# bxh1/VIDO-SLAM

Hardware: AMD Instinct MI355X
Metric: frames/sec end-to-end (flow+depth+track+local-BA) at 640x480; BA iters/sec (higher is better)
Workload: dtype f32

## Files before the change

include/vido_c.h:

```cpp
#ifndef VIDO_C_H
#define VIDO_C_H
#include <stdint.h>
#include <stddef.h>
#ifdef __cplusplus
extern "C" {
#endif

#define VIDO_OK              0
#define VIDO_E_INVALID      -1
#define VIDO_E_NO_DEVICE    -2
#define VIDO_E_HIP          -3
#define VIDO_E_CAPACITY     -4
#define VIDO_E_NOMEM        -5

#define VIDO_MAX_LEVELS 16

typedef struct vido_ctx vido_ctx;

typedef struct vido_keypoint { float x, y, size, angle, response; int32_t octave; } vido_keypoint;

typedef struct vido_config {
    int32_t device;
    int32_t width, height;
    int32_t max_batch;
// ... 93 lines not shown
    double info_edge, info_prior, huber_delta;
    int32_t use_huber, rounds, drop_kernel_after_round;
    int32_t iters[4];
    float chi2_th[4];
} vido_pose_problem;

typedef struct vido_pose_result { double T[16]; int32_t n_inliers, lm_iterations; double chi2_final; } vido_pose_result;

int vido_pose_optimize(vido_ctx* ctx, const vido_pose_problem* prob, vido_pose_result* result, uint8_t* outlier_out, double* flow_out);
int vido_pose_optimize_batch(vido_ctx* ctx, const vido_pose_problem* probs, int n_prob, vido_pose_result* results,
                             uint8_t* const* outlier_out, double* const* flow_out);

typedef struct vido_ba_problem {
    int32_t n_cam, n_pt, n_obs, n_odo, prior_cam, use_huber, max_iters, pad;
    double* cam_T; double* pt_xyz;
    const int32_t* obs_cam; const int32_t* obs_pt; const double* obs_meas;
    const int32_t* odo_i; const int32_t* odo_j; const double* odo_T;
    double prior_T[12];
    double info_obs, info_odo, info_prior, huber_obs, huber_odo, gain_threshold;
    int32_t pt_lo, pt_hi;
    int32_t rank, world;
} vido_ba_problem;

typedef struct vido_ba_result { int32_t iterations, lm_trials; double chi2_initial, chi2_final, lambda_final;
                                double ms_setup;
                                double ms_solve_loop;
                                double ms_linearize_kernel;
                                double ms_schur_kernel;
} vido_ba_result;

typedef int (*vido_allreduce_fn)(void* user, void* dev_ptr, size_t count, int op);

int vido_ba_optimize(vido_ctx* ctx, vido_ba_problem* prob, vido_ba_result* result, vido_allreduce_fn allreduce, void* user);
int vido_rccl_unique_id(uint8_t id_out[128]);
int vido_rccl_init(vido_ctx* ctx, const uint8_t id[128], int rank, int world);
int vido_rccl_allreduce(void* user_ctx, void* dev_ptr, size_t count, int op);
int vido_rccl_destroy(vido_ctx* ctx);

typedef struct vido_ba_dynamic {
    int32_t n_H, n_dyn, n_tern, n_smooth;
    double* H_T;
    double* dyn_xyz;
    const int32_t* dyn_cam; const double* dyn_meas;
    const int32_t* tern_prev; const int32_t* tern_cur; const int32_t* tern_H;
    const int32_t* sm_i; const int32_t* sm_j;
    double info_dyn, info_tern, info_smooth, huber_dyn, huber_tern, huber_smooth;
} vido_ba_dynamic;
int vido_ba_optimize_dynamic(vido_ctx* ctx, vido_ba_problem* prob, vido_ba_dynamic* dyn, vido_ba_result* result,
                             vido_allreduce_fn allreduce, void* user);

int vido_correlation(vido_ctx* ctx, const float* first, const float* second, int B, int C, int H, int W, int stride,
                     float* out, int on_device);
int vido_det_order(vido_ctx* ctx, const float* scores, const long long* labels, const int* n_det, float confidence, int cap, long long* order, long long* labels_out, long long* n_live);
int vido_roi_levels(vido_ctx* ctx, const float* boxes, int n, float k_min, float k_max, int* out);
int vido_mask_logit_select(vido_ctx* ctx, const float* feat, const float* w, const float* b, const long long* labels, float* out, int n, int c, int hw, int classes);
int vido_bias_act(vido_ctx* ctx, float* x, const float* bias, int N, int C, int H, int W, float slope);
int vido_bias_unary(vido_ctx* ctx, float* x, const float* bias, int N, int C, int H, int W, int kind);
int vido_upcat_reflect(vido_ctx* ctx, const float* x, const float* skip, int C1, int C2, int h, int w, float* out);
int vido_minmax_norm_u16(vido_ctx* ctx, const float* d, const float* mm, int64_t n, int32_t* out);
int vido_bias_res_act(vido_ctx* ctx, float* x, const float* bias, const float* res, int N, int C, int H, int W, float slope);
int vido_area_feed(vido_ctx* ctx, const uint8_t* bgr, int H, int W, float* out, int OH, int OW, float div);
int vido_backwarp(vido_ctx* ctx, const float* x, const float* flow, int B, int C, int H, int W, float* out);
int vido_deconv4s2_depthwise(vido_ctx* ctx, const float* x, const float* weight, int B, int C, int H, int W, float input_slope, float* out);

int vido_conv1x1_supported(int cin, int cout, int hw);
int vido_conv1x1_layout(int cin, int cout, int hw);
int vido_conv1x1_set_arith(int arith);
int vido_conv1x1_range_flag(vido_ctx* ctx, int reset);
int vido_range_latch(vido_ctx* ctx, unsigned* dst);
int vido_conv1x1_bias_act(vido_ctx* ctx, const float* x, const float* w_packed, const float* bias, const float* residual, float* y, int cin, int cout, int hw, float slope);
int vido_deconv2x2_supported(int n, int cin, int cout, int h, int w);
int vido_deconv2x2_bias_act(vido_ctx* ctx, const float* x, const float* w_packed, const float* bias, float* y, int n, int cin, int cout, int h, int w, float slope);
int vido_conv1x1_bias_up2_act(vido_ctx* ctx, const float* x, const float* w_packed, const float* bias, const float* residual_half, float* y, int cin, int cout, int h, int w, float slope);

int vido_conv_kxk_c2(vido_ctx* ctx, const float* x, const float* w, const float* bias, const float* residual, float* y, int cin, int k, int h, int w_);
int vido_conv1x1_skinny(vido_ctx* ctx, const float* x, const float* w_packed, const float* bias, const float* residual, float* y, int cin, int cout, long long hw, float slope);

int vido_conv_direct_supported(int cin, int cout, int h, int w, int kh, int kw, int sh, int sw, int ph, int pw);
long long vido_conv_direct_packed_floats(int cin, int cout, int kh, int kw);
int vido_conv_direct_pack(const float* w, int cin, int cout, int kh, int kw, float* w_packed);
int vido_conv_direct_bias_act(vido_ctx* ctx, const float* x, const float* w_packed, const float* bias, float* y, int n, int cin, int cout, int h, int w,
                              int kh, int kw, int sh, int sw, int ph, int pw, float slope);

int vido_wino3x3_supported(int cin, int cout, int h, int w);
int vido_wino3x3_fills_chip(int n, int cout, int h, int w, int min_wgs);
long long vido_wino3x3_packed_floats(int cin, int cout);
int vido_wino3x3_pack(const float* w, int cin, int cout, float* u_packed);
int vido_wino3x3_bias_act(vido_ctx* ctx, const float* x, const float* u_packed, const float* bias, float* y, int n, int cin, int cout, int h, int w, float slope);
int vido_wino3x3_form(int n, int cin, int cout, int h, int w);
int vido_fc_h_splitk(int rows, int k, int outs);
int vido_fc_h(vido_ctx* ctx, const float* x, const void* w_packed, const float* bias, float* part, float* y, int rows, int k, int outs, float slope);
int vido_conv3x3_h_supported(int n, int cin, int cout, int h, int w);
int vido_conv3x3_h_workgroups(int n, int cout, int h, int w);
int vido_conv3x3_h_bias_act(vido_ctx* ctx, const float* x, const void* w_packed, const float* bias, float* y, int n, int cin, int cout, int h, int w, float slope);
long long vido_wino3x3_packed_floats_form(int cin, int cout, int form);
int vido_wino3x3_pack_form(const float* w, int cin, int cout, int form, float* u_packed);
int vido_wino3x3_bias_act_form(vido_ctx* ctx, const float* x, const float* u_packed, const float* bias, float* y, int n, int cin, int cout, int h, int w, float slope, int form);
int vido_gconv3x3_supported(int H, int W, int cpg_in, int cpg_out);
int64_t vido_gconv3x3_packed_size(int groups, int cpg_in, int cpg_out);
int vido_gconv3x3_bias_act(vido_ctx* ctx, const float* x, const float* in_bias, const float* w_packed, const float* bias, float* y, int groups, int cpg_in, int cpg_out, int H, int W, float slope);
int vido_gconv3x3_s2_supported(int H, int W, int cpg_in, int cpg_out);
int vido_gconv3x3_s2_bias_act(vido_ctx* ctx, const float* x, const float* w_packed, const float* bias, float* y, int groups, int cpg_in, int cpg_out, int H, int W, float slope);
int vido_lfn_reg_front(vido_ctx* ctx, const float* im1, const float* im2, const float* flow, const float* mean, float scale, int B, int C, int H, int W, float* out, int out_channels);
int vido_lfn_reg_tail(vido_ctx* ctx, const float* dist, const float* flow, const float* wx, const float* bx, const float* wy, const float* by, int B, int K, int H, int W, float* out);
int vido_roi_align(vido_ctx* ctx, const float* feat, int B, int C, int H, int W, const float* rois, int n_rois,
                   float spatial_scale, int pooled_h, int pooled_w, int sampling_ratio, float* out, int on_device);
int vido_nms(vido_ctx* ctx, const float* boxes_xyxy, const float* scores, int n, float thresh, int32_t* keep_out,
             int32_t* n_keep, int on_device);
int vido_nms_grouped(vido_ctx* ctx, const float* boxes_xyxy, const float* scores, const int32_t* groups, int n, float thresh,
                     int32_t* keep_out, int32_t* n_keep, int on_device);
int vido_nms_segments(vido_ctx* ctx, const float* boxes_xyxy, const int32_t* groups, const int32_t* seg_off, const int32_t* seg_n, int n_seg, int max_n, int total,
                      float thresh, int32_t* keep_out, int32_t* n_keep);
int vido_roi_align_fpn(vido_ctx* ctx, const float* const feat[4], const int H[4], const int W[4], const float scale[4], int C, const float* boxes, const int32_t* level,
                       int n, int pooled_h, int pooled_w, int sampling_ratio, float* out);
int vido_nchw_to_nhwc(vido_ctx* ctx, const float* src, int B, int C, int H, int W, float* dst);
int vido_roi_align_fpn_nhwc(vido_ctx* ctx, const float* const feat[4], const int H[4], const int W[4], const float scale[4], int C, const float* boxes, const int32_t* level,
                            int n, int pooled_h, int pooled_w, int sampling_ratio, float* out);
int vido_bawin_create(vido_ctx* ctx, int cap_frames, int cap_features);
int vido_bawin_push_frame(vido_ctx* ctx, int frame, int n, const double* meas, const float* xyz, const int32_t* asso);
int vido_bawin_set_labels(vido_ctx* ctx, int n, const int32_t* quads);
int vido_bawin_solve(vido_ctx* ctx, int start, int N, vido_ba_problem* prob, vido_ba_result* res, int32_t* n_obs_out, int32_t* n_pt_out);
int vido_bawin_read_points(vido_ctx* ctx, int frame, int n, float* xyz_out);
int vido_rpn_select(vido_ctx* ctx, int n_levels, const float* const* logits, const float* const* deltas, const int* h, const int* w, const int* stride, const float* cell_anchors,
                    int A, int K, int img_w, int img_h, float* boxes_out, float* scores_out, int32_t* n_out);
int vido_rpn_merge(vido_ctx* ctx, const float* boxes, const float* scores, const int32_t* keep, const int32_t* cnt, int n_levels, int K, int post_nms_top_n, int n_final,
                   float* out_boxes, float* out_scores, int32_t* n_valid);
int vido_det_class_sort(vido_ctx* ctx, const float* prob, const float* deltas, const float* proposals, const float* objectness, int N, int nc, float thresh, const float weights[4],
                        int img_w, int img_h, float* seg_boxes, int32_t* order, int32_t* seg_n);
int vido_det_select(vido_ctx* ctx, const float* prob, const float* seg_boxes, const int32_t* order, const int32_t* keep, const int32_t* cnt, int N, int nc, int detections_per_img, int cap,
                    int32_t* scratch, float* out_boxes, float* out_scores, int64_t* out_labels, int32_t* n_det);
int vido_mask_label_image(vido_ctx* ctx, const float* masks, const float* boxes, const int64_t* labels, int n, int M, int padding, float thresh, int H, int W, uint8_t* out);
int vido_mask_instance_image(vido_ctx* ctx, const float* masks, const float* boxes, const int64_t* labels, int n, int M, int padding, float thresh, int H, int W,
                             const int32_t* id_base_dev, uint8_t* out, int32_t* area_out);
int vido_box_decode(vido_ctx* ctx, const float* deltas, const float* boxes, int n, int k, const float weights[4],
                    float* out, int on_device);

int vido_pnp_ransac(vido_ctx* ctx, const float* pts3d, const float* pts2d, int n, double fx, double fy, double cx, double cy,
                    int max_iters, double reproj_err, double confidence, uint64_t seed, double T_out[16], uint8_t* inlier_mask,
                    int32_t* n_inliers);

int vido_pnp_ransac_batch(vido_ctx* ctx, int n_prob, const float* const* pts3d, const float* const* pts2d, const int32_t* n, double fx, double fy, double cx, double cy,
                          int max_iters, double reproj_err, double confidence, const uint64_t* seeds, double* T_out, uint8_t* const* inlier_mask, int32_t* n_inliers);

typedef struct vido_host_maps { const int32_t* mask; const float* depth; const float* flow; int32_t width, height; } vido_host_maps;
float vido_depth_noise(float z, unsigned seed);
int vido_undistort_points(const float* xy, int n, const float K[4], const float dist[5], float* xy_out);
int vido_renew_static(const vido_host_maps* maps, const float* stat_xy, int n_stat, const int32_t* TM_sta, int n_tm, const float* sample_xy, int n_sample,
                      int max_num, int32_t* src_out, int32_t* inlier_out, float* flow_out, int cap, int32_t* n_out);
int vido_renew_objects(const vido_host_maps* maps, const float* obj_xy, const int32_t* obj_label, int n_obj_pts,
                       int n_objects, const int32_t* inl_off, const int32_t* inl_ids, const uint8_t* obj_stat, const int32_t* sem_position, const int32_t* mod_label,
                       const float* tmp_xy, const float* tmp_depth, const int32_t* tmp_sem, const float* tmp_flow, const float* tmp_corr, int n_tmp, int max_num_obj,
                       float* keys_out, float* depth_out, int32_t* sem_out, float* flow_out, float* corr_out, int32_t* inlier_out, int32_t* label_out, int cap, int32_t* n_out);
typedef struct vido_point_samples { const int32_t* mask; const float* depth; const float* flow; } vido_point_samples;
int vido_renew_static_sampled(int width, int height, const float* stat_xy, int n_stat, const vido_point_samples* stat_samples, const int32_t* TM_sta, int n_tm,
                              const float* sample_xy, int n_sample, const vido_point_samples* sample_samples, int max_num,
                              int32_t* src_out, int32_t* inlier_out, float* flow_out, int cap, int32_t* n_out);
int vido_renew_objects_sampled(int width, int height, const float* obj_xy, const int32_t* obj_label, int n_obj_pts, const vido_point_samples* obj_samples,
                               int n_objects, const int32_t* inl_off, const int32_t* inl_ids, const uint8_t* obj_stat, const int32_t* sem_position, const int32_t* mod_label,
                               const float* tmp_xy, const float* tmp_depth, const int32_t* tmp_sem, const float* tmp_flow, const float* tmp_corr, int n_tmp, int max_num_obj,
                               float* keys_out, float* depth_out, int32_t* sem_out, float* flow_out, float* corr_out, int32_t* inlier_out, int32_t* label_out, int cap, int32_t* n_out);
int vido_dyn_obj_tracking(const int32_t* sem_label, int32_t* obj_label, const float* obj_xy, const float* obj_depth, const float* flow3d, const int32_t* last_sem_label, int n,
                          const int32_t* last_sem_position, const uint8_t* last_obj_stat, const int32_t* last_mod_label, int n_last, int rows, int cols,
                          float sf_mg_thres, float sf_ds_thres, float th_depth_obj, int f_id, int32_t* max_id,
                          int32_t* obj_off, int32_t* obj_ids, int32_t* mod_label_out, int32_t* sem_position_out, int max_objects, int32_t* n_objects);

int vido_tracklets_incremental(int n_rows, const int32_t* row_off, const int32_t* row_n, const int32_t* TM, const int32_t* labels, int n_feat0,
                               int32_t* trk_off, int32_t* pairs, int32_t* obj_id, int32_t* owner_trk, int32_t* owner_pos, int cap_trk, int cap_pairs, int32_t* n_trk);

typedef struct vido_system vido_system;
typedef struct vido_system_stats {
// ... 30 lines not shown
```

vido-slam_amd/csrc/conv1x1.hip:

```cpp
#include "common.hpp"
#include <atomic>

namespace {
typedef float f32x16 __attribute__((ext_vector_type(16)));
typedef float f32x4 __attribute__((ext_vector_type(4)));
typedef float f32x2 __attribute__((ext_vector_type(2)));

#define C1_TM 128
#define C1_TN 128

struct C1Args { const float* x; const float* wp; const float* bias; const float* res; float* y; int M, N, K, mt, total, nchunk; float slope; unsigned xbytes, wbytes; int W; unsigned* range_flag; int hwimg, c4; };

template <int RES, int KC>
__global__ __launch_bounds__(256) void k_conv1x1(C1Args A)
{
    constexpr int NG = KC / 8;
    constexpr int A_BUF = 4 * NG * 256, B_BUF = KC * C1_TN;
    constexpr int NPW = KC / 4;
    extern __shared__ __attribute__((aligned(16))) float c1_lds[];
    float* Al = c1_lds; float* Bl = c1_lds + 2 * A_BUF;
    const int tid = threadIdx.x, lane = tid & 63, w = __builtin_amdgcn_readfirstlane(tid >> 6), wm = w & 1, wn = w >> 1;
    const int per = gridDim.x >> 3, item = (blockIdx.x & 7) * per + (blockIdx.x >> 3);
    if (item >= A.total) return;
    const int nt = item / A.mt, mtile = item - nt * A.mt, n0 = nt * C1_TN, m0 = mtile * C1_TM;
    const __amdgpu_buffer_rsrc_t wr = __builtin_amdgcn_make_buffer_rsrc((void*)A.wp, 0, A.wbytes, 0x00020000);
    const unsigned avo = 16u * (unsigned)lane;
    const unsigned bvo = 4u * ((unsigned)(lane >> 5) * (unsigned)A.N + (unsigned)(n0 + 4 * (lane & 31)));
    const int kg = A.K / 8;
    auto issue = [&](int chunk, int buf, int first, int count) {
#pragma unroll
        for (int q = first; q < first + count; q++) {
            if (q >= NPW) break;
            const int i = 4 * q + w;
            if (q < NG) {
                const int mb = i / NG, g = i - mb * NG;
                const unsigned so = 4u * (unsigned)((((m0 >> 5) + mb) * kg + chunk * NG + g) * 256);
                __builtin_amdgcn_raw_ptr_buffer_load_lds(wr, (__attribute__((address_space(3))) void*)(Al + buf * A_BUF + i * 256), 16, avo, so, 0, 0);
            } else {
                const int p = i - 4 * NG;
                const unsigned so = 4u * (unsigned)(chunk * KC + 2 * p) * (unsigned)A.N;
                const __amdgpu_buffer_rsrc_t xr = __builtin_amdgcn_make_buffer_rsrc((void*)((const char*)A.x + so), 0, A.xbytes - so, 0x00020000);
                __builtin_amdgcn_raw_ptr_buffer_load_lds(xr, (__attribute__((address_space(3))) void*)(Bl + buf * B_BUF + 2 * p * C1_TN), 16, bvo, 0, 0, 0);
            }
        }
    };
    f32x16 acc[2][2];
#pragma unroll
    for (int mi = 0; mi < 2; mi++)
#pragma unroll
        for (int ni = 0; ni < 2; ni++)
#pragma unroll
            for (int r = 0; r < 16; r++) acc[mi][ni][r] = 0.f;
    issue(0, 0, 0, NPW);
    constexpr int PG = (NPW + (NG > 2 ? NG - 3 : 0)) / (NG > 2 ? NG - 2 : 1);
    for (int c = 0; c < A.nchunk; c++) {
        asm volatile("s_waitcnt vmcnt(0)" ::: "memory");
        __syncthreads();
        const int nb = (c + 1) & 1, cn = min(c + 1, A.nchunk - 1);
        const float* Ab = Al + (c & 1) * A_BUF + (2 * wm * NG) * 256 + lane * 4;
        const float* Bb = Bl + (c & 1) * B_BUF + (lane >> 5) * C1_TN + 64 * wn + (lane & 31);
        typedef const __attribute__((address_space(3))) float* lds_f;
        lds_f Bb1 = (lds_f)(Bb + 32);
        asm("" : "+v"(Bb1));
        lds_f Bb0 = (lds_f)Bb;
// ... 128 lines not shown
                __builtin_amdgcn_sched_group_barrier(0x008, 1, 0);
                __builtin_amdgcn_sched_group_barrier(0x100, 1, 0);
                __builtin_amdgcn_sched_group_barrier(0x020, 1, 0);
            }
        }
        __builtin_amdgcn_sched_barrier(0);
    }
    asm volatile("s_waitcnt vmcnt(0)" ::: "memory");
#pragma unroll
    for (int mi = 0; mi < 2; mi++)
#pragma unroll
        for (int j = 0; j < 7; j++) {
            const int co0 = m0 + 32 * w + 16 * mi + 4 * (lane >> 4), q = n0 + 16 * j + (lane & 15);
            if (q < A.N) {
                float rv[4], bv[4];
                size_t rq = (size_t)q, rn = (size_t)A.N;
                if (RES == 2) { const int yy = q / A.W, xx = q - yy * A.W; rq = (size_t)(yy >> 1) * (A.W >> 1) + (xx >> 1); rn = (size_t)(A.N / A.W >> 1) * (A.W >> 1); }
#pragma unroll
                for (int r = 0; r < 4; r++) { bv[r] = A.bias ? A.bias[co0 + r] : 0.f; rv[r] = RES ? A.res[(size_t)(co0 + r) * rn + rq] : 0.f; }
#pragma unroll
                for (int r = 0; r < 4; r++) {
                    const float v = acc[mi][j][r] + bv[r] + rv[r];
                    A.y[(size_t)(co0 + r) * A.N + q] = fmaxf(v, v * A.slope);
                }
            }
        }
}

typedef __bf16 bf16x8 __attribute__((ext_vector_type(8)));
typedef _Float16 f16x8 __attribute__((ext_vector_type(8)));
typedef _Float16 f16x2 __attribute__((ext_vector_type(2)));
typedef unsigned u32x4 __attribute__((ext_vector_type(4)));
#define B3_SLOTB(NP) ((NP) * 4096 + 8192)
#define B3_PWN(NP) ((NP) + 2)

__device__ __forceinline__ unsigned b3_cvt_pk(float lo, float hi) { unsigned r; asm("v_cvt_pk_bf16_f32 %0, %1, %2" : "=v"(r) : "v"(lo), "v"(hi)); return r; }
__device__ __forceinline__ void b3_split2(float x0, float x1, unsigned& p0, unsigned& p1, unsigned& p2)
{
    p0 = b3_cvt_pk(x0, x1);
    const float r0 = x0 - __uint_as_float(p0 << 16), r1 = x1 - __uint_as_float(p0 & 0xffff0000u);
    p1 = b3_cvt_pk(r0, r1);
    const float s0 = r0 - __uint_as_float(p1 << 16), s1 = r1 - __uint_as_float(p1 & 0xffff0000u);
    p2 = b3_cvt_pk(s0, s1);
}

template <int RES, int G, int RB, int NP>
__global__ __launch_bounds__(256 * G, (G == 1 && RB != 6) ? 2 : G) void k_conv1x1_b3(C1Args A)
{
    constexpr int B3_SLOT = B3_SLOTB(NP), B3_PW = B3_PWN(NP);
    constexpr int SLOTB = G * B3_SLOT;
    extern __shared__ __attribute__((aligned(16))) float c1_lds[];
    char* L = (char*)c1_lds;
    const int tid = threadIdx.x, lane = tid & 63, wv = __builtin_amdgcn_readfirstlane(tid >> 6), w = wv & 3, g = wv >> 2;
    const int per = gridDim.x >> 3, item = (blockIdx.x & 7) * per + (blockIdx.x >> 3);
    if (item >= A.total) return;
    const int nt = item / A.mt, mtile = item - nt * A.mt, n0 = nt * C1_TN, m0 = mtile * C1_TM;
    const int ns = A.nchunk, nb = ns / G;
    const __amdgpu_buffer_rsrc_t wr = __builtin_amdgcn_make_buffer_rsrc((void*)A.wp, 0, A.wbytes, 0x00020000);
    const unsigned avo = 16u * (unsigned)lane;
    unsigned abase[3], bvo[2];
#pragma unroll
    for (int q = 0; q < NP; q++) { const int i = 4 * q + w, rb = i / NP, pl = i - NP * rb; abase[q] = 1024u * (unsigned)(((m0 >> 5) + rb) * ns * NP + pl); }
    unsigned pbase = 4u * (unsigned)(n0 + 4 * (lane & 31)), rowb = 4u * (unsigned)A.N;
    if (A.hwimg) { const int p = n0 + 4 * (lane & 31), img = p / A.hwimg; pbase = 4u * ((unsigned)img * (unsigned)A.K * (unsigned)A.hwimg + (unsigned)(p - img * A.hwimg)); rowb = 4u * (unsigned)A.hwimg; }
#pragma unroll
    for (int q = 0; q < 2; q++) bvo[q] = (unsigned)((lane >> 5) + 2 * (4 * q + w)) * rowb + pbase;
    const unsigned bstep = 16u * rowb;
    const int wofs = g * B3_SLOT + w * 1024;
    auto issue = [&](int T, int slot) {
        char* S = L + slot * SLOTB + wofs;
        const int t = G * T + g;
        const unsigned aoff = (unsigned)(NP * 1024) * (unsigned)t, boff = bstep * (unsigned)t;
#pragma unroll
        for (int q = 0; q < NP; q++) __builtin_amdgcn_raw_ptr_buffer_load_lds(wr, (__attribute__((address_space(3))) void*)(S + q * 4096), 16, avo, abase[q] + aoff, 0, 0);
        const __amdgpu_buffer_rsrc_t xr = __builtin_amdgcn_make_buffer_rsrc((void*)((const char*)A.x + boff), 0, A.xbytes - boff, 0x00020000);
#pragma unroll
        for (int q = 0; q < 2; q++) __builtin_amdgcn_raw_ptr_buffer_load_lds(xr, (__attribute__((address_space(3))) void*)(S + NP * 4096 + q * 4096), 16, bvo[q], 0, 0, 0);
    };
    f32x16 acc[4], acl[4];
#pragma unroll
    for (int rb = 0; rb < 4; rb++)
#pragma unroll
        for (int r = 0; r < 16; r++) { acc[rb][r] = 0.f; acl[rb][r] = 0.f; }
    for (int T = 0; T < RB - 1; T++) issue(min(T, nb - 1), T);
    u32x4 a[2][4][NP], bp[2][NP]; float braw[8];
    float xmax = 0.f;
    const f32x2 k2048 = {2048.f, 2048.f};
    typedef const __attribute__((address_space(3))) char* lds_c;
    const unsigned a_lane = (unsigned)(g * B3_SLOT) + 16u * (unsigned)lane, b_lane = (unsigned)(g * B3_SLOT) + (unsigned)(NP * 4096) + 4u * (unsigned)((lane >> 5) * 8 * C1_TN + 32 * w + (lane & 31));
    auto lda = [&](int slot, int buf) {
        lds_c Ab = (lds_c)(L + slot * SLOTB) + a_lane;
#pragma unroll
        for (int rb = 0; rb < 4; rb++)
#pragma unroll
            for (int pl = 0; pl < NP; pl++) a[buf][rb][pl] = *(const __attribute__((address_space(3))) u32x4*)(Ab + (rb * NP + pl) * 1024);
    };
    auto ldb = [&](int slot) {
#ifdef H2_PRESPLIT_EMU
        if (NP == 2) return;
#endif
        const __attribute__((address_space(3))) float* Bb = (const __attribute__((address_space(3))) float*)((lds_c)(L + slot * SLOTB) + b_lane);
#pragma unroll
        for (int i = 0; i < 8; i++) braw[i] = Bb[i * C1_TN];
    };
    auto split = [&](int buf) {
        if constexpr (NP == 2) {
#ifdef H2_PRESPLIT_EMU
            { lds_c Bq = (lds_c)(L + (buf ? SLOTB : 0)) + 16u * (unsigned)lane; bp[buf][0] = *(const __attribute__((address_space(3))) u32x4*)(Bq + 8192); bp[buf][1] = *(const __attribute__((address_space(3))) u32x4*)(Bq + 9216); }
            return;
#endif
#pragma unroll
            for (int pr = 0; pr < 4; pr++) {
                const f32x2 v = {braw[2 * pr], braw[2 * pr + 1]};
                const f16x2 h = __builtin_convertvector(v, f16x2);
                f32x2 vs, r;
                asm("v_pk_mul_f32 %0, %1, %2" : "=v"(vs) : "v"(v), "v"(k2048));
                asm("v_fma_mix_f32 %0, %1, %2, %3 op_sel_hi:[1,0,0]" : "=v"(r.x) : "v"(h), "s"(-2048.f), "v"(vs.x));
                asm("v_fma_mix_f32 %0, %1, %2, %3 op_sel:[1,0,0] op_sel_hi:[1,0,0]" : "=v"(r.y) : "v"(h), "s"(-2048.f), "v"(vs.y));
                const f16x2 l = __builtin_convertvector(r, f16x2);
                bp[buf][0][pr] = __builtin_bit_cast(unsigned, h); bp[buf][1][pr] = __builtin_bit_cast(unsigned, l);
                xmax = __builtin_elementwise_maximum(__builtin_elementwise_maximum(xmax, __builtin_fabsf(v.x)), __builtin_fabsf(v.y));
            }
        } else {
#pragma unroll
#ifdef B3_NOSPLIT
            for (int pr = 0; pr < 4; pr++) { bp[buf][0][pr] = __float_as_uint(braw[2 * pr]); bp[buf][1][pr] = __float_as_uint(braw[2 * pr + 1]); bp[buf][2][pr] = __float_as_uint(braw[2 * pr]) ^ 1; }
#else
            for (int pr = 0; pr < 4; pr++) { unsigned p0, p1, p2; b3_split2(braw[2 * pr], braw[2 * pr + 1], p0, p1, p2); bp[buf][0][pr] = p0; bp[buf][1][pr] = p1; bp[buf][2][pr] = p2; }
// ... 25 lines not shown
                        d = __builtin_amdgcn_mfma_f32_32x32x16_f16(__builtin_bit_cast(f16x8, a[h][rb][PA[term]]), __builtin_bit_cast(f16x8, bp[h][PB[term]]), d, 0, 0, 0);
                    }
                }
                split(h ^ 1);
                __builtin_amdgcn_sched_group_barrier(0x002, 2, 0);
#pragma unroll
                for (int i = 0; i < 12; i++) {
                    __builtin_amdgcn_sched_group_barrier(0x008, 1, 0);
                    if (i < 4) __builtin_amdgcn_sched_group_barrier(0x100, 3, 0); else if (i < 6) __builtin_amdgcn_sched_group_barrier(0x100, 2, 0);
                    if (i >= 1 && i < 5) __builtin_amdgcn_sched_group_barrier(0x020, 1, 0);
                    if (i >= 4) __builtin_amdgcn_sched_group_barrier(0x002, 4, 0);
                }
            } else {
#pragma unroll
            for (int term = 0; term < 6; term++) {
                constexpr int PA[6] = {0, 1, 2, 0, 1, 0}, PB[6] = {2, 1, 0, 1, 0, 0};
#pragma unroll
                for (int rb = 0; rb < 4; rb++) {
                    f32x16& d = term == 5 ? acc[rb] : acl[rb];
                    d = __builtin_amdgcn_mfma_f32_32x32x16_bf16(__builtin_bit_cast(bf16x8, a[h][rb][PA[term]]), __builtin_bit_cast(bf16x8, bp[h][PB[term]]), d, 0, 0, 0);
                }
            }
            split(h ^ 1);
            __builtin_amdgcn_sched_group_barrier(0x002, 2, 0);
#pragma unroll
            for (int i = 0; i < 24; i++) {
                __builtin_amdgcn_sched_group_barrier(0x008, 1, 0);
                if (i < 8) __builtin_amdgcn_sched_group_barrier(0x100, 2, 0); else if (i < 12) __builtin_amdgcn_sched_group_barrier(0x100, 1, 0);
                if (i >= 3 && i < 8) __builtin_amdgcn_sched_group_barrier(0x020, 1, 0);
                if (i >= 6) __builtin_amdgcn_sched_group_barrier(0x002, 3, 0);
            }
            }
            __builtin_amdgcn_sched_barrier(0);
            slot = sn;
        }
    }
    asm volatile("s_waitcnt vmcnt(0) lgkmcnt(0)" ::: "memory");
#pragma unroll
    for (int rb = 0; rb < 4; rb++) acc[rb] += NP == 2 ? acl[rb] * 0x1p-11f : acl[rb];
    if (NP == 2 && !(xmax < 65504.f) && A.range_flag) atomicOr(A.range_flag, 1u);
    const float* wsc = (const float*)((const char*)A.wp + (size_t)4 * A.K * A.M);
    struct Ep { float rv[16], bv[16], sv[16]; };
    const int q_out = n0 + 32 * w + (lane & 31);
    size_t rq = (size_t)q_out, rn = (size_t)A.N;
    if (RES == 2) { const int yy = q_out / A.W, xx = q_out - yy * A.W; rq = (size_t)(yy >> 1) * (A.W >> 1) + (xx >> 1); rn = (size_t)(A.N / A.W >> 1) * (A.W >> 1); }
    size_t oq = (size_t)q_out, on = (size_t)A.N; int co_sub = 0;
    if (RES == 3) {
        const int tap = m0 / A.c4, img = q_out / A.hwimg, rem = q_out - img * A.hwimg, ii = rem / A.W, jj = rem - ii * A.W;
        co_sub = tap * A.c4; on = (size_t)4 * A.hwimg;
        oq = (size_t)img * A.c4 * on + (size_t)(2 * ii + (tap >> 1)) * (2 * A.W) + 2 * jj + (tap & 1);
    }
    auto ep_load = [&](int rb, Ep& E) {
        const int co0 = m0 + 32 * rb + 4 * (lane >> 5);
        if (q_out < A.N) {
#pragma unroll
            for (int r = 0; r < 16; r++) {
                const int co = co0 + 8 * (r >> 2) + (r & 3);
                E.bv[r] = A.bias ? A.bias[co - co_sub] : 0.f;
                E.rv[r] = (RES == 1 || RES == 2) ? A.res[(size_t)co * rn + rq] : 0.f;
                E.sv[r] = NP == 2 ? wsc[co] : 1.f;
            }
        }
    };
    auto ep_store = [&](int rb, const f32x16& v0, const float* other, const Ep& E) {
        const int co0 = m0 + 32 * rb + 4 * (lane >> 5);
        float ov[16];
#pragma unroll
        for (int r = 0; r < 16; r++) ov[r] = other ? other[r * 64] : 0.f;
        if (q_out < A.N) {
#pragma unroll
            for (int r = 0; r < 16; r++) {
                const int co = co0 + 8 * (r >> 2) + (r & 3);
                const float v = (NP == 2 ? (v0[r] + ov[r]) * E.sv[r] : v0[r] + ov[r]) + E.bv[r] + E.rv[r];
                A.y[(size_t)(co - co_sub) * on + oq] = fmaxf(v, v * A.slope);
            }
        }
    };
    Ep E0, E1;
    if (G == 1) {
        ep_load(0, E0);
        ep_load(1, E1); ep_store(0, acc[0], nullptr, E0);
        ep_load(2, E0); ep_store(1, acc[1], nullptr, E1);
        ep_load(3, E1); ep_store(2, acc[2], nullptr, E0);
        ep_store(3, acc[3], nullptr, E1);
    } else {
        float* X = (float*)L;
        if (g == 0) { ep_load(0, E0); ep_load(1, E1); } else { ep_load(2, E0); ep_load(3, E1); }
        __builtin_amdgcn_s_barrier();
        auto put = [&](int which, const f32x16& v0, const f32x16& v1) {
            float* Pw = X + (((which * 4 + w) * 2) * 16) * 64 + lane;
#pragma unroll
            for (int r = 0; r < 16; r++) { Pw[r * 64] = v0[r]; Pw[(16 + r) * 64] = v1[r]; }
        };
        if (g == 1) put(0, acc[0], acc[1]); else put(1, acc[2], acc[3]);
        __syncthreads();
        const float* Pr = X + (((g * 4 + w) * 2) * 16) * 64 + lane;
        if (g == 0) { ep_store(0, acc[0], Pr, E0); ep_store(1, acc[1], Pr + 16 * 64, E1); }
        else { ep_store(2, acc[2], Pr, E0); ep_store(3, acc[3], Pr + 16 * 64, E1); }
    }
}
}

extern "C" {

int vido_conv1x1_supported(int cin, int cout, int hw)
{
    return cin >= 32 && cin % 32 == 0 && cout >= C1_TM && cout % C1_TM == 0 && hw >= C1_TN && 4ll * cin * hw < (1ll << 32) && 4ll * cin * cout < (1ll << 32);
}

static std::atomic<int>& c1_arith()
{
    static std::atomic<int> v{[] { const char* e = getenv("VIDO_CONV1X1_ARITH");
                                   return (e && !strcmp(e, "f32")) || (!e && getenv("VIDO_CONV1X1_TN")) ? 1 : (e && (!strcmp(e, "bf16x3") || !strcmp(e, "bf16"))) ? 2 : 0; }()};
    return v;
}

int vido_conv1x1_set_arith(int arith) { return c1_arith().exchange(arith == 1 ? 1 : arith == 2 ? 2 : 0); }

int vido_conv1x1_range_flag(vido_ctx* ctx, int reset)
{
    if (!ctx || !ctx->c1_range_flag) return 0;
    return reset ? (int)__atomic_exchange_n(ctx->c1_range_flag, 0u, __ATOMIC_ACQ_REL) : (int)__atomic_load_n(ctx->c1_range_flag, __ATOMIC_ACQUIRE);
}

int vido_conv1x1_layout(int cin, int cout, int hw)
{
    { const int ar = c1_arith().load(std::memory_order_relaxed); if (ar != 1) return ar == 2 ? 2 : 3; }
    static const int force = [] { const char* e = getenv("VIDO_CONV1X1_TN"); return e ? atoi(e) : 128; }();
    if (force == 128 || cin % 64 != 0) return 0;
    if (force == 112) return 1;
    const long long mt = cout / C1_TM, t128 = mt * ((hw + 127) / 128), t112 = mt * ((hw + C2_TN - 1) / C2_TN);
    const long long c128 = ((t128 + 255) / 256) * 128, c112 = ((t112 + 255) / 256) * C2_TN;
    return c112 < c128 ? 1 : 0;
}

static int c1_launch(vido_ctx* ctx, const float* x, const float* w_packed, const float* bias, const float* residual, int res_mode, float* y, int cin, int cout, int hw, int w, float slope,
                     int hwimg = 0, int c4 = 0)
{
    if (!ctx) return VIDO_E_INVALID;
    if (!x || !w_packed || !y || x == y || !vido_conv1x1_supported(cin, cout, hw) || slope < 0.f || slope > 1.f || (((uintptr_t)x | (uintptr_t)y | (uintptr_t)residual) & 3) || ((uintptr_t)w_packed & 15))
        return vido_set_error(ctx, VIDO_E_INVALID, "conv1x1: no kernel for %d -> %d channels at %d positions (or a pointer is misaligned, or slope outside [0, 1])", cin, cout, hw);
    HIP_TRY(ctx, hipSetDevice(ctx->device));
    hipStream_t st = ctx->has_ext_stream ? ctx->ext_stream : ctx->stream;
    const int rm = res_mode == 3 ? 3 : (residual ? res_mode : 0);
    const int layout = vido_conv1x1_layout(cin, cout, hw);
    if ((hwimg || rm == 3) && layout != 3) return vido_set_error(ctx, VIDO_E_INVALID, "conv1x1: the batch / transposed-convolution forms exist in the split-fp16 arithmetic only");
    if (layout >= 2) {
        const int np = layout == 3 ? 2 : 3;
        const int mt = cout / C1_TM, ntl = (hw + C1_TN - 1) / C1_TN, total = mt * ntl;
        C1Args A{x, w_packed, bias, residual, y, cout, hw, cin, mt, total, cin / 16, slope, (unsigned)(4ll * cin * hw), (unsigned)(2ll * np * cin * cout), w, ctx->c1_range_flag, hwimg, c4};
        static const int force_form = [] { const char* e = getenv("VIDO_CONV1X1_B3_FORM"); return e ? atoi(e) : 0; }();
        int form = force_form ? force_form : (cin >= 512 && total <= 320 ? 2 : 3);
        if (form == 2 && cin % 64) form = 3;
        static bool attr3[64] = {};
        if (!attr3[ctx->device & 63]) {
#define B3_ATTR(G_, RB_, NP_) for (const void* f : {(const void*)k_conv1x1_b3<0, G_, RB_, NP_>, (const void*)k_conv1x1_b3<1, G_, RB_, NP_>, (const void*)k_conv1x1_b3<2, G_, RB_, NP_>}) \
            HIP_TRY(ctx, hipFuncSetAttribute(f, hipFuncAttributeMaxDynamicSharedMemorySize, (int)((size_t)RB_ * G_ * B3_SLOTB(NP_))))
            B3_ATTR(1, 6, 3); B3_ATTR(2, 4, 3); B3_ATTR(1, 4, 3); B3_ATTR(2, 5, 2); B3_ATTR(1, 5, 2); B3_ATTR(1, 4, 2); B3_ATTR(1, 3, 2);
#undef B3_ATTR
            HIP_TRY(ctx, hipFuncSetAttribute((const void*)k_conv1x1_b3<3, 2, 5, 2>, hipFuncAttributeMaxDynamicSharedMemorySize, (int)((size_t)5 * 2 * B3_SLOTB(2))));
            HIP_TRY(ctx, hipFuncSetAttribute((const void*)k_conv1x1_b3<3, 1, 5, 2>, hipFuncAttributeMaxDynamicSharedMemorySize, (int)((size_t)5 * 1 * B3_SLOTB(2))));
            attr3[ctx->device & 63] = true;
        }
        const dim3 grid(8 * ((total + 7) / 8));
#define B3_LAUNCH(G_, RB_, NP_) do { const dim3 blk(256 * G_); const size_t lds = (size_t)RB_ * G_ * B3_SLOTB(NP_); \
            if (rm == 2) hipLaunchKernelGGL((k_conv1x1_b3<2, G_, RB_, NP_>), grid, blk, lds, st, A); else if (rm) hipLaunchKernelGGL((k_conv1x1_b3<1, G_, RB_, NP_>), grid, blk, lds, st, A); \
            else hipLaunchKernelGGL((k_conv1x1_b3<0, G_, RB_, NP_>), grid, blk, lds, st, A); } while (0)
        static const int rb_short = [] { const char* e = getenv("VIDO_CONV1X1_H2_RB"); return e ? atoi(e) : 5; }();
        if (rm == 3) {
            if (form == 2) hipLaunchKernelGGL((k_conv1x1_b3<3, 2, 5, 2>), grid, dim3(512), (size_t)5 * 2 * B3_SLOTB(2), st, A);
            else hipLaunchKernelGGL((k_conv1x1_b3<3, 1, 5, 2>), grid, dim3(256), (size_t)5 * B3_SLOTB(2), st, A);
        }
        else if (np == 2) { if (form == 2) B3_LAUNCH(2, 5, 2); else if (rb_short == 4) B3_LAUNCH(1, 4, 2); else if (rb_short == 3) B3_LAUNCH(1, 3, 2); else B3_LAUNCH(1, 5, 2); }
        else if (form == 2) B3_LAUNCH(2, 4, 3); else if (form == 1) B3_LAUNCH(1, 6, 3); else B3_LAUNCH(1, 4, 3);
#undef B3_LAUNCH
        HIP_TRY(ctx, hipGetLastError());
        return VIDO_OK;
    }
    if (layout == 1) {
        const int mt = cout / C1_TM, ntl = (hw + C2_TN - 1) / C2_TN, total = mt * ntl;
        C1Args A{x, w_packed, bias, residual, y, cout, hw, cin, mt, total, cin / 64, slope, (unsigned)(4ll * cin * hw), (unsigned)(4ll * cin * cout), w};
        constexpr size_t LDS112 = (size_t)2 * (8 * 4 * 256 + 2 * 16 * 272) * 4;
        static bool attr2[64] = {};
        if (!attr2[ctx->device & 63]) {
            for (const void* f : {(const void*)k_conv1x1_n112<0, 64>, (const void*)k_conv1x1_n112<1, 64>, (const void*)k_conv1x1_n112<2, 64>}) HIP_TRY(ctx, hipFuncSetAttribute(f, hipFuncAttributeMaxDynamicSharedMemorySize, (int)LDS112));
            attr2[ctx->device & 63] = true;
        }
        const dim3 grid(8 * ((total + 7) / 8)), blk(256);
        if (rm == 2) hipLaunchKernelGGL((k_conv1x1_n112<2, 64>), grid, blk, LDS112, st, A); else if (rm) hipLaunchKernelGGL((k_conv1x1_n112<1, 64>), grid, blk, LDS112, st, A); else hipLaunchKernelGGL((k_conv1x1_n112<0, 64>), grid, blk, LDS112, st, A);
        HIP_TRY(ctx, hipGetLastError());
        return VIDO_OK;
    }
    const int mt = cout / C1_TM, ntl = (hw + C1_TN - 1) / C1_TN, total = mt * ntl;
    static const int force_kc = [] { const char* e = getenv("VIDO_CONV1X1_KC"); return e ? atoi(e) : 0; }();
    const int kc = (cin % 64 == 0 && force_kc != 32) ? 64 : 32;
    C1Args A{x, w_packed, bias, residual, y, cout, hw, cin, mt, total, cin / kc, slope, (unsigned)(4ll * cin * hw), (unsigned)(4ll * cin * cout), w};
    const dim3 grid(8 * ((total + 7) / 8)), blk(256);
    constexpr size_t LDS64 = (size_t)2 * (4 * 8 * 256 + 64 * C1_TN) * 4, LDS32 = (size_t)2 * (4 * 4 * 256 + 32 * C1_TN) * 4;
    static bool attr[64] = {};
    if (!attr[ctx->device & 63]) {
        for (const void* f : {(const void*)k_conv1x1<0, 64>, (const void*)k_conv1x1<1, 64>, (const void*)k_conv1x1<2, 64>}) HIP_TRY(ctx, hipFuncSetAttribute(f, hipFuncAttributeMaxDynamicSharedMemorySize, (int)LDS64));
        for (const void* f : {(const void*)k_conv1x1<0, 32>, (const void*)k_conv1x1<1, 32>, (const void*)k_conv1x1<2, 32>}) HIP_TRY(ctx, hipFuncSetAttribute(f, hipFuncAttributeMaxDynamicSharedMemorySize, (int)LDS32));
        attr[ctx->device & 63] = true;
    }
    if (kc == 64) { if (rm == 2) hipLaunchKernelGGL((k_conv1x1<2, 64>), grid, blk, LDS64, st, A); else if (rm) hipLaunchKernelGGL((k_conv1x1<1, 64>), grid, blk, LDS64, st, A); else hipLaunchKernelGGL((k_conv1x1<0, 64>), grid, blk, LDS64, st, A); }
    else { if (rm == 2) hipLaunchKernelGGL((k_conv1x1<2, 32>), grid, blk, LDS32, st, A); else if (rm) hipLaunchKernelGGL((k_conv1x1<1, 32>), grid, blk, LDS32, st, A); else hipLaunchKernelGGL((k_conv1x1<0, 32>), grid, blk, LDS32, st, A); }
    HIP_TRY(ctx, hipGetLastError());
    return VIDO_OK;
}

int vido_deconv2x2_supported(int n, int cin, int cout, int h, int w)
{
    return n >= 1 && h >= 1 && w >= 1 && cout >= 128 && cout % 128 == 0 && (h * w) % 4 == 0 && (long long)n * h * w < (1ll << 28) && vido_conv1x1_supported(cin, 4 * cout, n * h * w)
           && 16ll * n * cout * h * w < (1ll << 32) && vido_conv1x1_layout(cin, 4 * cout, n * h * w) == 3;
}
int vido_deconv2x2_bias_act(vido_ctx* ctx, const float* x, const float* w_packed, const float* bias, float* y, int n, int cin, int cout, int h, int w, float slope)
{
    if (ctx && !vido_deconv2x2_supported(n, cin, cout, h, w)) return vido_set_error(ctx, VIDO_E_INVALID, "deconv2x2: no kernel for %d x %d -> %d channels at %d x %d", n, cin, cout, h, w);
    return c1_launch(ctx, x, w_packed, bias, nullptr, 3, y, cin, 4 * cout, n * h * w, w, slope, h * w, cout);
}

int vido_conv1x1_bias_act(vido_ctx* ctx, const float* x, const float* w_packed, const float* bias, const float* residual, float* y, int cin, int cout, int hw, float slope)
{
    return c1_launch(ctx, x, w_packed, bias, residual, 1, y, cin, cout, hw, hw, slope);
}

int vido_conv1x1_bias_up2_act(vido_ctx* ctx, const float* x, const float* w_packed, const float* bias, const float* residual_half, float* y, int cin, int cout, int h, int w, float slope)
{
    if (ctx && (h < 2 || w < 2 || (h & 1) || (w & 1) || !residual_half)) return vido_set_error(ctx, VIDO_E_INVALID, "conv1x1 (upsampled residual): %d x %d must be even and the residual given", h, w);
    return c1_launch(ctx, x, w_packed, bias, residual_half, 2, y, cin, cout, h * w, w, slope);
}

}
```

vido-slam_amd/csrc/conv3x3h.hip:

```cpp
#include "common.hpp"
#include <type_traits>

namespace {
typedef float f32x16 __attribute__((ext_vector_type(16)));
typedef float f32x2 __attribute__((ext_vector_type(2)));
typedef _Float16 f16x8 __attribute__((ext_vector_type(8)));
typedef _Float16 f16x2 __attribute__((ext_vector_type(2)));
typedef unsigned u32x4 __attribute__((ext_vector_type(4)));

#define C3_OOB 0x40000000u
#define C3_WSLOT 24576
#define C3_RBW 3
#define C3_WPIX(BR) (((BR) + 2) * 18)
#define C3_XP(BR) ((16 * C3_WPIX(BR) + 511) / 512)
#define C3_RAW(BR) (C3_XP(BR) * 8 * 256)
#define C3_PLANE(BR) (C3_WPIX(BR) * 32)
#define C3_PBUF(BR) (2 * C3_PLANE(BR))
#define C3_LDS(BR) (C3_RBW * C3_WSLOT + C3_RAW(BR) + 2 * C3_PBUF(BR))

struct C3Args { const float* x; const void* wp; const float* bias; float* y; int N, Cin, Cout, H, W, nby, nbx, mt, total, nchunk; float slope; unsigned wbytes; unsigned* range_flag; };

template <int RPW, int CG>
__global__ __launch_bounds__(512) void k_conv3x3_h(C3Args A)
{
    constexpr int BR = 16 / CG, MT = 32 * RPW * CG, WPIX = C3_WPIX(BR), XP = C3_XP(BR), RAWB = C3_RAW(BR), PLANE = C3_PLANE(BR), PBUF = C3_PBUF(BR), CK = (WPIX * 8 + 511) / 512, NMM = 9 * RPW, NRD = 2 * RPW + 2;
    extern __shared__ __attribute__((aligned(16))) char c3_lds[];
    char* L = c3_lds;
    const int tid = threadIdx.x, lane = tid & 63, w = __builtin_amdgcn_readfirstlane(tid >> 6);
    const int per = gridDim.x >> 3, item = (blockIdx.x & 7) * per + (blockIdx.x >> 3);
    if (item >= A.total) return;
    const int nt = item / A.mt, mtile = item - nt * A.mt, m0 = mtile * MT;
    const int bpi = A.nby * A.nbx, n = nt / bpi, brem = nt - n * bpi, by = brem / A.nbx, bx = brem - by * A.nbx, Y0 = by * BR, X0 = bx * 16;
    const int rp = CG == 1 ? w : (w & 3), rb0 = CG == 1 ? 0 : RPW * (w >> 2);
    const int hw = A.H * A.W, nsteps = A.nchunk * 3;

    const __amdgpu_buffer_rsrc_t wr = __builtin_amdgcn_make_buffer_rsrc((void*)A.wp, 0, A.wbytes, 0x00020000);
    const unsigned avo = 16u * (unsigned)lane;
    unsigned abase[3], avq[3];
#pragma unroll
    for (int q = 0; q < 3; q++) { const int i = w + 8 * q, rb = i / 6, rem = i - 6 * rb; abase[q] = 1024u * (unsigned)(((m0 >> 5) + rb) * A.nchunk * 18 + rem); avq[q] = rb < RPW * CG ? avo : 0x80000000u; }
    unsigned xvo[11];
#pragma unroll
    for (int j = 0; j < XP; j++) {
        const int e = 64 * (8 * j + w) + lane, ch = e / WPIX, rem = e - ch * WPIX, row = rem / 18, col = rem - row * 18, gy = Y0 - 1 + row, gx = X0 - 1 + col;
        xvo[j] = (e < 16 * WPIX && gy >= 0 && gy < A.H && gx >= 0 && gx < A.W) ? 4u * (unsigned)(ch * hw + gy * A.W + gx) : C3_OOB;
    }
    const unsigned ximg = 4u * (unsigned)n * (unsigned)A.Cin * (unsigned)hw, ximg_end = ximg + 4u * (unsigned)A.Cin * (unsigned)hw, xchunk = 64u * (unsigned)hw;
    char* const RAW = L + C3_RBW * C3_WSLOT;
    char* const PL = RAW + RAWB;
    auto issue_w = [&](int s, int slot) {
        char* S = L + slot * C3_WSLOT + w * 1024;
        const unsigned so = 6144u * (unsigned)s;
#pragma unroll
        for (int q = 0; q < 3; q++) __builtin_amdgcn_raw_ptr_buffer_load_lds(wr, (__attribute__((address_space(3))) void*)(S + q * 8192), 16, avq[q], abase[q] + so, 0, 0);
    };
    auto issue_x = [&](int c) {
        const unsigned so = ximg + xchunk * (unsigned)c;
        const __amdgpu_buffer_rsrc_t xc = __builtin_amdgcn_make_buffer_rsrc((void*)((const char*)A.x + so), 0, ximg_end - so, 0x00020000);
#pragma unroll
        for (int j = 0; j < XP; j++) __builtin_amdgcn_raw_ptr_buffer_load_lds(xc, (__attribute__((address_space(3))) void*)(RAW + (8 * j + w) * 256), 4, xvo[j], 0, 0, 0);
    };
    float xmax = 0.f;
    const f32x2 k2048 = {2048.f, 2048.f};
    auto convert = [&](int buf) {
        const float* R = (const float*)RAW;
        unsigned* P = (unsigned*)(PL + buf * PBUF);
#pragma unroll
        for (int k = 0; k < CK; k++) {
            const int idx = tid + 512 * k;
            if (k < CK - 1 || idx < WPIX * 8) {
                const int q = idx / WPIX, pix = idx - q * WPIX;
                const f32x2 v = {R[(2 * q) * WPIX + pix], R[(2 * q + 1) * WPIX + pix]};
                const f16x2 h = __builtin_convertvector(v, f16x2);
                f32x2 vs, r;
                asm("v_pk_mul_f32 %0, %1, %2" : "=v"(vs) : "v"(v), "v"(k2048));
                asm("v_fma_mix_f32 %0, %1, %2, %3 op_sel_hi:[1,0,0]" : "=v"(r.x) : "v"(h), "s"(-2048.f), "v"(vs.x));
                asm("v_fma_mix_f32 %0, %1, %2, %3 op_sel:[1,0,0] op_sel_hi:[1,0,0]" : "=v"(r.y) : "v"(h), "s"(-2048.f), "v"(vs.y));
                const f16x2 l = __builtin_convertvector(r, f16x2);
                P[pix * 8 + q] = __builtin_bit_cast(unsigned, h); P[PLANE / 4 + pix * 8 + q] = __builtin_bit_cast(unsigned, l);
                xmax = __builtin_elementwise_maximum(__builtin_elementwise_maximum(xmax, __builtin_fabsf(v.x)), __builtin_fabsf(v.y));
            }
        }
    };
// ... 60 lines not shown
        asm volatile("s_waitcnt vmcnt(3) lgkmcnt(0)\n\ts_barrier" ::: "memory");
        step(std::integral_constant<int, 2>{}, std::integral_constant<int, 3>{}, pbuf, [&] { const int sf = slot == 0 ? C3_RBW - 1 : slot - 1; issue_w(min(3 * c + 4, nsteps - 1), sf); });
        convert(pbuf ^ 1);
        slot = slot + 1 == C3_RBW ? 0 : slot + 1;
    }
    asm volatile("s_waitcnt vmcnt(0) lgkmcnt(0)" ::: "memory");
#pragma unroll
    for (int rb = 0; rb < RPW; rb++) acc[rb] += acl[rb] * 0x1p-11f;
    if (!(xmax < 65504.f) && A.range_flag) atomicOr(A.range_flag, 1u);

    const float* wsc = (const float*)((const char*)A.wp + (size_t)A.nchunk * 16 * 18 * A.Cout * 2);
    const int p = lane & 31, Y = Y0 + 2 * rp + (p >> 4), X = X0 + (p & 15);
    const bool inside = Y < A.H && X < A.W;
    float* yb = A.y + (size_t)n * A.Cout * hw + (size_t)Y * A.W + X;
#pragma unroll
    for (int rb = 0; rb < RPW; rb++) {
        float bv[16], sv[16];
#pragma unroll
        for (int r = 0; r < 16; r++) { const int co = m0 + 32 * (rb0 + rb) + 8 * (r >> 2) + 4 * (lane >> 5) + (r & 3); bv[r] = A.bias ? A.bias[co] : 0.f; sv[r] = wsc[co]; }
        if (inside) {
#pragma unroll
            for (int r = 0; r < 16; r++) {
                const int co = m0 + 32 * (rb0 + rb) + 8 * (r >> 2) + 4 * (lane >> 5) + (r & 3);
                const float v = acc[rb][r] * sv[r] + bv[r];
                yb[(size_t)co * hw] = fmaxf(v, v * A.slope);
            }
        }
    }
}
}

extern "C" {

int vido_conv3x3_h_supported(int n, int cin, int cout, int h, int w)
{
    const long long cp = (cin + 15) / 16 * 16;
    return n >= 1 && cin >= 1 && (cout == 32 || cout == 64 || (cout >= 128 && cout % 128 == 0)) && h >= 1 && w >= 1 && 4ll * n * cin * h * w < (1ll << 30) && 4ll * n * cout * h * w < (1ll << 30)
           && 36ll * cp * cout < (1ll << 31);
}

#define C3_MIN16 190
static int c3_block_rows(int n, int cout, int h, int w)
{
    static const int force = [] { const char* e = getenv("VIDO_CONV3X3_H_ROWS"); return e ? atoi(e) : 0; }();
    if (cout == 32) return 16;
    if (force == 16 || force == 8) return force;
    const int mt = cout >= 128 ? cout / 128 : 1;
    return n * ((h + 15) / 16) * ((w + 15) / 16) * mt >= C3_MIN16 ? 16 : 8;
}
int vido_conv3x3_h_workgroups(int n, int cout, int h, int w) { const int br = c3_block_rows(n, cout, h, w); return n * ((h + br - 1) / br) * ((w + 15) / 16) * (cout >= 128 ? cout / 128 : 1); }

int vido_conv3x3_h_bias_act(vido_ctx* ctx, const float* x, const void* w_packed, const float* bias, float* y, int n, int cin, int cout, int h, int w, float slope)
{
    if (!ctx) return VIDO_E_INVALID;
    if (!x || !w_packed || !y || x == y || !vido_conv3x3_h_supported(n, cin, cout, h, w) || slope < 0.f || slope > 1.f || (((uintptr_t)x | (uintptr_t)y) & 3) || ((uintptr_t)w_packed & 15))
        return vido_set_error(ctx, VIDO_E_INVALID, "conv3x3_h: no kernel for %d x %d -> %d channels at %d x %d (or a pointer is misaligned, or slope outside [0, 1])", n, cin, cout, h, w);
    HIP_TRY(ctx, hipSetDevice(ctx->device));
    hipStream_t st = ctx->has_ext_stream ? ctx->ext_stream : ctx->stream;
    const int br = c3_block_rows(n, cout, h, w);
    const int nby = (h + br - 1) / br, nbx = (w + 15) / 16, mt = cout >= 128 ? cout / 128 : 1, total = n * nby * nbx * mt;
    const int nchunk = (cin + 15) / 16;
    C3Args A{x, w_packed, bias, y, n, cin, cout, h, w, nby, nbx, mt, total, nchunk, slope, (unsigned)(36ll * 16 * nchunk * cout), ctx->c1_range_flag};
    static bool attr[64] = {};
    if (!attr[ctx->device & 63]) {
#define C3_ATTR(RPW_, CG_) HIP_TRY(ctx, hipFuncSetAttribute((const void*)k_conv3x3_h<RPW_, CG_>, hipFuncAttributeMaxDynamicSharedMemorySize, (int)C3_LDS(16 / CG_)))
        C3_ATTR(4, 1); C3_ATTR(2, 2); C3_ATTR(2, 1); C3_ATTR(1, 2); C3_ATTR(1, 1);
#undef C3_ATTR
        attr[ctx->device & 63] = true;
    }
    const dim3 grid(8 * ((total + 7) / 8));
#define C3_LAUNCH(RPW_, CG_) hipLaunchKernelGGL((k_conv3x3_h<RPW_, CG_>), grid, dim3(512), C3_LDS(16 / CG_), st, A)
    if (cout >= 128) { if (br == 16) C3_LAUNCH(4, 1); else C3_LAUNCH(2, 2); }
    else if (cout == 64) { if (br == 16) C3_LAUNCH(2, 1); else C3_LAUNCH(1, 2); }
    else C3_LAUNCH(1, 1);
#undef C3_LAUNCH
    HIP_TRY(ctx, hipGetLastError());
    return VIDO_OK;
}

}
```

vido-slam_amd/csrc/nets.hip:

```cpp
#include "common.hpp"
#include <numeric>

#define CORR_CH 8
__global__ __launch_bounds__(256) void k_correlation(const float* __restrict__ f1, const float* __restrict__ f2, int C, int H, int W, int s,
                                                     int Ho, int Wo, float* __restrict__ out, int nsplit, int cper)
{
    __shared__ float t2[CORR_CH][22][23];
    const int tx = threadIdx.x & 15, ty = threadIdx.x >> 4, b = blockIdx.z / nsplit, split = blockIdx.z - b * nsplit;
    const int c_lo = split * cper, c_hi = min(C, c_lo + cper);
    const int x = blockIdx.x * 16 + tx, y = blockIdx.y * 16 + ty;
    const bool valid = x < Wo && y < Ho;
    float acc[49];
#pragma unroll
    for (int k = 0; k < 49; k++) acc[k] = 0.f;
    const size_t plane = (size_t)H * W;
    for (int c0 = c_lo; c0 < c_hi; c0 += CORR_CH) {
        const int nc = min(CORR_CH, c_hi - c0);
        for (int i = threadIdx.x; i < nc * 22 * 22; i += 256) {
            const int cc = i / (22 * 22), r = (i / 22) % 22, q = i % 22;
            const int yy = (blockIdx.y * 16 + r - 3), xx = (blockIdx.x * 16 + q - 3);
            float v = 0.f;
            if (yy >= 0 && yy < Ho && xx >= 0 && xx < Wo) v = f2[((size_t)b * C + c0 + cc) * plane + (size_t)(yy * s) * W + xx * s];
            t2[cc][r][q] = v;
        }
        float a[CORR_CH];
#pragma unroll
        for (int cc = 0; cc < CORR_CH; cc++) a[cc] = (valid && cc < nc) ? f1[((size_t)b * C + c0 + cc) * plane + (size_t)(y * s) * W + x * s] : 0.f;
        __syncthreads();
#pragma unroll
        for (int cc = 0; cc < CORR_CH; cc++) {
            if (cc < nc) {
#pragma unroll
                for (int p = 0; p < 7; p++)
#pragma unroll
                    for (int o = 0; o < 7; o++) acc[p * 7 + o] += a[cc] * t2[cc][ty + p][tx + o];
            }
        }
        __syncthreads();
    }
    if (valid) {
        float* o = out + (size_t)split * (gridDim.z / nsplit) * 49 * Ho * Wo;
#pragma unroll
        for (int k = 0; k < 49; k++) o[(((size_t)b * 49 + k) * Ho + y) * Wo + x] = nsplit == 1 ? acc[k] / (float)C : acc[k];
    }
}
__global__ __launch_bounds__(256) void k_correlation_reduce(const float* __restrict__ part, int nsplit, size_t n, float inv_c_dummy, int C, float* __restrict__ out)
{
    const size_t i = blockIdx.x * (size_t)blockDim.x + threadIdx.x;
    if (i >= n) return;
    float sum = 0.f;
    for (int k = 0; k < nsplit; k++) sum += part[(size_t)k * n + i];
    out[i] = sum / (float)C;
}

__global__ __launch_bounds__(1024) void k_det_order(const float* __restrict__ scores, const long long* __restrict__ labels, const int* __restrict__ n_det, float confidence, int cap,
                                                   long long* __restrict__ order, long long* __restrict__ labels_out, long long* __restrict__ n_live)
{
    __shared__ float key[1024];
    __shared__ int cnt;
    const int i = threadIdx.x;
    if (i == 0) cnt = 0;
    const int nd = *n_det;
    bool live = false;
    if (i < cap) { live = scores[i] > confidence && i < nd; key[i] = live ? scores[i] : -1.0f; }
    __syncthreads();
    if (i < cap) {
        const float k = key[i]; int rank = 0;
        for (int j = 0; j < cap; j++) { const float kj = key[j]; rank += (kj > k) || (kj == k && j < i); }
        order[rank] = i; labels_out[rank] = live ? labels[i] : 0;
        if (live) atomicAdd(&cnt, 1);
    }
    __syncthreads();
    if (i == 0) *n_live = cnt;
}

__global__ void k_roi_levels(const float* __restrict__ boxes, int n, float k_min, float k_max, int* __restrict__ out)
{
    const int i = blockIdx.x * blockDim.x + threadIdx.x;
    if (i >= n) return;
    const float x1 = boxes[4 * i], y1 = boxes[4 * i + 1], x2 = boxes[4 * i + 2], y2 = boxes[4 * i + 3];
    const float area = __fmul_rn(__fadd_rn(__fsub_rn(x2, x1), 1.f), __fadd_rn(__fsub_rn(y2, y1), 1.f));
    const float t = __fadd_rn(__fdiv_rn(__fsqrt_rn(area), 224.f), 1e-6f);
    float l = floorf(__fadd_rn(4.f, log2f(t)));
    l = fminf(fmaxf(l, k_min), k_max);
    out[i] = (int)l - (int)k_min;
}

__global__ __launch_bounds__(256) void k_mask_logit_select(const float* __restrict__ feat, const float* __restrict__ w, const float* __restrict__ b, const long long* __restrict__ labels,
                                                           float* __restrict__ out, int c, int hw, int classes)
{
    __shared__ float wl[1024];
    const int n = blockIdx.y, p = blockIdx.x * 256 + threadIdx.x;
    long long lab = labels[n]; lab = lab < 0 ? 0 : (lab >= classes ? classes - 1 : lab);
    for (int i = threadIdx.x; i < c; i += 256) wl[i] = w[(size_t)lab * c + i];
    __syncthreads();
    if (p >= hw) return;
    const float* f = feat + (size_t)n * c * hw + p;
    double a0 = 0, a1 = 0, a2 = 0, a3 = 0;
    int i = 0;
    for (; i + 4 <= c; i += 4) { a0 += (double)wl[i] * f[(size_t)i * hw]; a1 += (double)wl[i + 1] * f[(size_t)(i + 1) * hw]; a2 += (double)wl[i + 2] * f[(size_t)(i + 2) * hw]; a3 += (double)wl[i + 3] * f[(size_t)(i + 3) * hw]; }
    for (; i < c; i++) a0 += (double)wl[i] * f[(size_t)i * hw];
    const float v = (float)((a0 + a1) + (a2 + a3) + (b ? (double)b[lab] : 0.0));
    out[(size_t)n * hw + p] = 1.f / (1.f + expf(-v));
}

__global__ __launch_bounds__(256) void k_bias_act(float* __restrict__ x, const float* __restrict__ bias, int C, size_t hw, size_t total, float slope)
{
    const size_t i = (blockIdx.x * (size_t)blockDim.x + threadIdx.x) * 4;
    if (i >= total) return;
    if ((hw & 3) == 0) {
        const float b = bias[(i / hw) % C];
        float4 v = *(float4*)(x + i);
        v.x += b; v.y += b; v.z += b; v.w += b;
        v.x = v.x > 0.f ? v.x : v.x * slope; v.y = v.y > 0.f ? v.y : v.y * slope; v.z = v.z > 0.f ? v.z : v.z * slope; v.w = v.w > 0.f ? v.w : v.w * slope;
        *(float4*)(x + i) = v;
    } else {
        for (size_t k = i; k < min(i + 4, total); k++) { float v = x[k] + bias[(k / hw) % C]; x[k] = v > 0.f ? v : v * slope; }
    }
}

template <int KIND>
__global__ __launch_bounds__(256) void k_bias_unary(float* __restrict__ x, const float* __restrict__ bias, int C, size_t hw, size_t total)
{
    const size_t i = blockIdx.x * (size_t)blockDim.x + threadIdx.x;
    if (i >= total) return;
    const float v = x[i] + bias[(i / hw) % C];
    x[i] = KIND == 1 ? (v > 0.f ? v : expf(v) - 1.f) : 1.f / (1.f + expf(-v));
}

__global__ __launch_bounds__(256) void k_upcat_reflect(const float* __restrict__ x, const float* __restrict__ skip, int C1, int C2, int h, int w, float* __restrict__ out)
{
    const int H2 = 2 * h, W2 = 2 * w, OW = W2 + 2, OH = H2 + 2;
    const size_t i = blockIdx.x * (size_t)blockDim.x + threadIdx.x, total = (size_t)(C1 + C2) * OH * OW;
    if (i >= total) return;
    const int X = (int)(i % OW), Y = (int)((i / OW) % OH), c = (int)(i / ((size_t)OW * OH));
    int yy = Y - 1, xx = X - 1;
    yy = yy < 0 ? -yy : (yy >= H2 ? 2 * H2 - 2 - yy : yy); xx = xx < 0 ? -xx : (xx >= W2 ? 2 * W2 - 2 - xx : xx);
    out[i] = c < C1 ? x[((size_t)c * h + (yy >> 1)) * w + (xx >> 1)] : skip[((size_t)(c - C1) * H2 + yy) * W2 + xx];
}

__global__ __launch_bounds__(256) void k_minmax_norm_u16(const float* __restrict__ d, const float* __restrict__ mm, size_t n, int* __restrict__ out)
{
    const size_t i = blockIdx.x * (size_t)blockDim.x + threadIdx.x;
    if (i >= n) return;
    const float lo = mm[0], hi = mm[1];
    float v = (d[i] - lo) / (hi - lo + 1e-12f) * 65536.0f;
    v = fminf(fmaxf(v, 0.f), 65535.f);
    out[i] = (int)v;
}

__global__ __launch_bounds__(256) void k_bias_res_act(float* __restrict__ x, const float* __restrict__ bias, const float* __restrict__ res, int C, size_t hw, size_t total, float slope)
{
    const size_t i = (blockIdx.x * (size_t)blockDim.x + threadIdx.x) * 4;
    if (i >= total) return;
    if ((hw & 3) == 0) {
        const float b = bias[(i / hw) % C];
        float4 v = *(float4*)(x + i); const float4 r = *(const float4*)(res + i);
        v.x += b + r.x; v.y += b + r.y; v.z += b + r.z; v.w += b + r.w;
        v.x = v.x > 0.f ? v.x : v.x * slope; v.y = v.y > 0.f ? v.y : v.y * slope; v.z = v.z > 0.f ? v.z : v.z * slope; v.w = v.w > 0.f ? v.w : v.w * slope;
        *(float4*)(x + i) = v;
    } else {
        for (size_t k = i; k < min(i + 4, total); k++) { float v = x[k] + bias[(k / hw) % C] + res[k]; x[k] = v > 0.f ? v : v * slope; }
    }
}

struct RoiLevels { const float* feat[4]; int H[4], W[4]; float scale[4]; };
template <int SR >
__global__ __launch_bounds__(256) void k_roi_align_nhwc(RoiLevels L, int C, const float* __restrict__ rois, int roi_stride ,
                                                        const int* __restrict__ level , int PH, int PW, int sampling, float* __restrict__ out)
{
    extern __shared__ __attribute__((aligned(16))) float rl_tile[];
    const int i = blockIdx.x, c0 = blockIdx.y * 64, lane = threadIdx.x & 63, wave = threadIdx.x >> 6;
    const int nbin = PH * PW, pitch = nbin | 1;
    const float* r = rois + (size_t)roi_stride * i;
    const int l = level ? level[i] : 0, bi = roi_stride == 5 ? (int)r[0] : 0;
    const float* box = r + (roi_stride == 5 ? 1 : 0);
    const float scale = L.scale[l]; const int H = L.H[l], W = L.W[l];
    const float sw = box[0] * scale, sh = box[1] * scale, ew = box[2] * scale, eh = box[3] * scale;
    const float rw = fmaxf(ew - sw, 1.f), rh = fmaxf(eh - sh, 1.f);
    const float bh = rh / (float)PH, bw = rw / (float)PW;
    const int gh = SR > 0 ? SR : (sampling > 0 ? sampling : (int)ceilf(rh / PH)), gw = SR > 0 ? SR : (sampling > 0 ? sampling : (int)ceilf(rw / PW));
    const float count = (float)(gh * gw);
    const int c = min(c0 + lane, C - 1);
    const float* d = L.feat[l] + (size_t)bi * H * W * C + c;
    auto taps = [&](float y, float x, int& o1, int& o2, int& o3, int& o4, float& w1, float& w2, float& w3, float& w4) {
        const bool out = y < -1.0 || y > H || x < -1.0 || x > W;
        if (y <= 0) y = 0;
        if (x <= 0) x = 0;
        int yl = out ? 0 : (int)y, xl = out ? 0 : (int)x, yh, xh;
        if (yl >= H - 1) { yh = yl = H - 1; y = (float)yl; } else yh = yl + 1;
        if (xl >= W - 1) { xh = xl = W - 1; x = (float)xl; } else xh = xl + 1;
        const float ly = y - yl, lx = x - xl, hy = 1.f - ly, hx = 1.f - lx;
        o1 = yl * W + xl; o2 = yl * W + xh; o3 = yh * W + xl; o4 = yh * W + xh;
        w1 = hy * hx; w2 = hy * lx; w3 = ly * hx; w4 = ly * lx;
        return out;
    };
    for (int bin = wave; bin < nbin; bin += 4) {
        const int ph = bin / PW, pw = bin - ph * PW;
        float acc = 0.f;
        if (SR == 2) {
            int o[4][4]; float w[4][4], v[4][4]; bool out[4];
#pragma unroll
            for (int s2 = 0; s2 < 4; s2++) {
                const int iy = s2 >> 1, ix = s2 & 1;
                const float y = sh + ph * bh + (float)(iy + .5f) * bh / (float)gh, x = sw + pw * bw + (float)(ix + .5f) * bw / (float)gw;
                out[s2] = taps(y, x, o[s2][0], o[s2][1], o[s2][2], o[s2][3], w[s2][0], w[s2][1], w[s2][2], w[s2][3]);
            }
#pragma unroll
            for (int s2 = 0; s2 < 4; s2++)
#pragma unroll
                for (int t = 0; t < 4; t++) v[s2][t] = d[(size_t)o[s2][t] * C];
#pragma unroll
            for (int s2 = 0; s2 < 4; s2++) acc += out[s2] ? 0.f : (w[s2][0] * v[s2][0] + w[s2][1] * v[s2][1] + w[s2][2] * v[s2][2] + w[s2][3] * v[s2][3]);
        } else {
            for (int iy = 0; iy < gh; iy++) {
                const float y = sh + ph * bh + (float)(iy + .5f) * bh / (float)gh;
                for (int ix = 0; ix < gw; ix++) {
                    const float x = sw + pw * bw + (float)(ix + .5f) * bw / (float)gw;
                    int o1, o2, o3, o4; float w1, w2, w3, w4;
                    if (taps(y, x, o1, o2, o3, o4, w1, w2, w3, w4)) { acc += 0.f; continue; }
                    const float v1 = d[(size_t)o1 * C], v2 = d[(size_t)o2 * C], v3 = d[(size_t)o3 * C], v4 = d[(size_t)o4 * C];
                    acc += (w1 * v1 + w2 * v2 + w3 * v3 + w4 * v4);
                }
            }
// ... 408 lines not shown
    }
    out[((size_t)bc * OH + oy) * OW + ox] = acc;
}

static int roi_lds_limit(vido_ctx* ctx, size_t lds)
{
    static size_t have = 48 * 1024;
    if (lds <= have) return VIDO_OK;
    HIP_TRY(ctx, hipFuncSetAttribute((const void*)k_roi_align_nhwc<2>, hipFuncAttributeMaxDynamicSharedMemorySize, (int)lds));
    HIP_TRY(ctx, hipFuncSetAttribute((const void*)k_roi_align_nhwc<0>, hipFuncAttributeMaxDynamicSharedMemorySize, (int)lds));
    have = lds;
    return VIDO_OK;
}

extern "C" {

int vido_correlation(vido_ctx* ctx, const float* first, const float* second, int B, int C, int H, int W, int stride, float* out, int on_device)
{
    if (!ctx) return VIDO_E_INVALID;
    if (!first || !second || !out || B < 1 || C < 1 || H < 1 || W < 1 || (stride != 1 && stride != 2)) return vido_set_error(ctx, VIDO_E_INVALID, "correlation: bad arguments");
    HIP_TRY(ctx, hipSetDevice(ctx->device));
    hipStream_t st = (on_device && ctx->has_ext_stream) ? ctx->ext_stream : ctx->stream;
    const int Ho = (H + stride - 1) / stride, Wo = (W + stride - 1) / stride;
    const size_t nin = (size_t)B * C * H * W * 4, nout = (size_t)B * 49 * Ho * Wo * 4;
    const float *d1 = first, *d2 = second; float* dout = out;
    const int tiles = ((Wo + 15) / 16) * ((Ho + 15) / 16) * B, nchunk = (C + CORR_CH - 1) / CORR_CH;
    int nsplit = std::max(1, std::min(nchunk, 512 / std::max(tiles, 1)));
    const int cper = ((nchunk + nsplit - 1) / nsplit) * CORR_CH; nsplit = (C + cper - 1) / cper;
    const size_t nel = (size_t)B * 49 * Ho * Wo, io_bytes = on_device ? 0 : 2 * al256(nin) + al256(nout), pbytes = nsplit > 1 ? al256(nel * 4 * nsplit) : 0;
    NetState* S = nullptr;
    if (io_bytes + pbytes) { int rc = net_scratch(ctx, io_bytes + pbytes, &S); if (rc) return rc; }
    if (!on_device) {
        memcpy(S->h, first, nin); memcpy(S->h + al256(nin), second, nin);
        HIP_TRY(ctx, hipMemcpyAsync(S->d, S->h, 2 * al256(nin), hipMemcpyHostToDevice, st));
        d1 = (float*)S->d; d2 = (float*)(S->d + al256(nin)); dout = (float*)(S->d + 2 * al256(nin));
    }
    if (nsplit == 1) hipLaunchKernelGGL(k_correlation, dim3((Wo + 15) / 16, (Ho + 15) / 16, B), dim3(256), 0, st, d1, d2, C, H, W, stride, Ho, Wo, dout, 1, C);
    else {
        float* part = (float*)(S->d + io_bytes);
        hipLaunchKernelGGL(k_correlation, dim3((Wo + 15) / 16, (Ho + 15) / 16, B * nsplit), dim3(256), 0, st, d1, d2, C, H, W, stride, Ho, Wo, part, nsplit, cper);
        hipLaunchKernelGGL(k_correlation_reduce, dim3((unsigned)((nel + 255) / 256)), dim3(256), 0, st, (const float*)part, nsplit, nel, 0.f, C, dout);
    }
    HIP_TRY(ctx, hipGetLastError());
    if (!on_device) {
        HIP_TRY(ctx, hipStreamSynchronize(st));
        HIP_TRY(ctx, hipMemcpyAsync(S->h, dout, nout, hipMemcpyDeviceToHost, st)); HIP_TRY(ctx, hipStreamSynchronize(st));
        memcpy(out, S->h, nout);
    }
    return VIDO_OK;
}

int vido_det_order(vido_ctx* ctx, const float* scores, const long long* labels, const int* n_det, float confidence, int cap, long long* order, long long* labels_out, long long* n_live)
{
    if (!ctx) return VIDO_E_INVALID;
    if (!scores || !labels || !n_det || !order || !labels_out || !n_live || cap < 1 || cap > 1024) return vido_set_error(ctx, VIDO_E_INVALID, "det_order: bad arguments (cap 1 .. 1024)");
    HIP_TRY(ctx, hipSetDevice(ctx->device));
    hipStream_t st = ctx->has_ext_stream ? ctx->ext_stream : ctx->stream;
    hipLaunchKernelGGL(k_det_order, dim3(1), dim3(1024), 0, st, scores, labels, n_det, confidence, cap, order, labels_out, n_live);
    HIP_TRY(ctx, hipGetLastError());
    return VIDO_OK;
}

int vido_roi_levels(vido_ctx* ctx, const float* boxes, int n, float k_min, float k_max, int* out)
{
    if (!ctx) return VIDO_E_INVALID;
    if (!boxes || !out || n < 0 || !(k_min <= k_max)) return vido_set_error(ctx, VIDO_E_INVALID, "roi_levels: bad arguments");
    if (n == 0) return VIDO_OK;
    HIP_TRY(ctx, hipSetDevice(ctx->device));
    hipStream_t st = ctx->has_ext_stream ? ctx->ext_stream : ctx->stream;
    hipLaunchKernelGGL(k_roi_levels, dim3((unsigned)((n + 255) / 256)), dim3(256), 0, st, boxes, n, k_min, k_max, out);
    HIP_TRY(ctx, hipGetLastError());
    return VIDO_OK;
}

int vido_mask_logit_select(vido_ctx* ctx, const float* feat, const float* w, const float* b, const long long* labels, float* out, int n, int c, int hw, int classes)
{
    if (!ctx) return VIDO_E_INVALID;
    if (!feat || !w || !labels || !out || n < 1 || c < 1 || c > 1024 || hw < 1 || classes < 1) return vido_set_error(ctx, VIDO_E_INVALID, "mask_logit_select: bad arguments");
    HIP_TRY(ctx, hipSetDevice(ctx->device));
    hipStream_t st = ctx->has_ext_stream ? ctx->ext_stream : ctx->stream;
    hipLaunchKernelGGL(k_mask_logit_select, dim3((unsigned)((hw + 255) / 256), (unsigned)n), dim3(256), 0, st, feat, w, b, labels, out, c, hw, classes);
    HIP_TRY(ctx, hipGetLastError());
    return VIDO_OK;
}

int vido_bias_act(vido_ctx* ctx, float* x, const float* bias, int N, int C, int H, int W, float slope)
{
    if (!ctx) return VIDO_E_INVALID;
    if (!x || !bias || N < 1 || C < 1 || H < 1 || W < 1) return vido_set_error(ctx, VIDO_E_INVALID, "bias_act: bad arguments");
    HIP_TRY(ctx, hipSetDevice(ctx->device));
    hipStream_t st = ctx->has_ext_stream ? ctx->ext_stream : ctx->stream;
    const size_t hw = (size_t)H * W, total = (size_t)N * C * hw;
    hipLaunchKernelGGL(k_bias_act, dim3((unsigned)((total / 4 + 256) / 256)), dim3(256), 0, st, x, bias, C, hw, total, slope);
    HIP_TRY(ctx, hipGetLastError());
    return VIDO_OK;
}

int vido_bias_unary(vido_ctx* ctx, float* x, const float* bias, int N, int C, int H, int W, int kind)
{
    if (!ctx) return VIDO_E_INVALID;
    if (!x || !bias || N < 1 || C < 1 || H < 1 || W < 1 || (kind != 1 && kind != 2)) return vido_set_error(ctx, VIDO_E_INVALID, "bias_unary: bad arguments");
    HIP_TRY(ctx, hipSetDevice(ctx->device));
    hipStream_t st = ctx->has_ext_stream ? ctx->ext_stream : ctx->stream;
    const size_t hw = (size_t)H * W, total = (size_t)N * C * hw;
    if (kind == 1) hipLaunchKernelGGL(k_bias_unary<1>, dim3((unsigned)((total + 255) / 256)), dim3(256), 0, st, x, bias, C, hw, total);
    else hipLaunchKernelGGL(k_bias_unary<2>, dim3((unsigned)((total + 255) / 256)), dim3(256), 0, st, x, bias, C, hw, total);
    HIP_TRY(ctx, hipGetLastError());
    return VIDO_OK;
}

int vido_upcat_reflect(vido_ctx* ctx, const float* x, const float* skip, int C1, int C2, int h, int w, float* out)
{
    if (!ctx) return VIDO_E_INVALID;
    if (!x || !out || C1 < 1 || C2 < 0 || (C2 && !skip) || h < 1 || w < 1) return vido_set_error(ctx, VIDO_E_INVALID, "upcat_reflect: bad arguments");
    HIP_TRY(ctx, hipSetDevice(ctx->device));
    hipStream_t st = ctx->has_ext_stream ? ctx->ext_stream : ctx->stream;
    const size_t total = (size_t)(C1 + C2) * (2 * h + 2) * (2 * w + 2);
    hipLaunchKernelGGL(k_upcat_reflect, dim3((unsigned)((total + 255) / 256)), dim3(256), 0, st, x, skip, C1, C2, h, w, out);
    HIP_TRY(ctx, hipGetLastError());
    return VIDO_OK;
}

int vido_minmax_norm_u16(vido_ctx* ctx, const float* d, const float* mm, int64_t n, int32_t* out)
{
    if (!ctx) return VIDO_E_INVALID;
    if (!d || !mm || !out || n < 1) return vido_set_error(ctx, VIDO_E_INVALID, "minmax_norm_u16: bad arguments");
    HIP_TRY(ctx, hipSetDevice(ctx->device));
    hipStream_t st = ctx->has_ext_stream ? ctx->ext_stream : ctx->stream;
    hipLaunchKernelGGL(k_minmax_norm_u16, dim3((unsigned)((n + 255) / 256)), dim3(256), 0, st, d, mm, (size_t)n, (int*)out);
    HIP_TRY(ctx, hipGetLastError());
    return VIDO_OK;
}

int vido_area_feed(vido_ctx* ctx, const uint8_t* bgr, int H, int W, float* out, int OH, int OW, float div)
// ... 52 lines not shown
    else hipLaunchKernelGGL(k_lfn_reg_tail<7>, grid, dim3(256), 0, st, dist, flow, wx, bx, wy, by, B, H, W, out);
    HIP_TRY(ctx, hipGetLastError());
    return VIDO_OK;
}

int vido_bias_res_act(vido_ctx* ctx, float* x, const float* bias, const float* res, int N, int C, int H, int W, float slope)
{
    if (!ctx) return VIDO_E_INVALID;
    if (!res) return vido_bias_act(ctx, x, bias, N, C, H, W, slope);
    if (!x || !bias || N < 1 || C < 1 || H < 1 || W < 1) return vido_set_error(ctx, VIDO_E_INVALID, "bias_res_act: bad arguments");
    HIP_TRY(ctx, hipSetDevice(ctx->device));
    hipStream_t st = ctx->has_ext_stream ? ctx->ext_stream : ctx->stream;
    const size_t hw = (size_t)H * W, total = (size_t)N * C * hw;
    hipLaunchKernelGGL(k_bias_res_act, dim3((unsigned)((total / 4 + 256) / 256)), dim3(256), 0, st, x, bias, res, C, hw, total, slope);
    HIP_TRY(ctx, hipGetLastError());
    return VIDO_OK;
}

int vido_nchw_to_nhwc(vido_ctx* ctx, const float* src, int B, int C, int H, int W, float* dst)
{
    if (!ctx) return VIDO_E_INVALID;
    if (!src || !dst || B < 1 || C < 1 || H < 1 || W < 1 || B > 65535) return vido_set_error(ctx, VIDO_E_INVALID, "nchw_to_nhwc: bad arguments");
    HIP_TRY(ctx, hipSetDevice(ctx->device));
    hipStream_t st = ctx->has_ext_stream ? ctx->ext_stream : ctx->stream;
    hipLaunchKernelGGL(k_nchw_to_nhwc, dim3((H * W + 63) / 64, (C + 63) / 64, B), dim3(256), 0, st, src, C, H * W, dst);
    HIP_TRY(ctx, hipGetLastError());
    return VIDO_OK;
}

int vido_roi_align(vido_ctx* ctx, const float* feat, int B, int C, int H, int W, const float* rois, int n_rois, float spatial_scale,
                   int pooled_h, int pooled_w, int sampling_ratio, float* out, int on_device)
{
    if (!ctx) return VIDO_E_INVALID;
    if (!feat || (n_rois && (!rois || !out)) || B < 1 || C < 1 || H < 1 || W < 1 || n_rois < 0 || pooled_h < 1 || pooled_w < 1) return vido_set_error(ctx, VIDO_E_INVALID, "roi_align: bad arguments");
    if (n_rois == 0) return VIDO_OK;
    HIP_TRY(ctx, hipSetDevice(ctx->device));
    hipStream_t st = (on_device && ctx->has_ext_stream) ? ctx->ext_stream : ctx->stream;
    const size_t nf = (size_t)B * C * H * W * 4, nr = (size_t)n_rois * 5 * 4, nout = (size_t)n_rois * C * pooled_h * pooled_w * 4;
    const float *df = feat, *dr = rois; float* dout = out; NetState* S = nullptr;
    const size_t base = on_device ? 0 : al256(nf) + al256(nr) + al256(nout);
    { int rc = net_scratch(ctx, base + al256(nf), &S); if (rc) return rc; }
    if (!on_device) {
        for (int i = 0; i < n_rois; i++) if (!(rois[5 * i] >= 0 && rois[5 * i] < B)) return vido_set_error(ctx, VIDO_E_INVALID, "roi_align: roi %d has batch index %g", i, rois[5 * i]);
        memcpy(S->h, feat, nf); memcpy(S->h + al256(nf), rois, nr);
        HIP_TRY(ctx, hipMemcpyAsync(S->d, S->h, al256(nf) + al256(nr), hipMemcpyHostToDevice, st));
        df = (float*)S->d; dr = (float*)(S->d + al256(nf)); dout = (float*)(S->d + al256(nf) + al256(nr));
    }
    float* nhwc = (float*)(S->d + base);
    hipLaunchKernelGGL(k_nchw_to_nhwc, dim3((H * W + 63) / 64, (C + 63) / 64, B), dim3(256), 0, st, df, C, H * W, nhwc);
    RoiLevels L{}; L.feat[0] = nhwc; L.H[0] = H; L.W[0] = W; L.scale[0] = spatial_scale;
    const size_t lds = (size_t)64 * ((pooled_h * pooled_w) | 1) * sizeof(float);
    if (lds > 150 * 1024) return vido_set_error(ctx, VIDO_E_CAPACITY, "roi_align: pooled size %d x %d too large", pooled_h, pooled_w);
    { int rc = roi_lds_limit(ctx, lds); if (rc) return rc; }
    if (sampling_ratio == 2) hipLaunchKernelGGL(k_roi_align_nhwc<2>, dim3(n_rois, (C + 63) / 64), dim3(256), lds, st, L, C, dr, 5, (const int*)nullptr, pooled_h, pooled_w, sampling_ratio, dout);
    else hipLaunchKernelGGL(k_roi_align_nhwc<0>, dim3(n_rois, (C + 63) / 64), dim3(256), lds, st, L, C, dr, 5, (const int*)nullptr, pooled_h, pooled_w, sampling_ratio, dout);
    HIP_TRY(ctx, hipGetLastError());
    if (!on_device) {
        HIP_TRY(ctx, hipStreamSynchronize(st));
        HIP_TRY(ctx, hipMemcpyAsync(S->h, dout, nout, hipMemcpyDeviceToHost, st)); HIP_TRY(ctx, hipStreamSynchronize(st));
        memcpy(out, S->h, nout);
    }
    return VIDO_OK;
}

static int nms_impl(vido_ctx* ctx, const float* boxes_xyxy, const float* scores, const int32_t* groups, int n, float thresh, int32_t* keep_out, int32_t* n_keep, int on_device)
{
    if (!ctx) return VIDO_E_INVALID;
    if (n < 0 || !n_keep || (n && (!boxes_xyxy || !keep_out)) || (!on_device && n && !scores)) return vido_set_error(ctx, VIDO_E_INVALID, "nms: bad arguments");
    if (n > 65536) return vido_set_error(ctx, VIDO_E_CAPACITY, "nms: %d boxes > 65536", n);
    HIP_TRY(ctx, hipSetDevice(ctx->device));
    hipStream_t st = (on_device && ctx->has_ext_stream) ? ctx->ext_stream : ctx->stream;
    if (n == 0) { if (on_device) HIP_TRY(ctx, hipMemsetAsync(n_keep, 0, 4, st)); else *n_keep = 0; return VIDO_OK; }
    const int cb = (n + 63) / 64;
    const size_t nb = (size_t)n * 16, nm = (size_t)n * cb * 8, nk = (size_t)n * 4 + 256, ng = (size_t)n * 4;
    NetState* S = nullptr;
    int rc = net_scratch(ctx, al256(nb) + al256(nm) + al256(nk) + al256(ng), &S); if (rc) return rc;
    const int* dgroups = groups;
    const float* dboxes = boxes_xyxy; unsigned long long* dmask = (unsigned long long*)(S->d + al256(nb));
    int* dkeep = keep_out; int* dn = n_keep;
    std::vector<int> order;
    if (!on_device) {
        order.resize(n); std::iota(order.begin(), order.end(), 0);
        std::stable_sort(order.begin(), order.end(), [&](int a, int b) { return scores[a] > scores[b]; });
        float* hb = (float*)S->h;
        for (int i = 0; i < n; i++) memcpy(hb + 4 * (size_t)i, boxes_xyxy + 4 * (size_t)order[i], 16);
        HIP_TRY(ctx, hipMemcpyAsync(S->d, S->h, nb, hipMemcpyHostToDevice, st));
        dboxes = (float*)S->d; dkeep = (int*)(S->d + al256(nb) + al256(nm)); dn = dkeep + n;
        if (groups) {
            int* hg = (int*)(S->h + al256(nb)); for (int i = 0; i < n; i++) hg[i] = groups[order[i]];
            int* dg = (int*)(S->d + al256(nb) + al256(nm) + al256(nk));
            HIP_TRY(ctx, hipMemcpyAsync(dg, hg, ng, hipMemcpyHostToDevice, st)); dgroups = dg;
        }
    }
    hipLaunchKernelGGL(k_nms_mask, dim3((cb * (cb + 1) / 2 + 3) / 4), dim3(256), 0, st, dboxes, dgroups, n, thresh, dmask, cb);
    hipLaunchKernelGGL(k_nms_sweep, dim3(1), dim3(64), 0, st, dmask, n, cb, dkeep, dn);
    HIP_TRY(ctx, hipGetLastError());
    if (!on_device) {
        HIP_TRY(ctx, hipStreamSynchronize(st));
        HIP_TRY(ctx, hipMemcpyAsync(S->h, dkeep, nk, hipMemcpyDeviceToHost, st)); HIP_TRY(ctx, hipStreamSynchronize(st));
        const int* hk = (const int*)S->h; const int m = hk[n];
        for (int i = 0; i < m; i++) keep_out[i] = order[hk[i]];
        std::sort(keep_out, keep_out + m);
        *n_keep = m;
    }
    return VIDO_OK;
}

int vido_nms(vido_ctx* ctx, const float* boxes_xyxy, const float* scores, int n, float thresh, int32_t* keep_out, int32_t* n_keep, int on_device)
{
    return nms_impl(ctx, boxes_xyxy, scores, nullptr, n, thresh, keep_out, n_keep, on_device);
}
int vido_nms_grouped(vido_ctx* ctx, const float* boxes_xyxy, const float* scores, const int32_t* groups, int n, float thresh,
                     int32_t* keep_out, int32_t* n_keep, int on_device)
{
    if (n > 0 && !groups) return ctx ? vido_set_error(ctx, VIDO_E_INVALID, "nms_grouped: null groups") : VIDO_E_INVALID;
    return nms_impl(ctx, boxes_xyxy, scores, groups, n, thresh, keep_out, n_keep, on_device);
}

int vido_nms_segments(vido_ctx* ctx, const float* boxes_xyxy, const int32_t* groups, const int32_t* seg_off, const int32_t* seg_n, int n_seg, int max_n, int total,
                      float thresh, int32_t* keep_out, int32_t* n_keep)
{
    if (!ctx) return VIDO_E_INVALID;
    if (!boxes_xyxy || !seg_off || !seg_n || !keep_out || !n_keep || n_seg < 1 || max_n < 1 || total < 1) return vido_set_error(ctx, VIDO_E_INVALID, "nms_segments: bad arguments");
    if (max_n > 65536) return vido_set_error(ctx, VIDO_E_CAPACITY, "nms_segments: %d boxes per segment > 65536", max_n);
    HIP_TRY(ctx, hipSetDevice(ctx->device));
    hipStream_t st = ctx->has_ext_stream ? ctx->ext_stream : ctx->stream;
    const int cb = (max_n + 63) / 64;
    NetState* S = nullptr;
    int rc = net_scratch(ctx, al256((size_t)total * cb * 8), &S); if (rc) return rc;
    unsigned long long* dmask = (unsigned long long*)S->d;
    hipLaunchKernelGGL(k_nms_mask_seg, dim3((cb * (cb + 1) / 2 + 3) / 4, n_seg), dim3(256), 0, st, boxes_xyxy, groups, seg_off, seg_n, thresh, dmask, cb);
    hipLaunchKernelGGL(k_nms_sweep_seg, dim3(n_seg), dim3(64), 0, st, dmask, seg_off, seg_n, cb, keep_out, n_keep, max_n);
    HIP_TRY(ctx, hipGetLastError());
    return VIDO_OK;
}

int vido_roi_align_fpn(vido_ctx* ctx, const float* const feat[4], const int H[4], const int W[4], const float scale[4], int C, const float* boxes, const int32_t* level,
                       int n, int pooled_h, int pooled_w, int sampling_ratio, float* out)
{
    if (!ctx) return VIDO_E_INVALID;
    if (!feat || !H || !W || !scale || C < 1 || n < 0 || pooled_h < 1 || pooled_w < 1 || (n && (!boxes || !level || !out))) return vido_set_error(ctx, VIDO_E_INVALID, "roi_align_fpn: bad arguments");
    if (n == 0) return VIDO_OK;
    HIP_TRY(ctx, hipSetDevice(ctx->device));
    hipStream_t st = ctx->has_ext_stream ? ctx->ext_stream : ctx->stream;
    size_t off[5] = {0, 0, 0, 0, 0};
    for (int l = 0; l < 4; l++) off[l + 1] = off[l] + al256((size_t)C * H[l] * W[l] * 4);
    NetState* S = nullptr;
    { int rc = net_scratch(ctx, off[4], &S); if (rc) return rc; }
    const float* nh[4];
    for (int l = 0; l < 4; l++) {
        hipLaunchKernelGGL(k_nchw_to_nhwc, dim3((H[l] * W[l] + 63) / 64, (C + 63) / 64, 1), dim3(256), 0, st, feat[l], C, H[l] * W[l], (float*)(S->d + off[l]));
        nh[l] = (const float*)(S->d + off[l]);
    }
    return vido_roi_align_fpn_nhwc(ctx, nh, H, W, scale, C, boxes, level, n, pooled_h, pooled_w, sampling_ratio, out);
}

int vido_roi_align_fpn_nhwc(vido_ctx* ctx, const float* const feat[4], const int H[4], const int W[4], const float scale[4], int C, const float* boxes, const int32_t* level,
                            int n, int pooled_h, int pooled_w, int sampling_ratio, float* out)
{
    if (!ctx) return VIDO_E_INVALID;
    if (!feat || !H || !W || !scale || C < 1 || n < 0 || pooled_h < 1 || pooled_w < 1 || (n && (!boxes || !level || !out))) return vido_set_error(ctx, VIDO_E_INVALID, "roi_align_fpn_nhwc: bad arguments");
    if (n == 0) return VIDO_OK;
    HIP_TRY(ctx, hipSetDevice(ctx->device));
    hipStream_t st = ctx->has_ext_stream ? ctx->ext_stream : ctx->stream;
    RoiLevels L;
    for (int l = 0; l < 4; l++) { L.feat[l] = feat[l]; L.H[l] = H[l]; L.W[l] = W[l]; L.scale[l] = scale[l]; }
    const size_t lds = (size_t)64 * ((pooled_h * pooled_w) | 1) * sizeof(float);
    if (lds > 150 * 1024) return vido_set_error(ctx, VIDO_E_CAPACITY, "roi_align_fpn: pooled size %d x %d too large", pooled_h, pooled_w);
    { int rc = roi_lds_limit(ctx, lds); if (rc) return rc; }
    if (sampling_ratio == 2) hipLaunchKernelGGL(k_roi_align_nhwc<2>, dim3(n, (C + 63) / 64), dim3(256), lds, st, L, C, boxes, 4, level, pooled_h, pooled_w, sampling_ratio, out);
    else hipLaunchKernelGGL(k_roi_align_nhwc<0>, dim3(n, (C + 63) / 64), dim3(256), lds, st, L, C, boxes, 4, level, pooled_h, pooled_w, sampling_ratio, out);
    HIP_TRY(ctx, hipGetLastError());
    return VIDO_OK;
}

int vido_mask_label_image(vido_ctx* ctx, const float* masks, const float* boxes, const int64_t* labels, int n, int M, int padding, float thresh, int H, int W, uint8_t* out)
{
    if (!ctx) return VIDO_E_INVALID;
    if (!out || H < 1 || W < 1 || n < 0 || M < 1 || padding < 0 || (n && (!masks || !boxes || !labels))) return vido_set_error(ctx, VIDO_E_INVALID, "mask_label_image: bad arguments");
    HIP_TRY(ctx, hipSetDevice(ctx->device));
    hipStream_t st = ctx->has_ext_stream ? ctx->ext_stream : ctx->stream;
    if (n == 0) { HIP_TRY(ctx, hipMemsetAsync(out, 0, (size_t)H * W, st)); return VIDO_OK; }
    NetState* S = nullptr;
    int rc = net_scratch(ctx, al256((size_t)n * sizeof(PasteDet)), &S); if (rc) return rc;
    PasteDet* det = (PasteDet*)S->d;
    hipLaunchKernelGGL(k_paste_prepare, dim3((n + 255) / 256), dim3(256), 0, st, boxes, labels, n, M, padding, det);
    hipLaunchKernelGGL(k_paste_label, dim3((W + 31) / 32, (H + 7) / 8), dim3(256), 0, st, masks, det, n, M, padding, thresh, H, W, out);
    HIP_TRY(ctx, hipGetLastError());
    return VIDO_OK;
}

int vido_mask_instance_image(vido_ctx* ctx, const float* masks, const float* boxes, const int64_t* labels, int n, int M, int padding, float thresh, int H, int W,
                             const int32_t* id_base_dev, uint8_t* out, int32_t* area_out)
{
    if (!ctx) return VIDO_E_INVALID;
    if (!out || H < 1 || W < 1 || n < 0 || M < 1 || padding < 0 || (n && (!masks || !boxes || !labels))) return vido_set_error(ctx, VIDO_E_INVALID, "mask_instance_image: bad arguments");
    if (n > 255) return vido_set_error(ctx, VIDO_E_CAPACITY, "mask_instance_image: %d detections, ids are u8 (n + id_base <= 255)", n);
    HIP_TRY(ctx, hipSetDevice(ctx->device));
    hipStream_t st = ctx->has_ext_stream ? ctx->ext_stream : ctx->stream;
    PasteDet* det = nullptr;
    if (n) {
        NetState* S = nullptr;
        int rc = net_scratch(ctx, al256((size_t)n * sizeof(PasteDet)), &S); if (rc) return rc;
        det = (PasteDet*)S->d;
        if (area_out) hipLaunchKernelGGL(k_zero_i32, dim3((n + 255) / 256), dim3(256), 0, st, area_out, n);
        hipLaunchKernelGGL(k_paste_prepare, dim3((n + 255) / 256), dim3(256), 0, st, boxes, labels, n, M, padding, det);
    }
    hipLaunchKernelGGL(k_paste_instance, dim3((W + 31) / 32, (H + 7) / 8), dim3(256), 0, st, masks, det, n, M, padding, thresh, H, W, id_base_dev, out, area_out);
    HIP_TRY(ctx, hipGetLastError());
    return VIDO_OK;
}

int vido_box_decode(vido_ctx* ctx, const float* deltas, const float* boxes, int n, int k, const float weights[4], float* out, int on_device)
{
    if (!ctx) return VIDO_E_INVALID;
    if (n < 0 || k < 1 || !weights || (n && (!deltas || !boxes || !out))) return vido_set_error(ctx, VIDO_E_INVALID, "box_decode: bad arguments");
    if (n == 0) return VIDO_OK;
    HIP_TRY(ctx, hipSetDevice(ctx->device));
    hipStream_t st = (on_device && ctx->has_ext_stream) ? ctx->ext_stream : ctx->stream;
    const size_t nd = (size_t)n * k * 16, nb = (size_t)n * 16;
    const float *dd = deltas, *db = boxes; float* dout = out; NetState* S = nullptr;
    if (!on_device) {
        int rc = net_scratch(ctx, 2 * al256(nd) + al256(nb), &S); if (rc) return rc;
        memcpy(S->h, deltas, nd); memcpy(S->h + al256(nd), boxes, nb);
// ... 15 lines not shown
```

vido-slam_amd/nets/maskrcnn.py:

```python
import math
import os
from collections import OrderedDict
from dataclasses import dataclass
import numpy as np
import torch
import torch.nn as nn
import torch.nn.functional as F


@dataclass
class MaskRCNNConfig:
    blocks: tuple = (3, 4, 23, 3)
    groups: int = 32
    width_per_group: int = 8
    stride_in_1x1: bool = False
    stem_out: int = 64
    res2_out: int = 256
    fpn_out: int = 256
    anchor_sizes: tuple = (32, 64, 128, 256, 512)
    aspect_ratios: tuple = (0.5, 1.0, 2.0)
    anchor_strides: tuple = (4, 8, 16, 32, 64)
    pre_nms_top_n: int = 1000
    post_nms_top_n: int = 1000
    fpn_post_nms_top_n: int = 1000
# ... 164 lines not shown
    rows = [[xc - 0.5 * (a * s - 1), yc - 0.5 * (b * s - 1), xc + 0.5 * (a * s - 1), yc + 0.5 * (b * s - 1)] for a, b in zip(ws, hs)]
    return torch.from_numpy(np.asarray(rows, np.float64)).float()


class _Buffers(nn.Module):
    def __init__(self, tensors):
        super().__init__()
        for i, t in enumerate(tensors):
            self.register_buffer(str(i), t)

    def __iter__(self):
        return iter(self._buffers.values())


class _AnchorGenerator(nn.Module):
    def __init__(self, c):
        super().__init__()
        self.strides = c.anchor_strides
        self.cell_anchors = _Buffers([cell_anchors(st, sz, c.aspect_ratios) for st, sz in zip(c.anchor_strides, c.anchor_sizes)])

    def forward(self, grid_sizes):
        out = []
        for (gh, gw), stride, base in zip(grid_sizes, self.strides, self.cell_anchors):
            sx = torch.arange(0, gw * stride, step=stride, dtype=torch.float32, device=base.device)
            sy = torch.arange(0, gh * stride, step=stride, dtype=torch.float32, device=base.device)
            yy, xx = torch.meshgrid(sy, sx, indexing="ij")
            shifts = torch.stack((xx.reshape(-1), yy.reshape(-1), xx.reshape(-1), yy.reshape(-1)), 1)
            out.append((shifts.view(-1, 1, 4) + base.view(1, -1, 4)).reshape(-1, 4))
        return out


class _RPNHead(nn.Module):
    def __init__(self, ch, na):
        super().__init__()
        self.conv = nn.Conv2d(ch, ch, 3, 1, 1); self.cls_logits = nn.Conv2d(ch, na, 1); self.bbox_pred = nn.Conv2d(ch, na * 4, 1)

    _ops = None

    def forward(self, feats):
        t = [_conv_bias_relu(self.conv, f, self._ops) for f in feats]
        ops = self._ops
        if ops is not None and t[0].is_cuda and hasattr(ops, "conv1x1_skinny") and not os.environ.get("VIDO_NO_CONVSMALL") and t[0].shape[0] == 1 and self.conv.out_channels % 2 == 0 and self.conv.out_channels <= 256:
            from .ops import pack_conv1x1_skinny
            key = (self.cls_logits.weight.data_ptr(), self.cls_logits.weight._version, self.bbox_pred.weight.data_ptr(), self.bbox_pred.weight._version, str(t[0].device))
            if getattr(self, "_head_key", None) != key:
                self._head_w = pack_conv1x1_skinny(torch.cat([self.cls_logits.weight, self.bbox_pred.weight], 0)).to(t[0].device)
                self._head_b = torch.cat([self.cls_logits.bias, self.bbox_pred.bias], 0).detach().contiguous(); self._head_key = key
            na = self.cls_logits.out_channels; nt = na + self.bbox_pred.out_channels
            ys = [ops.conv1x1_skinny(x, self._head_w, self._head_b, nt, 1.0) for x in t]
            return [y[:, :na] for y in ys], [y[:, na:] for y in ys]
        return [self.cls_logits(x) for x in t], [self.bbox_pred(x) for x in t]


def _conv_bias_relu(conv, x, ops):
    if ops is None or not x.is_cuda or conv.bias is None:
        return F.relu(conv(x))
    if isinstance(conv, nn.Conv2d) and hasattr(ops, "wino3x3_conv") and not os.environ.get("VIDO_NO_WINO"):
        y = ops.wino3x3_conv(conv, x, 0.0)
        if y is not None:
            return y
    if isinstance(conv, nn.ConvTranspose2d) and hasattr(ops, "deconv2x2_conv"):
        y = ops.deconv2x2_conv(conv, x, 0.0)
        if y is not None:
            return y
    if isinstance(conv, nn.ConvTranspose2d):
        y = F.conv_transpose2d(x, conv.weight, None, conv.stride, conv.padding, conv.output_padding, conv.groups, conv.dilation)
    else:
        y = F.conv2d(x, conv.weight, None, conv.stride, conv.padding, conv.dilation, conv.groups)
    return ops.bias_act_(y.contiguous(), conv.bias, 0.0)


def clip_boxes(b, w, h):
    b = b.clone()
    b[:, 0::2] = b[:, 0::2].clamp(min=0, max=w - 1); b[:, 1::2] = b[:, 1::2].clamp(min=0, max=h - 1)
    return b


def _topk_stable(v, k):
    s, idx = torch.sort(v, descending=True, stable=True)
    return s[:k], idx[:k]


class _RPN(nn.Module):
    def __init__(self, c, ops):
        super().__init__()
        self.c, self.ops = c, ops
        self.anchor_generator = _AnchorGenerator(c)
        self.head = _RPNHead(c.fpn_out, len(c.aspect_ratios))

    def forward(self, feats, image_wh):
        logits, deltas = self.head(feats)
        return self.proposals(feats, logits, deltas, image_wh)

    def proposals(self, feats, logits, deltas, image_wh):
        if hasattr(self.ops, "nms_segments") and logits[0].is_cuda and self.c.rpn_min_size <= 0:
            return self.proposals_device(feats, logits, deltas, image_wh)
        c = self.c; W, H = image_wh
        anchors = self.anchor_generator([f.shape[-2:] for f in feats])
        boxes, scores = [], []
        for a, lo, de in zip(anchors, logits, deltas):
            A, h, w = lo.shape[1:]
            obj = lo[0].permute(1, 2, 0).reshape(-1).sigmoid()
            reg = de[0].view(A, 4, h, w).permute(2, 3, 0, 1).reshape(-1, 4)
            k = min(c.pre_nms_top_n, obj.numel())
            obj, idx = _topk_stable(obj, k)
            prop = clip_boxes(self.ops.box_decode(reg[idx], a[idx], (1.0, 1.0, 1.0, 1.0)), W, H)
            keep = ((prop[:, 2] - prop[:, 0] + 1 >= c.rpn_min_size) & (prop[:, 3] - prop[:, 1] + 1 >= c.rpn_min_size)).nonzero().squeeze(1)
            prop, obj = prop[keep], obj[keep]
            keep = self.ops.nms(prop, obj, c.rpn_nms)[: c.post_nms_top_n]
            boxes.append(prop[keep]); scores.append(obj[keep])
        boxes, scores = torch.cat(boxes), torch.cat(scores)
        k = min(c.fpn_post_nms_top_n, scores.numel())
        _, idx = _topk_stable(scores, k)
        return boxes[idx], scores[idx]

# ... 9 lines not shown
        reg = de[0].view(A, 4, h, w).permute(2, 3, 0, 1).reshape(-1, 4)
        k = min(K, obj.numel())
        obj, idx = _topk_stable(obj, k)
        prop = clip_boxes(self.ops.box_decode(reg[idx], a[idx], (1.0, 1.0, 1.0, 1.0)), W, H)
        if k < K:
            prop = torch.cat([prop, prop.new_zeros((K - k, 4))]); obj = torch.cat([obj, obj.new_full((K - k,), -1.0)])
        props.append(prop); objs.append(obj); ns.append(k)
    L = len(props)
    boxes = torch.cat(props); scores = torch.cat(objs)
    dev = boxes.device
    key = (L, K, tuple(ns), str(dev))
    if getattr(self, "_seg_key", None) != key:
        self._seg_off = torch.arange(L, device=dev, dtype=torch.int32) * K; self._seg_n = torch.tensor(ns, device=dev, dtype=torch.int32); self._seg_key = key
        self._pos = torch.arange(K, device=dev, dtype=torch.int32).unsqueeze(0).expand(L, K)
    keep, cnt = self.ops.nms_segments(boxes, self._seg_off, self._seg_n, K, c.rpn_nms)
    kept = torch.zeros((L, K + 1), dtype=torch.bool, device=dev)
    kept.scatter_(1, torch.where(keep >= 0, keep, torch.full_like(keep, K)).long(), True)
    kept = kept[:, :K]
    if c.post_nms_top_n < K:
        kept &= (kept.cumsum(1) <= c.post_nms_top_n)
    scores = torch.where(kept.reshape(-1), scores, scores.new_full((), -1.0))
    k = min(c.fpn_post_nms_top_n, scores.numel())
    top, idx = _topk_stable(scores, k)
    valid = top >= 0
    return torch.where(valid.unsqueeze(1), boxes[idx], boxes.new_zeros(())), top


_RPN.proposals_device = _rpn_proposals_device


def _rpn_proposals_fused(self, feats, logits, deltas, image_wh):
    c = self.c; W, H = image_wh; K = c.pre_nms_top_n; L = len(logits); dev = logits[0].device
    boxes, scores, n = self.ops.rpn_select(logits, deltas, list(self.anchor_generator.cell_anchors), self.anchor_generator.strides, K, (W, H))
    if getattr(self, "_fseg_key", None) != (L, K, str(dev)):
        self._fseg_off = torch.arange(L, device=dev, dtype=torch.int32) * K; self._fseg_key = (L, K, str(dev))
    keep, cnt = self.ops.nms_segments(boxes, self._fseg_off, n, K, c.rpn_nms)
    props, obj, _ = self.ops.rpn_merge(boxes, scores, keep, cnt, K, c.post_nms_top_n, min(c.fpn_post_nms_top_n, L * K))
    return props, obj


_RPN.proposals_fused = _rpn_proposals_fused


class FpnMaps(tuple):
    nhwc = ()


class _Pooler(nn.Module):
    def __init__(self, resolution, scales, sampling_ratio, ops):
        super().__init__()
        self.res, self.scales, self.sr, self.ops = resolution, scales, sampling_ratio, ops
        self.k_min = -math.log2(scales[0]); self.k_max = -math.log2(scales[-1])

    def forward(self, feats, boxes):
        if boxes.is_cuda and boxes.dtype == torch.float32 and hasattr(self.ops, "roi_levels") and not os.environ.get("VIDO_NO_ROI_LEVELS"):
            lvl = self.ops.roi_levels(boxes, self.k_min, self.k_max)
        else:
            area = (boxes[:, 2] - boxes[:, 0] + 1) * (boxes[:, 3] - boxes[:, 1] + 1)
            lvl = torch.floor(4 + torch.log2(torch.sqrt(area) / 224 + 1e-6)).clamp(min=self.k_min, max=self.k_max).to(torch.int64) - int(self.k_min)
        if isinstance(feats, FpnMaps):
            return self.ops.roi_align_fpn_nhwc(feats.nhwc, boxes, lvl, (self.res, self.res), self.scales, self.sr)
        if hasattr(self.ops, "roi_align_fpn") and boxes.is_cuda and len(feats) == 4:
            return self.ops.roi_align_fpn(feats, boxes, lvl, (self.res, self.res), self.scales, self.sr)
        rois = torch.cat([boxes.new_zeros((len(boxes), 1)), boxes], 1)
        out = feats[0].new_zeros((len(boxes), feats[0].shape[1], self.res, self.res))
        for l, (f, s) in enumerate(zip(feats, self.scales)):
            idx = torch.nonzero(lvl == l).squeeze(1)
            if idx.numel():
                out[idx] = self.ops.roi_align(f, rois[idx], (self.res, self.res), s, self.sr)
        return out


class _BoxFeatures(nn.Module):
    def __init__(self, c, ops):
        super().__init__()
        self.pooler = _Pooler(c.box_resolution, c.pool_scales, c.sampling_ratio, ops)
        self.fc6 = nn.Linear(c.fpn_out * c.box_resolution ** 2, c.mlp_dim); self.fc7 = nn.Linear(c.mlp_dim, c.mlp_dim)

    def forward(self, feats, boxes):
        x = self.pooler(feats, boxes).flatten(1)
        ops = self.pooler.ops
        use = ops is not None and hasattr(ops, "fc_h_linear") and x.shape[0] >= 128
        y = ops.fc_h_linear(self.fc6, x, 0.0) if use else None
        if y is None:
            y = F.relu(self.fc6(x))
        z = ops.fc_h_linear(self.fc7, y, 0.0) if use else None
        return z if z is not None else F.relu(self.fc7(y))


class _BoxPredictor(nn.Module):
    def __init__(self, c):
        super().__init__()
        self.cls_score = nn.Linear(c.mlp_dim, c.num_classes); self.bbox_pred = nn.Linear(c.mlp_dim, c.num_classes * 4)

    def forward(self, x):
        return self.cls_score(x), self.bbox_pred(x)


class _BoxHead(nn.Module):
    def __init__(self, c, ops):
        super().__init__()
        self.c, self.ops = c, ops
        self.feature_extractor = _BoxFeatures(c, ops); self.predictor = _BoxPredictor(c)

    def forward(self, feats, proposals, image_wh, objectness=None):
        logits, deltas = self.predictor(self.feature_extractor(feats, proposals))
        return self.postprocess(logits, deltas, proposals, image_wh, objectness)

    def postprocess(self, logits, deltas, proposals, image_wh, objectness=None):
        c = self.c; W, H = image_wh; nc = logits.shape[1]
        prob = F.softmax(logits, -1)
        if objectness is not None and objectness.is_cuda:
            prob = prob * (objectness >= 0).unsqueeze(1)
        boxes = clip_boxes(self.ops.box_decode(deltas, proposals, c.bbox_reg_weights).reshape(-1, 4), W, H).reshape(-1, nc * 4)
# ... 26 lines not shown
    bx_sorted = torch.gather(bx_cls, 1, order.unsqueeze(-1).expand(-1, -1, 4)).reshape(-1, 4)
    st = getattr(self, "_static_tabs", None)
    if st is None or st[0] != (nc, N, str(dev)):
        st = ((nc, N, str(dev)), torch.arange(nc - 1, device=dev, dtype=torch.int32) * N,
              (torch.arange(1, nc, device=dev, dtype=torch.int64).unsqueeze(1).expand(nc - 1, N)).reshape(-1).contiguous())
        self._static_tabs = st
    seg_off, lab_grid = st[1], st[2]
    seg_n = valid.sum(1).to(torch.int32)
    keep, _ = self.ops.nms_segments(bx_sorted, seg_off, seg_n, N, c.nms)
    kept_sorted = torch.zeros((nc - 1, N + 1), dtype=torch.bool, device=dev)
    kept_sorted.scatter_(1, torch.where(keep >= 0, keep, torch.full_like(keep, N)).long(), True)
    Fk = torch.zeros((nc - 1, N), dtype=torch.bool, device=dev).scatter_(1, order, kept_sorted[:, :N])
    Sc = torch.where(Fk, S, S.new_full((), -1.0)).reshape(-1)
    n_keep = Fk.sum()
    if c.detections_per_img > 0:
        top = torch.sort(Sc, descending=True)[0]
        th = torch.where(n_keep > c.detections_per_img, top[c.detections_per_img - 1], top.new_full((), -0.5))
        Fk = Fk & (Sc.reshape(nc - 1, N) >= th)
    flat = Fk.reshape(-1)
    pos = torch.cumsum(flat, 0) - 1
    n_det = flat.sum()
    dst = torch.where(flat & (pos < cap), pos, torch.full_like(pos, cap))
    ob = boxes.new_zeros((cap + 1, 4)).index_copy_(0, dst, bx_cls.reshape(-1, 4))
    osc = boxes.new_zeros((cap + 1,)).index_copy_(0, dst, S.reshape(-1))
    olb = torch.zeros((cap + 1,), dtype=torch.int64, device=dev).index_copy_(0, dst, lab_grid)
    return ob[:cap], osc[:cap], olb[:cap], n_det


_BoxHead.postprocess_static = _postprocess_static


def _postprocess_fused(self, logits, deltas, proposals, image_wh, objectness, cap):
    c = self.c; W, H = image_wh; nc = logits.shape[1]; N = logits.shape[0]; dev = logits.device
    prob = F.softmax(logits, -1)
    seg, order, seg_n = self.ops.det_class_sort(prob, deltas, proposals, objectness, c.score_thresh, c.bbox_reg_weights, (W, H))
    if getattr(self, "_fseg_key", None) != (nc, N, str(dev)):
        self._fseg_off = torch.arange(nc - 1, device=dev, dtype=torch.int32) * N; self._fseg_key = (nc, N, str(dev))
    keep, cnt = self.ops.nms_segments(seg, self._fseg_off, seg_n, N, c.nms)
    ob, osc, ol, nd = self.ops.det_select(prob, seg, order, keep, cnt, c.detections_per_img, cap)
    return ob, osc, ol, nd[0]


_BoxHead.postprocess_fused = _postprocess_fused


class _MaskFeatures(nn.Module):
    def __init__(self, c, ops):
        super().__init__()
        self.pooler = _Pooler(c.mask_resolution, c.pool_scales, c.sampling_ratio, ops)
        cin = c.fpn_out; self.names = []
        for i, ch in enumerate(c.mask_layers, 1):
            setattr(self, "mask_fcn%d" % i, nn.Conv2d(cin, ch, 3, 1, 1)); self.names.append("mask_fcn%d" % i); cin = ch

    def forward(self, feats, boxes):
        x = self.pooler(feats, boxes)
        for n in self.names:
            x = _conv_bias_relu(getattr(self, n), x, self.pooler.ops if hasattr(self.pooler.ops, "bias_act_") else None)
        return x


class _MaskPredictor(nn.Module):
    def __init__(self, c):
        super().__init__()
        self.conv5_mask = nn.ConvTranspose2d(c.mask_layers[-1], c.mask_layers[-1], 2, 2, 0)
        self.mask_fcn_logits = nn.Conv2d(c.mask_layers[-1], c.num_classes, 1)

    _ops = None

    def forward(self, x):
        return self.mask_fcn_logits(_conv_bias_relu(self.conv5_mask, x, self._ops))

    def selected(self, x, labels):
        y = _conv_bias_relu(self.conv5_mask, x, self._ops)
        if self._ops is not None and y.is_cuda and hasattr(self._ops, "mask_logit_select") and not os.environ.get("VIDO_NO_MASK_SELECT") and labels.dtype == torch.int64:
            return self._ops.mask_logit_select(y.contiguous(), self.mask_fcn_logits, labels.contiguous())
        return self.mask_fcn_logits(y).sigmoid()[torch.arange(x.shape[0], device=labels.device), labels][:, None]


class _MaskHead(nn.Module):
    buckets = (4, 8, 16, 32, 64, 100)

    def __init__(self, c, ops):
        super().__init__()
        self.feature_extractor = _MaskFeatures(c, ops); self.predictor = _MaskPredictor(c)

    def forward(self, feats, boxes, labels):
        if not len(boxes):
            return feats[0].new_zeros((0, 1, 2 * self.feature_extractor.pooler.res, 2 * self.feature_extractor.pooler.res))
        n = len(boxes); self.last_n = n
        idx = torch.arange(n, device=labels.device)
        if not (boxes.is_cuda and self.buckets):
            return self.predictor(self.feature_extractor(feats, boxes)).sigmoid()[idx, labels][:, None]
        out = []; big = self.buckets[-1]
        for a in range(0, n, big):
            bx, lb = boxes[a:a + big], labels[a:a + big]; k = len(bx)
            m = next(b for b in self.buckets if b >= k)
            if m > k:
                bx = torch.cat([bx, bx.new_zeros((m - k, 4))]); lb = torch.cat([lb, lb.new_zeros((m - k,))])
            g = self.graphed.get(m) if self.graphed and feats[0].data_ptr() == self._graph_feat_ptr else None
            logits = g(bx) if g is not None else self.chunk_logits(feats, bx)
            out.append(logits.sigmoid()[torch.arange(m, device=lb.device), lb][:k, None])
        return torch.cat(out)

    graphed = None; _graph_feat_ptr = 0; last_n = 0

    def chunk_logits(self, feats, bx):
        return self.predictor(self.feature_extractor(feats, bx))

    def capture_buckets(self, feats, graphed_cls):
        feats = list(feats)
        self.graphed = {}
        for b in self.buckets:
            ex = torch.tensor([[10.0, 10.0, 200.0, 300.0]], device=feats[0].device).repeat(b, 1)
            self.graphed[b] = graphed_cls(lambda bx, _f=feats: self.chunk_logits(_f, bx), [ex])
        self._graph_feat_ptr = feats[0].data_ptr()


class _RoiHeads(nn.Module):
    def __init__(self, c, ops):
        super().__init__()
        self.box = _BoxHead(c, ops); self.mask = _MaskHead(c, ops)


def paste_masks(masks, boxes, im_h, im_w, thresh=0.5, padding=1):
    n, M = masks.shape[0], masks.shape[-1]
    out = torch.zeros((n, im_h, im_w), dtype=torch.bool, device=masks.device)
    if n == 0:
        return out
# ... 4 lines not shown
    xc, yc = (b[:, 2] + b[:, 0]) * 0.5, (b[:, 3] + b[:, 1]) * 0.5
    ib = torch.stack([xc - wh, yc - hh, xc + wh, yc + hh], 1).to(torch.int32).cpu().tolist()
    for i, (x0, y0, x1, y1) in enumerate(ib):
        w, h = max(x1 - x0 + 1, 1), max(y1 - y0 + 1, 1)
        m = F.interpolate(padded[i:i + 1], size=(h, w), mode="bilinear", align_corners=False)[0, 0] > thresh
        xa, xb, ya, yb = max(x0, 0), min(x1 + 1, im_w), max(y0, 0), min(y1 + 1, im_h)
        if xb > xa and yb > ya:
            out[i, ya:yb, xa:xb] = m[ya - y0:yb - y0, xa - x0:xb - x0]
    return out


class MaskRCNN(nn.Module):

    def __init__(self, ops, config=None):
        super().__init__()
        self.config = c = config or MaskRCNNConfig()
        self.backbone = nn.Sequential(OrderedDict([("body", _Body(c)), ("fpn", _FPN(c))]))
        self.rpn = _RPN(c, ops)
        self.roi_heads = _RoiHeads(c, ops)
        for m in self.modules():
            if isinstance(m, (_RPNHead, _MaskPredictor, _FPN)):
                m._ops = ops if hasattr(ops, "bias_act_") else None

    @torch.no_grad()
    def forward(self, image):
        feats, logits, deltas = self.trunk(image)
        return self.heads(feats, logits, deltas, image.shape[-2:])

    @torch.no_grad()
    def trunk(self, image):
        feats = self.backbone(image)
        logits, deltas = self.rpn.head(feats)
        return feats, logits, deltas

    @torch.no_grad()
    def heads(self, feats, logits, deltas, image_hw):
        H, W = image_hw
        proposals, objectness = self.rpn.proposals(feats, logits, deltas, (W, H))
        maps = self.fpn_maps(feats)
        boxes, scores, labels = self.roi_heads.box(maps, proposals, (W, H), objectness)
        masks = self.roi_heads.mask(maps, boxes, labels)
        return dict(boxes=boxes, scores=scores, labels=labels, masks=masks, proposals=proposals, objectness=objectness, n_proposals=(objectness >= 0).sum())


def _fpn_maps(self, feats):
    ops = self.rpn.ops; lv = tuple(feats[:len(self.config.pool_scales)])
    if not (hasattr(ops, "to_nhwc") and lv[0].is_cuda and len(lv) == 4):
        return lv
    m = FpnMaps(lv); m.nhwc = tuple(ops.to_nhwc(f) for f in lv)
    return m


@torch.no_grad()
def _heads_static(self, feats, logits, deltas, image_hw, cap=None):
    H, W = image_hw; c = self.config; cap = cap or c.detections_per_img
    fused = self.fused_post and hasattr(self.rpn.ops, "det_select") and c.pre_nms_top_n <= 1024 and c.rpn_min_size <= 0
    proposals, objectness = (self.rpn.proposals_fused if fused else self.rpn.proposals_device)(feats, logits, deltas, (W, H))
    maps = self.fpn_maps(feats)
    bh = self.roi_heads.box
    lg, dl = bh.predictor(bh.feature_extractor(maps, proposals))
    boxes, scores, labels, n_det = (bh.postprocess_fused if fused else bh.postprocess_static)(lg, dl, proposals, (W, H), objectness, cap)
    mh = self.roi_heads.mask
    masks = mh.predictor.selected(mh.feature_extractor(maps, boxes), labels)
    return dict(boxes=boxes, scores=scores, labels=labels, masks=masks, n_det=n_det, proposals=proposals, objectness=objectness, n_proposals=(objectness >= 0).sum())


MaskRCNN.fused_post = True
MaskRCNN.fpn_maps = _fpn_maps
MaskRCNN.heads_static = _heads_static


LABEL_MODES = ("class", "instance")


def _check_label_mode(label_mode):
    if label_mode not in LABEL_MODES:
        raise ValueError("label_mode: one of %s, not %r" % (LABEL_MODES, label_mode))


def label_image_torch(masks, boxes, scores, labels, H, W, confidence=0.8, label_mode="class", id_base=0, max_instances=None):
    _check_label_mode(label_mode)
    keep = torch.nonzero(scores > confidence).squeeze(1)
    keep = keep[scores[keep].sort(0, descending=True)[1]]
    if label_mode == "instance" and max_instances is not None:
        keep = keep[:max_instances]
    labels = labels[keep]
    n = int(keep.numel())
    if n == 0:
        return torch.zeros((H, W), dtype=torch.uint8, device=masks.device), labels
    pasted = paste_masks(masks[keep], boxes[keep], H, W)
    if label_mode == "class":
        return (pasted.to(torch.int32) * labels.view(-1, 1, 1).to(torch.int32)).sum(0).remainder(256).to(torch.uint8), labels
    if not torch.is_tensor(id_base) and n + int(id_base) > 255:
        raise ValueError("label_mode='instance': %d detections above id base %d, ids are u8 (n + id_base <= 255)" % (n, id_base))
    slot = torch.arange(1, n + 1, dtype=torch.int32, device=masks.device).view(-1, 1, 1)
    first = torch.where(pasted & (labels != 0).view(-1, 1, 1), slot, slot.new_full((), n + 1)).min(0)[0]
    base = id_base.reshape(()).to(torch.int32) if torch.is_tensor(id_base) else int(id_base)
    return torch.where(first <= n, first + base, torch.zeros_like(first)).to(torch.uint8), labels


@torch.no_grad()
def analyse_image_static(net, feats, logits, deltas, out_hw, feed=(1088, 800), confidence=0.8, cap=None, label_mode="class", id_base=None):
    _check_label_mode(label_mode)
    H, W = out_hw
    out = net.heads_static(feats, logits, deltas, feed, cap)
    cap = out["boxes"].shape[0]
    rw, rh = float(W) / feed[1], float(H) / feed[0]
    cache = net.__dict__.setdefault("_const_cache", {})
    key = ("box_scale", rw, rh, str(out["boxes"].device))
    if key not in cache:
        cache[key] = out["boxes"].new_tensor([rw, rh, rw, rh])
    boxes = out["boxes"] * cache[key]
    ops = net.rpn.ops
    nd = out["n_det"]
    if hasattr(ops, "det_order") and cap <= 1024 and nd.dtype == torch.int32 and out["labels"].dtype == torch.int64 and not os.environ.get("VIDO_NO_DET_ORDER"):
        order, labels, n_live = ops.det_order(out["scores"].contiguous(), out["labels"].contiguous(), nd.reshape(1), confidence)
    else:
        live = (out["scores"] > confidence) & (torch.arange(cap, device=boxes.device) < nd)
        order = torch.sort(torch.where(live, out["scores"], out["scores"].new_full((), -1.0)), descending=True, stable=True)[1]
        labels = torch.where(live, out["labels"], torch.zeros_like(out["labels"]))[order]
        n_live = live.sum()
    if label_mode == "instance":
        if cap > 255:
            raise ValueError("label_mode='instance': %d slots, ids are u8" % cap)
        img = ops.mask_instance_image(out["masks"][order], boxes[order], labels, H, W, id_base=id_base)
    else:
        img = ops.mask_label_image(out["masks"][order], boxes[order], labels, H, W)
    return img, labels, n_live, out["n_det"]


def image_to_feed(bgr, dev, feed=(1088, 800), ops=None):
    if ops is not None and torch.is_tensor(bgr) and bgr.is_cuda and bgr.dtype == torch.uint8:
        return ops.area_feed(bgr.contiguous(), feed)
    t = (bgr.to(dev).flip(-1) if torch.is_tensor(bgr) else torch.as_tensor(bgr[:, :, ::-1].copy(), device=dev)).permute(2, 0, 1).float().unsqueeze(0)
    return F.interpolate(t, size=feed, mode="area")


@torch.no_grad()
def analyse_image(net, bgr, feed=(1088, 800), confidence=0.8, trunk=None, on_range=None, label_mode="class", id_base=None, max_instances=None):
    _check_label_mode(label_mode)
    if on_range is not None:
        from .ops import range_checked
        return range_checked(lambda safe: analyse_image(net, bgr, feed, confidence, None if safe else trunk, None, label_mode, id_base, max_instances), (net,), on_range, "the detector")
    dev = next(net.parameters()).device
    H, W = bgr.shape[:2]
    if trunk is not None:
        feats, logits, deltas = trunk(bgr)
        out = net.heads(feats, logits, deltas, feed)
    else:
        out = net(image_to_feed(bgr, dev, feed))
    rw, rh = float(W) / feed[1], float(H) / feed[0]
    boxes = out["boxes"] * out["boxes"].new_tensor([rw, rh, rw, rh]) if rw != rh else out["boxes"] * rw
    ops = getattr(net.rpn, "ops", None)
    if hasattr(ops, "mask_label_image") and out["masks"].is_cuda:
        keep = torch.nonzero(out["scores"] > confidence).squeeze(1)
        keep = keep[out["scores"][keep].sort(0, descending=True)[1]]
        if label_mode == "instance" and max_instances is not None:
            keep = keep[:max_instances]
        labels = out["labels"][keep]
        if label_mode == "instance":
            return ops.mask_instance_image(out["masks"][keep], boxes[keep], labels, H, W, id_base=id_base), labels
        return ops.mask_label_image(out["masks"][keep], boxes[keep], labels, H, W), labels
    return label_image_torch(out["masks"], boxes, out["scores"], out["labels"], H, W, confidence, label_mode, 0 if id_base is None else id_base, max_instances)
```

vido-slam_amd/nets/ops.py:

```python
import contextlib
import ctypes as C
import os
import torch

_WINO_MIN_WGS = int(os.environ.get("VIDO_WINO_MIN_WGS", "0"))
_CONV3X3_H_MIN_WGS = 0 if os.environ.get("VIDO_CONV3X3_H") == "0" else int(os.environ.get("VIDO_CONV3X3_H_MIN_WGS", "128"))
_CONVDIRECT_SET = os.environ.get("VIDO_CONVDIRECT_SET", "novalu")


def correlation_torch_reference(first, second, stride):
    a, b = first[:, :, ::stride, ::stride], second[:, :, ::stride, ::stride]
    pad = torch.nn.functional.pad(b, (3, 3, 3, 3))
    H, W = a.shape[2], a.shape[3]
    return torch.stack([(a * pad[:, :, p:p + H, o:o + W]).mean(1) for p in range(7) for o in range(7)], 1)


class HipOps:

    _range_safe = 0

    def __init__(self, ctx):
        self.ctx = ctx

    @property
    def range_safe_active(self):
        return self._range_safe > 0

    def _adopt_stream(self):
        st = torch.cuda.current_stream().cuda_stream
        self.ctx._check(self.ctx.lib.vido_set_stream(self.ctx.h, C.c_void_p(st), 1))

    def correlation(self, first, second, stride):
        if not first.is_cuda:
            raise RuntimeError("HipOps.correlation needs CUDA(HIP) tensors; there is no CPU fallback")
        first = first.contiguous().float(); second = second.contiguous().float()
        B, Cc, H, W = first.shape
        out = torch.empty((B, 49, (H + stride - 1) // stride, (W + stride - 1) // stride), device=first.device, dtype=torch.float32)
        self._adopt_stream()
        self.ctx._check(self.ctx.lib.vido_correlation(self.ctx.h, C.c_void_p(first.data_ptr()), C.c_void_p(second.data_ptr()), B, Cc, H, W, stride,
                                                      C.c_void_p(out.data_ptr()), 1))
        return out

    def bias_act_(self, x, bias, slope):
        assert x.is_cuda and x.is_contiguous() and x.dtype == torch.float32
        N, Cc, H, W = x.shape
        self._adopt_stream()
        self.ctx._check(self.ctx.lib.vido_bias_act(self.ctx.h, C.c_void_p(x.data_ptr()), C.c_void_p(bias.data_ptr()), N, Cc, H, W, C.c_float(slope)))
        return x

    def deconv2x2_conv(self, conv, x, slope):
        w = conv.weight
        if (tuple(w.shape[2:]) != (2, 2) or tuple(conv.stride) != (2, 2) or tuple(conv.padding) != (0, 0) or tuple(conv.output_padding) != (0, 0) or tuple(conv.dilation) != (1, 1)
                or conv.groups != 1 or not x.is_cuda or x.dtype != torch.float32 or os.environ.get("VIDO_NO_DECONV_H") or self._range_safe):
            return None
        n, cin, H, W = (int(v) for v in x.shape); cout = int(w.shape[1])
        if not self.ctx.lib.vido_deconv2x2_supported(n, cin, cout, H, W):
            return None
        key = (w.data_ptr(), w._version, str(x.device))
        if getattr(conv, "_dc_key", None) != key:
            conv._dc_w = pack_deconv2x2(w).to(x.device); conv._dc_key = key
        out = torch.empty((n, cout, 2 * H, 2 * W), device=x.device, dtype=torch.float32)
        self.gconv_flops = getattr(self, "gconv_flops", 0.0) + 2.0 * n * cin * cout * 4 * H * W
        self._adopt_stream()
        b = conv.bias
        self.ctx._check(self.ctx.lib.vido_deconv2x2_bias_act(self.ctx.h, C.c_void_p(x.contiguous().data_ptr()), C.c_void_p(conv._dc_w.data_ptr()), C.c_void_p(b.data_ptr()) if b is not None else None,
                                                             C.c_void_p(out.data_ptr()), n, cin, cout, H, W, C.c_float(slope)))
        return out

    def det_order(self, scores, labels, n_det, confidence):
        assert scores.is_cuda and scores.dtype == torch.float32 and labels.dtype == torch.int64 and n_det.dtype == torch.int32 and scores.is_contiguous() and labels.is_contiguous()
        cap = int(scores.shape[0]); dev = scores.device
        order = torch.empty((cap,), device=dev, dtype=torch.int64); lab = torch.empty((cap,), device=dev, dtype=torch.int64); n_live = torch.empty((), device=dev, dtype=torch.int64)
        self._adopt_stream()
        self.ctx._check(self.ctx.lib.vido_det_order(self.ctx.h, C.c_void_p(scores.data_ptr()), C.c_void_p(labels.data_ptr()), C.c_void_p(n_det.data_ptr()), C.c_float(confidence), cap,
                                                    C.c_void_p(order.data_ptr()), C.c_void_p(lab.data_ptr()), C.c_void_p(n_live.data_ptr())))
        return order, lab, n_live

    def roi_levels(self, boxes, k_min, k_max):
        assert boxes.is_cuda and boxes.dtype == torch.float32
        boxes = boxes.contiguous(); n = int(boxes.shape[0])
        out = torch.empty((n,), device=boxes.device, dtype=torch.int32)
        self._adopt_stream()
        self.ctx._check(self.ctx.lib.vido_roi_levels(self.ctx.h, C.c_void_p(boxes.data_ptr()), n, C.c_float(k_min), C.c_float(k_max), C.c_void_p(out.data_ptr())))
        return out

    def mask_logit_select(self, feat, conv, labels):
        assert feat.is_cuda and feat.is_contiguous() and feat.dtype == torch.float32 and labels.dtype == torch.int64 and labels.is_contiguous()
        n, c, H, W = feat.shape; classes = int(conv.weight.shape[0])
        w = conv.weight.reshape(classes, c)
        if not w.is_contiguous():
            w = w.contiguous()
        out = torch.empty((n, 1, H, W), device=feat.device, dtype=torch.float32)
        self._adopt_stream()
        self.ctx._check(self.ctx.lib.vido_mask_logit_select(self.ctx.h, C.c_void_p(feat.data_ptr()), C.c_void_p(w.data_ptr()), C.c_void_p(conv.bias.data_ptr()) if conv.bias is not None else None,
                                                            C.c_void_p(labels.data_ptr()), C.c_void_p(out.data_ptr()), int(n), int(c), int(H * W), classes))
        return out

    def bias_res_act_(self, x, bias, res, slope):
        assert x.is_cuda and x.is_contiguous() and x.dtype == torch.float32
        N, Cc, H, W = x.shape
        if res is not None:
            assert res.shape == x.shape and res.is_contiguous() and res.dtype == torch.float32
        self._adopt_stream()
        self.ctx._check(self.ctx.lib.vido_bias_res_act(self.ctx.h, C.c_void_p(x.data_ptr()), C.c_void_p(bias.data_ptr()),
                                                       C.c_void_p(res.data_ptr()) if res is not None else None, N, Cc, H, W, C.c_float(slope)))
        return x

    def bias_unary_(self, x, bias, kind):
        assert x.is_cuda and x.is_contiguous() and x.dtype == torch.float32
        N, Cc, H, W = x.shape
        self._adopt_stream()
        self.ctx._check(self.ctx.lib.vido_bias_unary(self.ctx.h, C.c_void_p(x.data_ptr()), C.c_void_p(bias.data_ptr()), N, Cc, H, W, 1 if kind == "elu" else 2))
        return x

    def upcat_reflect(self, x, skip=None):
        assert x.is_cuda and x.is_contiguous() and x.dtype == torch.float32 and x.shape[0] == 1
        _, C1, h, w = x.shape
        C2 = 0
        if skip is not None:
            assert skip.is_contiguous() and skip.shape[0] == 1 and tuple(skip.shape[2:]) == (2 * h, 2 * w)
            C2 = skip.shape[1]
        out = torch.empty((1, C1 + C2, 2 * h + 2, 2 * w + 2), device=x.device, dtype=torch.float32)
        self._adopt_stream()
        self.ctx._check(self.ctx.lib.vido_upcat_reflect(self.ctx.h, C.c_void_p(x.data_ptr()), C.c_void_p(skip.data_ptr()) if skip is not None else None, C1, C2, h, w, C.c_void_p(out.data_ptr())))
        return out

    def minmax_norm_u16(self, d):
        d = d.contiguous()
        mm = torch.stack(torch.aminmax(d))
        out = torch.empty(d.shape, device=d.device, dtype=torch.int32)
        self._adopt_stream()
        self.ctx._check(self.ctx.lib.vido_minmax_norm_u16(self.ctx.h, C.c_void_p(d.data_ptr()), C.c_void_p(mm.data_ptr()), C.c_int64(d.numel()), C.c_void_p(out.data_ptr())))
        return out

    def area_feed(self, bgr, feed, div=1.0):
        assert bgr.is_cuda and bgr.dtype == torch.uint8 and bgr.is_contiguous() and bgr.dim() == 3 and bgr.shape[2] == 3
        out = torch.empty((1, 3, int(feed[0]), int(feed[1])), device=bgr.device, dtype=torch.float32)
        self._adopt_stream()
        self.ctx._check(self.ctx.lib.vido_area_feed(self.ctx.h, C.c_void_p(bgr.data_ptr()), bgr.shape[0], bgr.shape[1], C.c_void_p(out.data_ptr()), int(feed[0]), int(feed[1]), C.c_float(div)))
        return out

    def backwarp(self, x, flow):
        assert x.is_cuda and x.dtype == torch.float32 and flow.dtype == torch.float32 and x.shape[0] == flow.shape[0] and x.shape[2:] == flow.shape[2:] and flow.shape[1] == 2
        x = x.contiguous(); flow = flow.contiguous()
        out = torch.empty_like(x)
        self._adopt_stream()
        self.ctx._check(self.ctx.lib.vido_backwarp(self.ctx.h, C.c_void_p(x.data_ptr()), C.c_void_p(flow.data_ptr()), x.shape[0], x.shape[1], x.shape[2], x.shape[3], C.c_void_p(out.data_ptr())))
        return out
# ... 98 lines not shown
        if (w.shape[0] != 2 or w.shape[2] != w.shape[3] or k not in (3, 5, 7) or tuple(conv.stride) != (1, 1) or tuple(conv.padding) != (k // 2, k // 2) or tuple(conv.dilation) != (1, 1)
                or conv.groups != 1 or not x.is_cuda or x.shape[0] != 1 or x.dtype != torch.float32):
            return None
        x = x.contiguous(); wc = w.contiguous()
        _, cin, H, W = x.shape
        out = torch.empty((1, 2, H, W), device=x.device, dtype=torch.float32)
        if residual is not None:
            residual = residual.contiguous(); assert residual.shape == out.shape
        self.gconv_flops = getattr(self, "gconv_flops", 0.0) + 2.0 * 2 * cin * k * k * H * W
        self._adopt_stream()
        self.ctx._check(self.ctx.lib.vido_conv_kxk_c2(self.ctx.h, C.c_void_p(x.data_ptr()), C.c_void_p(wc.data_ptr()), C.c_void_p(conv.bias.data_ptr()) if conv.bias is not None else None,
                                                      C.c_void_p(residual.data_ptr()) if residual is not None else None, C.c_void_p(out.data_ptr()), int(cin), k, int(H), int(W)))
        return out

    def conv1x1_skinny(self, x, w_packed, bias, cout, slope=1.0, residual=None):
        assert x.is_cuda and x.dtype == torch.float32 and x.shape[0] == 1
        x = x.contiguous(); cin, H, W = int(x.shape[1]), int(x.shape[2]), int(x.shape[3])
        out = torch.empty((1, cout, H, W), device=x.device, dtype=torch.float32)
        if residual is not None:
            residual = residual.contiguous(); assert residual.shape == out.shape
        self.gconv_flops = getattr(self, "gconv_flops", 0.0) + 2.0 * cout * cin * H * W
        self._adopt_stream()
        self.ctx._check(self.ctx.lib.vido_conv1x1_skinny(self.ctx.h, C.c_void_p(x.data_ptr()), C.c_void_p(w_packed.data_ptr()), C.c_void_p(bias.data_ptr()) if bias is not None else None,
                                                         C.c_void_p(residual.data_ptr()) if residual is not None else None, C.c_void_p(out.data_ptr()), cin, int(cout), C.c_longlong(H * W), C.c_float(slope)))
        return out

    def conv1x1_skinny_conv(self, conv, x, slope=1.0):
        w = conv.weight
        cout, cin = int(w.shape[0]), int(w.shape[1])
        if (tuple(w.shape[2:]) != (1, 1) or tuple(conv.stride) != (1, 1) or tuple(conv.padding) != (0, 0) or conv.groups != 1 or cin % 2 or cin > 256 or cout > 256
                or not x.is_cuda or x.shape[0] != 1 or x.dtype != torch.float32):
            return None
        key = (w.data_ptr(), w._version, str(x.device))
        if getattr(conv, "_c1s_key", None) != key:
            conv._c1s_w = pack_conv1x1_skinny(w).to(x.device); conv._c1s_key = key
        return self.conv1x1_skinny(x, conv._c1s_w, conv.bias, cout, slope)

    def wino3x3_supported(self, cin, cout, H, W):
        return bool(self.ctx.lib.vido_wino3x3_supported(int(cin), int(cout), int(H), int(W)))

    def wino3x3_form(self, N, cin, cout, H, W):
        return int(self.ctx.lib.vido_wino3x3_form(int(N), int(cin), int(cout), int(H), int(W)))

    def wino3x3_bias_act(self, x, u_packed, bias, cout, slope=1.0, form=0):
        assert x.is_cuda and x.is_contiguous() and x.dtype == torch.float32 and u_packed.is_cuda
        N, cin, H, W = x.shape
        out = torch.empty((N, cout, H, W), device=x.device, dtype=torch.float32)
        self.gconv_flops = getattr(self, "gconv_flops", 0.0) + 2.0 * N * cout * cin * 9 * H * W
        self._adopt_stream()
        self.ctx._check(self.ctx.lib.vido_wino3x3_bias_act_form(self.ctx.h, C.c_void_p(x.data_ptr()), C.c_void_p(u_packed.data_ptr()), C.c_void_p(bias.data_ptr()) if bias is not None else None,
                                                                C.c_void_p(out.data_ptr()), int(N), int(cin), int(cout), int(H), int(W), C.c_float(slope), int(form)))
        return out

    def wino3x3_conv(self, conv, x, slope, weight=None, bias=None):
        w = conv.weight if weight is None else weight
        b = conv.bias if bias is None and weight is None else bias
        if (tuple(w.shape[2:]) != (3, 3) or tuple(conv.stride) != (1, 1) or tuple(conv.padding) != (1, 1) or tuple(conv.dilation) != (1, 1) or conv.groups != 1
                or getattr(conv, "padding_mode", "zeros") != "zeros" or not x.is_cuda or not self.wino3x3_supported(w.shape[1], w.shape[0], x.shape[2], x.shape[3])
                or 4 * x.numel() >= 1 << 30 or 4 * x.shape[0] * w.shape[0] * x.shape[2] * x.shape[3] >= 1 << 30):
            return None
        if _WINO_MIN_WGS > 0 and not self.ctx.lib.vido_wino3x3_fills_chip(int(x.shape[0]), int(w.shape[0]), int(x.shape[2]), int(x.shape[3]), _WINO_MIN_WGS):
            return None
        if (_CONV3X3_H_MIN_WGS > 0 and x.dtype == torch.float32 and not self._range_safe and self.ctx.lib.vido_conv3x3_h_supported(int(x.shape[0]), int(w.shape[1]), int(w.shape[0]), int(x.shape[2]), int(x.shape[3]))
                and self.ctx.lib.vido_conv3x3_h_workgroups(int(x.shape[0]), int(w.shape[0]), int(x.shape[2]), int(x.shape[3])) >= (1 if int(w.shape[0]) == 64 else _CONV3X3_H_MIN_WGS)):
            key = (w.data_ptr(), w._version, str(x.device))
            if getattr(conv, "_c3h_key", None) != key:
                conv._c3h_w = pack_conv3x3_h(w).to(x.device); conv._c3h_key = key
            return self.conv3x3_h_bias_act(x.contiguous(), conv._c3h_w, b, int(w.shape[0]), slope)
        form = self.wino3x3_form(x.shape[0], w.shape[1], w.shape[0], x.shape[2], x.shape[3])
        key = (w.data_ptr(), w._version, str(x.device))
        if getattr(conv, "_wino_key", None) != key:
            conv._wino_u = {}; conv._wino_key = key
        if form not in conv._wino_u:
            conv._wino_u[form] = pack_wino3x3(w, form).to(x.device)
        return self.wino3x3_bias_act(x.contiguous(), conv._wino_u[form], b, int(w.shape[0]), slope, form)

    def conv3x3_h_bias_act(self, x, w_packed, bias, cout, slope):
        assert x.is_cuda and x.is_contiguous() and x.dtype == torch.float32
        N, cin, H, W = x.shape
        assert w_packed.dtype == torch.int16 and w_packed.numel() == 2 * cout * ((cin + 15) // 16 * 16 * 9 + 1), "conv3x3_h: weight not packed by pack_conv3x3_h for this layer"
        out = torch.empty((N, cout, H, W), device=x.device, dtype=torch.float32)
        self.gconv_flops = getattr(self, "gconv_flops", 0.0) + 2.0 * N * cout * cin * 9 * H * W
        self._adopt_stream()
        self.ctx._check(self.ctx.lib.vido_conv3x3_h_bias_act(self.ctx.h, C.c_void_p(x.data_ptr()), C.c_void_p(w_packed.data_ptr()), C.c_void_p(bias.data_ptr()) if bias is not None else None,
                                                             C.c_void_p(out.data_ptr()), int(N), int(cin), int(cout), int(H), int(W), C.c_float(slope)))
        return out

    def fc_h(self, x, w_packed, bias, outs, slope=1.0):
        assert x.is_cuda and x.is_contiguous() and x.dtype == torch.float32 and x.dim() == 2
        rows, k = int(x.shape[0]), int(x.shape[1])
        S = int(self.ctx.lib.vido_fc_h_splitk(rows, k, int(outs)))
        if S <= 0:
            return None
        assert w_packed.dtype == torch.int16 and w_packed.numel() == 2 * outs * (k + 1), "fc_h: weight not packed (pack_conv1x1(w[:, :, None, None], 3))"
        part = torch.empty((S, rows, outs), device=x.device, dtype=torch.float32); y = torch.empty((rows, outs), device=x.device, dtype=torch.float32)
        self.gconv_flops = getattr(self, "gconv_flops", 0.0) + 2.0 * rows * k * outs
        self._adopt_stream()
        self.ctx._check(self.ctx.lib.vido_fc_h(self.ctx.h, C.c_void_p(x.data_ptr()), C.c_void_p(w_packed.data_ptr()), C.c_void_p(bias.data_ptr()) if bias is not None else None,
                                               C.c_void_p(part.data_ptr()), C.c_void_p(y.data_ptr()), rows, k, int(outs), C.c_float(slope)))
        return y

    def fc_h_linear(self, lin, x, slope=1.0):
        w = lin.weight
        if not x.is_cuda or x.dtype != torch.float32 or x.dim() != 2 or os.environ.get("VIDO_NO_FC_H") or self._range_safe or int(self.ctx.lib.vido_fc_h_splitk(int(x.shape[0]), int(w.shape[1]), int(w.shape[0]))) <= 0:
            return None
        key = (w.data_ptr(), w._version, str(x.device))
        if getattr(lin, "_fch_key", None) != key:
            lin._fch_w = pack_conv1x1(w.detach().reshape(int(w.shape[0]), int(w.shape[1]), 1, 1), 3).to(x.device); lin._fch_key = key
        return self.fc_h(x.contiguous(), lin._fch_w, lin.bias, int(w.shape[0]), slope)

    def conv_direct_conv(self, conv, x, slope):
        w = conv.weight
        kh, kw = int(w.shape[2]), int(w.shape[3]); sh, sw = (int(v) for v in conv.stride); ph, pw = (int(v) for v in conv.padding)
        if _CONVDIRECT_SET == "novalu" and (kh, kw) in ((3, 3), (7, 7)) and int(w.shape[0]) >= 32:
            return None
        if (tuple(conv.dilation) != (1, 1) or conv.groups != 1 or getattr(conv, "padding_mode", "zeros") != "zeros" or not x.is_cuda or x.dtype != torch.float32
                or not self.ctx.lib.vido_conv_direct_supported(int(w.shape[1]), int(w.shape[0]), int(x.shape[2]), int(x.shape[3]), kh, kw, sh, sw, ph, pw)
                or 4 * x.numel() >= 1 << 30):
            return None
        N, cin, H, W = x.shape; cout = int(w.shape[0])
        Ho, Wo = (H + 2 * ph - kh) // sh + 1, (W + 2 * pw - kw) // sw + 1
        if 4 * N * cout * Ho * Wo >= 1 << 30:
            return None
        key = (w.data_ptr(), w._version, str(x.device))
        if getattr(conv, "_cd_key", None) != key:
            conv._cd_w = pack_conv_direct(w).to(x.device); conv._cd_key = key
        x = x.contiguous()
        out = torch.empty((N, cout, Ho, Wo), device=x.device, dtype=torch.float32)
        self.gconv_flops = getattr(self, "gconv_flops", 0.0) + 2.0 * N * cout * cin * kh * kw * Ho * Wo
        self._adopt_stream()
        b = conv.bias
        self.ctx._check(self.ctx.lib.vido_conv_direct_bias_act(self.ctx.h, C.c_void_p(x.data_ptr()), C.c_void_p(conv._cd_w.data_ptr()), C.c_void_p(b.data_ptr()) if b is not None else None,
                                                               C.c_void_p(out.data_ptr()), int(N), int(cin), cout, int(H), int(W), kh, kw, sh, sw, ph, pw, C.c_float(slope)))
        return out

    def lfn_reg_front(self, im1, im2, flow, scale, feat):
        im1 = im1.contiguous(); im2 = im2.contiguous(); flow = flow.contiguous()
        B, Cc, H, W = im1.shape
# ... 95 lines not shown
        return out

    def rpn_select(self, logits, deltas, cell_anchors, strides, K, image_wh):
        L = len(logits); A = logits[0].shape[1]; dev = logits[0].device
        logits = [t.contiguous() for t in logits]; deltas = [t.contiguous() for t in deltas]
        boxes = torch.empty((L * K, 4), device=dev, dtype=torch.float32); scores = torch.empty((L * K,), device=dev, dtype=torch.float32); n = torch.empty((L,), device=dev, dtype=torch.int32)
        lp = (C.c_void_p * L)(*[t.data_ptr() for t in logits]); dp = (C.c_void_p * L)(*[t.data_ptr() for t in deltas])
        hs = (C.c_int * L)(*[t.shape[2] for t in logits]); ws = (C.c_int * L)(*[t.shape[3] for t in logits]); st = (C.c_int * L)(*[int(s) for s in strides])
        key = ("anch", L, A)
        if getattr(self, "_anch_key", None) != key:
            self._anch = (C.c_float * (L * A * 4))(*[float(v) for a in cell_anchors for v in a.detach().cpu().reshape(-1).tolist()]); self._anch_key = key
        self._adopt_stream()
        self.ctx._check(self.ctx.lib.vido_rpn_select(self.ctx.h, L, lp, dp, hs, ws, st, self._anch, A, int(K), int(image_wh[0]), int(image_wh[1]),
                                                     C.c_void_p(boxes.data_ptr()), C.c_void_p(scores.data_ptr()), C.c_void_p(n.data_ptr())))
        return boxes, scores, n

    def rpn_merge(self, boxes, scores, keep, cnt, K, post_nms_top_n, n_final):
        L = cnt.shape[0]; dev = boxes.device
        ob = torch.empty((n_final, 4), device=dev, dtype=torch.float32); osc = torch.empty((n_final,), device=dev, dtype=torch.float32); nv = torch.empty((1,), device=dev, dtype=torch.int32)
        self._adopt_stream()
        self.ctx._check(self.ctx.lib.vido_rpn_merge(self.ctx.h, C.c_void_p(boxes.data_ptr()), C.c_void_p(scores.data_ptr()), C.c_void_p(keep.data_ptr()), C.c_void_p(cnt.data_ptr()),
                                                    L, int(K), int(post_nms_top_n), int(n_final), C.c_void_p(ob.data_ptr()), C.c_void_p(osc.data_ptr()), C.c_void_p(nv.data_ptr())))
        return ob, osc, nv

    def det_class_sort(self, prob, deltas, proposals, objectness, thresh, weights, image_wh):
        prob = prob.contiguous(); deltas = deltas.contiguous(); proposals = proposals.contiguous()
        N, nc = prob.shape; dev = prob.device
        seg = torch.empty(((nc - 1) * N, 4), device=dev, dtype=torch.float32); order = torch.empty((nc - 1, N), device=dev, dtype=torch.int32); seg_n = torch.empty((nc - 1,), device=dev, dtype=torch.int32)
        wv = (C.c_float * 4)(*[float(x) for x in weights])
        self._adopt_stream()
        self.ctx._check(self.ctx.lib.vido_det_class_sort(self.ctx.h, C.c_void_p(prob.data_ptr()), C.c_void_p(deltas.data_ptr()), C.c_void_p(proposals.data_ptr()),
                                                         C.c_void_p(objectness.data_ptr()) if objectness is not None else None, N, nc, C.c_float(thresh), wv, int(image_wh[0]), int(image_wh[1]),
                                                         C.c_void_p(seg.data_ptr()), C.c_void_p(order.data_ptr()), C.c_void_p(seg_n.data_ptr())))
        return seg, order, seg_n

    def det_select(self, prob, seg_boxes, order, keep, cnt, detections_per_img, cap):
        N, nc = prob.shape; dev = prob.device
        ob = torch.empty((cap, 4), device=dev, dtype=torch.float32); osc = torch.empty((cap,), device=dev, dtype=torch.float32); ol = torch.empty((cap,), device=dev, dtype=torch.int64)
        nd = torch.empty((1,), device=dev, dtype=torch.int32); scratch = torch.empty((nc + 3,), device=dev, dtype=torch.int32)
        self._adopt_stream()
        self.ctx._check(self.ctx.lib.vido_det_select(self.ctx.h, C.c_void_p(prob.data_ptr()), C.c_void_p(seg_boxes.data_ptr()), C.c_void_p(order.data_ptr()), C.c_void_p(keep.data_ptr()),
                                                     C.c_void_p(cnt.data_ptr()), N, nc, int(detections_per_img), int(cap), C.c_void_p(scratch.data_ptr()),
                                                     C.c_void_p(ob.data_ptr()), C.c_void_p(osc.data_ptr()), C.c_void_p(ol.data_ptr()), C.c_void_p(nd.data_ptr())))
        return ob, osc, ol, nd

    def to_nhwc(self, x):
        assert x.is_cuda and x.dtype == torch.float32 and x.dim() == 4
        x = x.contiguous(); B, Cc, H, W = x.shape
        out = torch.empty((B, H, W, Cc), device=x.device, dtype=torch.float32)
        self._adopt_stream()
        self.ctx._check(self.ctx.lib.vido_nchw_to_nhwc(self.ctx.h, C.c_void_p(x.data_ptr()), B, Cc, H, W, C.c_void_p(out.data_ptr())))
        return out

    def roi_align_fpn_nhwc(self, feats_nhwc, boxes, level, output_size, scales, sampling_ratio):
        n = boxes.shape[0]; ph, pw = output_size; Cc = feats_nhwc[0].shape[3]
        out = torch.empty((n, Cc, ph, pw), device=boxes.device, dtype=torch.float32)
        if n == 0:
            return out
        boxes = boxes.contiguous().float(); level = level.to(torch.int32).contiguous()
        fp = (C.c_void_p * 4)(*[f.data_ptr() for f in feats_nhwc]); Hs = (C.c_int * 4)(*[f.shape[1] for f in feats_nhwc]); Ws = (C.c_int * 4)(*[f.shape[2] for f in feats_nhwc])
        sc = (C.c_float * 4)(*[float(x) for x in scales])
        self._adopt_stream()
        self.ctx._check(self.ctx.lib.vido_roi_align_fpn_nhwc(self.ctx.h, fp, Hs, Ws, sc, Cc, C.c_void_p(boxes.data_ptr()), C.c_void_p(level.data_ptr()), n, ph, pw, sampling_ratio,
                                                             C.c_void_p(out.data_ptr())))
        return out

    def mask_label_image(self, masks, boxes, labels, H, W, thresh=0.5, padding=1):
        out = torch.empty((H, W), device=masks.device, dtype=torch.uint8)
        n = masks.shape[0]
        masks = masks.contiguous().float(); boxes = boxes.contiguous().float(); labels = labels.contiguous().to(torch.int64)
        self._adopt_stream()
        self.ctx._check(self.ctx.lib.vido_mask_label_image(self.ctx.h, C.c_void_p(masks.data_ptr()) if n else None, C.c_void_p(boxes.data_ptr()) if n else None,
                                                           C.c_void_p(labels.data_ptr()) if n else None, n, masks.shape[-1] if n else 28, padding, C.c_float(thresh), H, W,
                                                           C.c_void_p(out.data_ptr())))
        return out

    def mask_propagate(self, mask, flow, depth=None, out=None, stats=None):
        from ..host import VidoError
        def bad(why):
            raise VidoError(-1, "mask_propagate: " + why)
        for name, t, dt in (("mask", mask, torch.int32), ("flow", flow, torch.float32), ("depth", depth, torch.float32), ("out", out, torch.int32), ("stats", stats, torch.int32)):
            if t is None:
                continue
            if not torch.is_tensor(t) or not t.is_cuda:
                bad("%s must be a device tensor; there is no CPU fallback" % name)
            if t.dtype != dt:
                bad("%s must be %s, got %s" % (name, dt, t.dtype))
            if not t.is_contiguous():
                bad("%s must be contiguous" % name)
            if t.device != mask.device:
                bad("%s is on another device than mask" % name)
        if mask.dim() != 2:
            bad("mask must be [H, W]")
        H, W = int(mask.shape[0]), int(mask.shape[1])
        if tuple(flow.shape) != (H, W, 2):
            bad("flow must be [%d, %d, 2], got %s" % (H, W, tuple(flow.shape)))
        if depth is not None and tuple(depth.shape) != (H, W):
            bad("depth must be [%d, %d], got %s" % (H, W, tuple(depth.shape)))
        if out is None:
            out = torch.empty((H, W), device=mask.device, dtype=torch.int32)
        elif tuple(out.shape) != (H, W):
            bad("out must be [%d, %d], got %s" % (H, W, tuple(out.shape)))
        if out.data_ptr() < mask.data_ptr() + 4 * H * W and mask.data_ptr() < out.data_ptr() + 4 * H * W:
            bad("out aliases mask")
        if stats is not None and stats.numel() < 3:
            bad("stats needs 3 elements")
        self._adopt_stream()
        self.ctx._check(self.ctx.lib.vido_mask_propagate(self.ctx.h, C.c_void_p(mask.data_ptr()), C.c_void_p(flow.data_ptr()), C.c_void_p(depth.data_ptr()) if depth is not None else None,
                                                         H, W, C.c_void_p(out.data_ptr()), C.c_void_p(stats.data_ptr()) if stats is not None else None))
        return out

    def mask_associate(self, prev, cur, state, classes=None, n=None, hold=0, out=None, lut=None, stats=None):
        from ..host import VidoError
        def bad(why):
            raise VidoError(-1, "mask_associate: " + why)
        for name, t, dt in (("cur", cur, torch.int32), ("prev", prev, torch.int32), ("state", state, torch.int32), ("classes", classes, torch.int64), ("out", out, torch.int32),
                            ("lut", lut, torch.int32), ("stats", stats, torch.int32)):
# ... 253 lines not shown
```

Baseline: 125.8.

## Skip dead detection slots in mask-head kernels using a device-side live count

The detection ordering kernel now also writes a 32-bit live-detection count on the device. The mask-head kernels (ROI align, 3x3 convs, 2x2 deconv, logit select) read that count and exit early or shrink their tile space, so padded, non-live detection slots cost almost nothing. The grid is still sized for the full capacity and a host sync is never needed, but outputs for dead slots are left unwritten (logit select zeros them), so anything downstream that reads those slots sees garbage.

```diff
diff --git a/include/vido_c.h b/include/vido_c.h
--- a/include/vido_c.h
+++ b/include/vido_c.h
@@ -169,8 +169,11 @@
 int vido_correlation(vido_ctx* ctx, const float* first, const float* second, int B, int C, int H, int W, int stride,
                      float* out, int on_device);
 int vido_det_order(vido_ctx* ctx, const float* scores, const long long* labels, const int* n_det, float confidence, int cap, long long* order, long long* labels_out, long long* n_live);
+int vido_det_order_n(vido_ctx* ctx, const float* scores, const long long* labels, const int* n_det, float confidence, int cap, long long* order, long long* labels_out, long long* n_live,
+                     int32_t* n_live32);
 int vido_roi_levels(vido_ctx* ctx, const float* boxes, int n, float k_min, float k_max, int* out);
 int vido_mask_logit_select(vido_ctx* ctx, const float* feat, const float* w, const float* b, const long long* labels, float* out, int n, int c, int hw, int classes);
+int vido_mask_logit_select_n(vido_ctx* ctx, const float* feat, const float* w, const float* b, const long long* labels, float* out, int n, int c, int hw, int classes, const int32_t* n_live);
 int vido_bias_act(vido_ctx* ctx, float* x, const float* bias, int N, int C, int H, int W, float slope);
 int vido_bias_unary(vido_ctx* ctx, float* x, const float* bias, int N, int C, int H, int W, int kind);
 int vido_upcat_reflect(vido_ctx* ctx, const float* x, const float* skip, int C1, int C2, int h, int w, float* out);
@@ -188,6 +191,7 @@
 int vido_conv1x1_bias_act(vido_ctx* ctx, const float* x, const float* w_packed, const float* bias, const float* residual, float* y, int cin, int cout, int hw, float slope);
 int vido_deconv2x2_supported(int n, int cin, int cout, int h, int w);
 int vido_deconv2x2_bias_act(vido_ctx* ctx, const float* x, const float* w_packed, const float* bias, float* y, int n, int cin, int cout, int h, int w, float slope);
+int vido_deconv2x2_bias_act_n(vido_ctx* ctx, const float* x, const float* w_packed, const float* bias, float* y, int n, int cin, int cout, int h, int w, float slope, const int32_t* n_live);
 int vido_conv1x1_bias_up2_act(vido_ctx* ctx, const float* x, const float* w_packed, const float* bias, const float* residual_half, float* y, int cin, int cout, int h, int w, float slope);
 
 int vido_conv_kxk_c2(vido_ctx* ctx, const float* x, const float* w, const float* bias, const float* residual, float* y, int cin, int k, int h, int w_);
@@ -210,6 +214,7 @@
 int vido_conv3x3_h_supported(int n, int cin, int cout, int h, int w);
 int vido_conv3x3_h_workgroups(int n, int cout, int h, int w);
 int vido_conv3x3_h_bias_act(vido_ctx* ctx, const float* x, const void* w_packed, const float* bias, float* y, int n, int cin, int cout, int h, int w, float slope);
+int vido_conv3x3_h_bias_act_n(vido_ctx* ctx, const float* x, const void* w_packed, const float* bias, float* y, int n, int cin, int cout, int h, int w, float slope, const int32_t* n_live);
 long long vido_wino3x3_packed_floats_form(int cin, int cout, int form);
 int vido_wino3x3_pack_form(const float* w, int cin, int cout, int form, float* u_packed);
 int vido_wino3x3_bias_act_form(vido_ctx* ctx, const float* x, const float* u_packed, const float* bias, float* y, int n, int cin, int cout, int h, int w, float slope, int form);
@@ -233,6 +238,8 @@
 int vido_nchw_to_nhwc(vido_ctx* ctx, const float* src, int B, int C, int H, int W, float* dst);
 int vido_roi_align_fpn_nhwc(vido_ctx* ctx, const float* const feat[4], const int H[4], const int W[4], const float scale[4], int C, const float* boxes, const int32_t* level,
                             int n, int pooled_h, int pooled_w, int sampling_ratio, float* out);
+int vido_roi_align_fpn_nhwc_n(vido_ctx* ctx, const float* const feat[4], const int H[4], const int W[4], const float scale[4], int C, const float* boxes, const int32_t* level,
+                              int n, int pooled_h, int pooled_w, int sampling_ratio, float* out, const int32_t* n_live);
 int vido_bawin_create(vido_ctx* ctx, int cap_frames, int cap_features);
 int vido_bawin_push_frame(vido_ctx* ctx, int frame, int n, const double* meas, const float* xyz, const int32_t* asso);
 int vido_bawin_set_labels(vido_ctx* ctx, int n, const int32_t* quads);
diff --git a/vido-slam_amd/csrc/conv1x1.hip b/vido-slam_amd/csrc/conv1x1.hip
--- a/vido-slam_amd/csrc/conv1x1.hip
+++ b/vido-slam_amd/csrc/conv1x1.hip
@@ -9,7 +9,7 @@
 #define C1_TM 128
 #define C1_TN 128
 
-struct C1Args { const float* x; const float* wp; const float* bias; const float* res; float* y; int M, N, K, mt, total, nchunk; float slope; unsigned xbytes, wbytes; int W; unsigned* range_flag; int hwimg, c4; };
+struct C1Args { const float* x; const float* wp; const float* bias; const float* res; float* y; int M, N, K, mt, total, nchunk; float slope; unsigned xbytes, wbytes; int W; unsigned* range_flag; int hwimg, c4; const int* n_live; };
 
 template <int RES, int KC>
 __global__ __launch_bounds__(256) void k_conv1x1(C1Args A)
@@ -244,8 +244,16 @@
     extern __shared__ __attribute__((aligned(16))) float c1_lds[];
     char* L = (char*)c1_lds;
     const int tid = threadIdx.x, lane = tid & 63, wv = __builtin_amdgcn_readfirstlane(tid >> 6), w = wv & 3, g = wv >> 2;
-    const int per = gridDim.x >> 3, item = (blockIdx.x & 7) * per + (blockIdx.x >> 3);
-    if (item >= A.total) return;
+    int total = A.total, per = gridDim.x >> 3, NL = A.N;
+    unsigned xbytes = A.xbytes;
+    if constexpr (RES == 3) {
+        if (A.n_live) {
+            const int nl = min(max(*A.n_live, 0), A.N / A.hwimg);
+            NL = nl * A.hwimg; total = A.mt * ((NL + C1_TN - 1) / C1_TN); per = (total + 7) >> 3; xbytes = 4u * (unsigned)A.K * (unsigned)NL;
+        }
+    }
+    const int q8 = blockIdx.x >> 3, item = (blockIdx.x & 7) * per + q8;
+    if (q8 >= per || item >= total) return;
     const int nt = item / A.mt, mtile = item - nt * A.mt, n0 = nt * C1_TN, m0 = mtile * C1_TM;
     const int ns = A.nchunk, nb = ns / G;
     const __amdgpu_buffer_rsrc_t wr = __builtin_amdgcn_make_buffer_rsrc((void*)A.wp, 0, A.wbytes, 0x00020000);
@@ -265,7 +273,7 @@
         const unsigned aoff = (unsigned)(NP * 1024) * (unsigned)t, boff = bstep * (unsigned)t;
 #pragma unroll
         for (int q = 0; q < NP; q++) __builtin_amdgcn_raw_ptr_buffer_load_lds(wr, (__attribute__((address_space(3))) void*)(S + q * 4096), 16, avo, abase[q] + aoff, 0, 0);
-        const __amdgpu_buffer_rsrc_t xr = __builtin_amdgcn_make_buffer_rsrc((void*)((const char*)A.x + boff), 0, A.xbytes - boff, 0x00020000);
+        const __amdgpu_buffer_rsrc_t xr = __builtin_amdgcn_make_buffer_rsrc((void*)((const char*)A.x + boff), 0, xbytes - boff, 0x00020000);
 #pragma unroll
         for (int q = 0; q < 2; q++) __builtin_amdgcn_raw_ptr_buffer_load_lds(xr, (__attribute__((address_space(3))) void*)(S + NP * 4096 + q * 4096), 16, bvo[q], 0, 0, 0);
     };
@@ -397,7 +405,7 @@
     }
     auto ep_load = [&](int rb, Ep& E) {
         const int co0 = m0 + 32 * rb + 4 * (lane >> 5);
-        if (q_out < A.N) {
+        if (q_out < NL) {
 #pragma unroll
             for (int r = 0; r < 16; r++) {
                 const int co = co0 + 8 * (r >> 2) + (r & 3);
@@ -412,7 +420,7 @@
         float ov[16];
 #pragma unroll
         for (int r = 0; r < 16; r++) ov[r] = other ? other[r * 64] : 0.f;
-        if (q_out < A.N) {
+        if (q_out < NL) {
 #pragma unroll
             for (int r = 0; r < 16; r++) {
                 const int co = co0 + 8 * (r >> 2) + (r & 3);
@@ -480,10 +488,10 @@
 }
 
 static int c1_launch(vido_ctx* ctx, const float* x, const float* w_packed, const float* bias, const float* residual, int res_mode, float* y, int cin, int cout, int hw, int w, float slope,
-                     int hwimg = 0, int c4 = 0)
+                     int hwimg = 0, int c4 = 0, const int32_t* n_live = nullptr)
 {
     if (!ctx) return VIDO_E_INVALID;
-    if (!x || !w_packed || !y || x == y || !vido_conv1x1_supported(cin, cout, hw) || slope < 0.f || slope > 1.f || (((uintptr_t)x | (uintptr_t)y | (uintptr_t)residual) & 3) || ((uintptr_t)w_packed & 15))
+    if (!x || !w_packed || !y || x == y || !vido_conv1x1_supported(cin, cout, hw) || slope < 0.f || slope > 1.f || (((uintptr_t)x | (uintptr_t)y | (uintptr_t)residual | (uintptr_t)n_live) & 3) || ((uintptr_t)w_packed & 15))
         return vido_set_error(ctx, VIDO_E_INVALID, "conv1x1: no kernel for %d -> %d channels at %d positions (or a pointer is misaligned, or slope outside [0, 1])", cin, cout, hw);
     HIP_TRY(ctx, hipSetDevice(ctx->device));
     hipStream_t st = ctx->has_ext_stream ? ctx->ext_stream : ctx->stream;
@@ -493,7 +501,7 @@
     if (layout >= 2) {
         const int np = layout == 3 ? 2 : 3;
         const int mt = cout / C1_TM, ntl = (hw + C1_TN - 1) / C1_TN, total = mt * ntl;
-        C1Args A{x, w_packed, bias, residual, y, cout, hw, cin, mt, total, cin / 16, slope, (unsigned)(4ll * cin * hw), (unsigned)(2ll * np * cin * cout), w, ctx->c1_range_flag, hwimg, c4};
+        C1Args A{x, w_packed, bias, residual, y, cout, hw, cin, mt, total, cin / 16, slope, (unsigned)(4ll * cin * hw), (unsigned)(2ll * np * cin * cout), w, ctx->c1_range_flag, hwimg, c4, n_live};
         static const int force_form = [] { const char* e = getenv("VIDO_CONV1X1_B3_FORM"); return e ? atoi(e) : 0; }();
         int form = force_form ? force_form : (cin >= 512 && total <= 320 ? 2 : 3);
         if (form == 2 && cin % 64) form = 3;
@@ -561,8 +569,12 @@
 }
 int vido_deconv2x2_bias_act(vido_ctx* ctx, const float* x, const float* w_packed, const float* bias, float* y, int n, int cin, int cout, int h, int w, float slope)
 {
+    return vido_deconv2x2_bias_act_n(ctx, x, w_packed, bias, y, n, cin, cout, h, w, slope, nullptr);
+}
+int vido_deconv2x2_bias_act_n(vido_ctx* ctx, const float* x, const float* w_packed, const float* bias, float* y, int n, int cin, int cout, int h, int w, float slope, const int32_t* n_live)
+{
     if (ctx && !vido_deconv2x2_supported(n, cin, cout, h, w)) return vido_set_error(ctx, VIDO_E_INVALID, "deconv2x2: no kernel for %d x %d -> %d channels at %d x %d", n, cin, cout, h, w);
-    return c1_launch(ctx, x, w_packed, bias, nullptr, 3, y, cin, 4 * cout, n * h * w, w, slope, h * w, cout);
+    return c1_launch(ctx, x, w_packed, bias, nullptr, 3, y, cin, 4 * cout, n * h * w, w, slope, h * w, cout, n_live);
 }
 
 int vido_conv1x1_bias_act(vido_ctx* ctx, const float* x, const float* w_packed, const float* bias, const float* residual, float* y, int cin, int cout, int hw, float slope)
diff --git a/vido-slam_amd/csrc/conv3x3h.hip b/vido-slam_amd/csrc/conv3x3h.hip
--- a/vido-slam_amd/csrc/conv3x3h.hip
+++ b/vido-slam_amd/csrc/conv3x3h.hip
@@ -18,7 +18,7 @@
 #define C3_PBUF(BR) (2 * C3_PLANE(BR))
 #define C3_LDS(BR) (C3_RBW * C3_WSLOT + C3_RAW(BR) + 2 * C3_PBUF(BR))
 
-struct C3Args { const float* x; const void* wp; const float* bias; float* y; int N, Cin, Cout, H, W, nby, nbx, mt, total, nchunk; float slope; unsigned wbytes; unsigned* range_flag; };
+struct C3Args { const float* x; const void* wp; const float* bias; float* y; int N, Cin, Cout, H, W, nby, nbx, mt, total, nchunk; float slope; unsigned wbytes; unsigned* range_flag; const int* n_live; };
 
 template <int RPW, int CG>
 __global__ __launch_bounds__(512) void k_conv3x3_h(C3Args A)
@@ -27,8 +27,10 @@
     extern __shared__ __attribute__((aligned(16))) char c3_lds[];
     char* L = c3_lds;
     const int tid = threadIdx.x, lane = tid & 63, w = __builtin_amdgcn_readfirstlane(tid >> 6);
-    const int per = gridDim.x >> 3, item = (blockIdx.x & 7) * per + (blockIdx.x >> 3);
-    if (item >= A.total) return;
+    int total = A.total, per = gridDim.x >> 3;
+    if (A.n_live) { const int nl = min(max(*A.n_live, 0), A.N); total = nl * A.nby * A.nbx * A.mt; per = (total + 7) >> 3; }
+    const int q8 = blockIdx.x >> 3, item = (blockIdx.x & 7) * per + q8;
+    if (q8 >= per || item >= total) return;
     const int nt = item / A.mt, mtile = item - nt * A.mt, m0 = mtile * MT;
     const int bpi = A.nby * A.nbx, n = nt / bpi, brem = nt - n * bpi, by = brem / A.nbx, bx = brem - by * A.nbx, Y0 = by * BR, X0 = bx * 16;
     const int rp = CG == 1 ? w : (w & 3), rb0 = CG == 1 ? 0 : RPW * (w >> 2);
@@ -195,15 +197,20 @@
 
 int vido_conv3x3_h_bias_act(vido_ctx* ctx, const float* x, const void* w_packed, const float* bias, float* y, int n, int cin, int cout, int h, int w, float slope)
 {
+    return vido_conv3x3_h_bias_act_n(ctx, x, w_packed, bias, y, n, cin, cout, h, w, slope, nullptr);
+}
+
+int vido_conv3x3_h_bias_act_n(vido_ctx* ctx, const float* x, const void* w_packed, const float* bias, float* y, int n, int cin, int cout, int h, int w, float slope, const int32_t* n_live)
+{
     if (!ctx) return VIDO_E_INVALID;
-    if (!x || !w_packed || !y || x == y || !vido_conv3x3_h_supported(n, cin, cout, h, w) || slope < 0.f || slope > 1.f || (((uintptr_t)x | (uintptr_t)y) & 3) || ((uintptr_t)w_packed & 15))
+    if (!x || !w_packed || !y || x == y || !vido_conv3x3_h_supported(n, cin, cout, h, w) || slope < 0.f || slope > 1.f || (((uintptr_t)x | (uintptr_t)y | (uintptr_t)n_live) & 3) || ((uintptr_t)w_packed & 15))
         return vido_set_error(ctx, VIDO_E_INVALID, "conv3x3_h: no kernel for %d x %d -> %d channels at %d x %d (or a pointer is misaligned, or slope outside [0, 1])", n, cin, cout, h, w);
     HIP_TRY(ctx, hipSetDevice(ctx->device));
     hipStream_t st = ctx->has_ext_stream ? ctx->ext_stream : ctx->stream;
     const int br = c3_block_rows(n, cout, h, w);
     const int nby = (h + br - 1) / br, nbx = (w + 15) / 16, mt = cout >= 128 ? cout / 128 : 1, total = n * nby * nbx * mt;
     const int nchunk = (cin + 15) / 16;
-    C3Args A{x, w_packed, bias, y, n, cin, cout, h, w, nby, nbx, mt, total, nchunk, slope, (unsigned)(36ll * 16 * nchunk * cout), ctx->c1_range_flag};
+    C3Args A{x, w_packed, bias, y, n, cin, cout, h, w, nby, nbx, mt, total, nchunk, slope, (unsigned)(36ll * 16 * nchunk * cout), ctx->c1_range_flag, n_live};
     static bool attr[64] = {};
     if (!attr[ctx->device & 63]) {
 #define C3_ATTR(RPW_, CG_) HIP_TRY(ctx, hipFuncSetAttribute((const void*)k_conv3x3_h<RPW_, CG_>, hipFuncAttributeMaxDynamicSharedMemorySize, (int)C3_LDS(16 / CG_)))
diff --git a/vido-slam_amd/csrc/nets.hip b/vido-slam_amd/csrc/nets.hip
--- a/vido-slam_amd/csrc/nets.hip
+++ b/vido-slam_amd/csrc/nets.hip
@@ -54,7 +54,7 @@
 }
 
 __global__ __launch_bounds__(1024) void k_det_order(const float* __restrict__ scores, const long long* __restrict__ labels, const int* __restrict__ n_det, float confidence, int cap,
-                                                   long long* __restrict__ order, long long* __restrict__ labels_out, long long* __restrict__ n_live)
+                                                   long long* __restrict__ order, long long* __restrict__ labels_out, long long* __restrict__ n_live, int* __restrict__ n_live32)
 {
     __shared__ float key[1024];
     __shared__ int cnt;
@@ -71,7 +71,7 @@
         if (live) atomicAdd(&cnt, 1);
     }
     __syncthreads();
-    if (i == 0) *n_live = cnt;
+    if (i == 0) { *n_live = cnt; if (n_live32) *n_live32 = cnt; }
 }
 
 __global__ void k_roi_levels(const float* __restrict__ boxes, int n, float k_min, float k_max, int* __restrict__ out)
@@ -87,10 +87,14 @@
 }
 
 __global__ __launch_bounds__(256) void k_mask_logit_select(const float* __restrict__ feat, const float* __restrict__ w, const float* __restrict__ b, const long long* __restrict__ labels,
-                                                           float* __restrict__ out, int c, int hw, int classes)
+                                                           float* __restrict__ out, int c, int hw, int classes, const int* __restrict__ n_live)
 {
     __shared__ float wl[1024];
     const int n = blockIdx.y, p = blockIdx.x * 256 + threadIdx.x;
+    if (n_live && n >= *n_live) {
+        if (p < hw) out[(size_t)n * hw + p] = 0.f;
+        return;
+    }
     long long lab = labels[n]; lab = lab < 0 ? 0 : (lab >= classes ? classes - 1 : lab);
     for (int i = threadIdx.x; i < c; i += 256) wl[i] = w[(size_t)lab * c + i];
     __syncthreads();
@@ -167,9 +171,10 @@
 struct RoiLevels { const float* feat[4]; int H[4], W[4]; float scale[4]; };
 template <int SR >
 __global__ __launch_bounds__(256) void k_roi_align_nhwc(RoiLevels L, int C, const float* __restrict__ rois, int roi_stride ,
-                                                        const int* __restrict__ level , int PH, int PW, int sampling, float* __restrict__ out)
+                                                        const int* __restrict__ level , int PH, int PW, int sampling, float* __restrict__ out, const int* __restrict__ n_live )
 {
     extern __shared__ __attribute__((aligned(16))) float rl_tile[];
+    if (n_live && (int)blockIdx.x >= *n_live) return;
     const int i = blockIdx.x, c0 = blockIdx.y * 64, lane = threadIdx.x & 63, wave = threadIdx.x >> 6;
     const int nbin = PH * PW, pitch = nbin | 1;
     const float* r = rois + (size_t)roi_stride * i;
@@ -684,11 +689,16 @@
 
 int vido_det_order(vido_ctx* ctx, const float* scores, const long long* labels, const int* n_det, float confidence, int cap, long long* order, long long* labels_out, long long* n_live)
 {
+    return vido_det_order_n(ctx, scores, labels, n_det, confidence, cap, order, labels_out, n_live, nullptr);
+}
+int vido_det_order_n(vido_ctx* ctx, const float* scores, const long long* labels, const int* n_det, float confidence, int cap, long long* order, long long* labels_out, long long* n_live,
+                     int32_t* n_live32)
+{
     if (!ctx) return VIDO_E_INVALID;
     if (!scores || !labels || !n_det || !order || !labels_out || !n_live || cap < 1 || cap > 1024) return vido_set_error(ctx, VIDO_E_INVALID, "det_order: bad arguments (cap 1 .. 1024)");
     HIP_TRY(ctx, hipSetDevice(ctx->device));
     hipStream_t st = ctx->has_ext_stream ? ctx->ext_stream : ctx->stream;
-    hipLaunchKernelGGL(k_det_order, dim3(1), dim3(1024), 0, st, scores, labels, n_det, confidence, cap, order, labels_out, n_live);
+    hipLaunchKernelGGL(k_det_order, dim3(1), dim3(1024), 0, st, scores, labels, n_det, confidence, cap, order, labels_out, n_live, n_live32);
     HIP_TRY(ctx, hipGetLastError());
     return VIDO_OK;
 }
@@ -707,11 +717,15 @@
 
 int vido_mask_logit_select(vido_ctx* ctx, const float* feat, const float* w, const float* b, const long long* labels, float* out, int n, int c, int hw, int classes)
 {
+    return vido_mask_logit_select_n(ctx, feat, w, b, labels, out, n, c, hw, classes, nullptr);
+}
+int vido_mask_logit_select_n(vido_ctx* ctx, const float* feat, const float* w, const float* b, const long long* labels, float* out, int n, int c, int hw, int classes, const int32_t* n_live)
+{
     if (!ctx) return VIDO_E_INVALID;
     if (!feat || !w || !labels || !out || n < 1 || c < 1 || c > 1024 || hw < 1 || classes < 1) return vido_set_error(ctx, VIDO_E_INVALID, "mask_logit_select: bad arguments");
     HIP_TRY(ctx, hipSetDevice(ctx->device));
     hipStream_t st = ctx->has_ext_stream ? ctx->ext_stream : ctx->stream;
-    hipLaunchKernelGGL(k_mask_logit_select, dim3((unsigned)((hw + 255) / 256), (unsigned)n), dim3(256), 0, st, feat, w, b, labels, out, c, hw, classes);
+    hipLaunchKernelGGL(k_mask_logit_select, dim3((unsigned)((hw + 255) / 256), (unsigned)n), dim3(256), 0, st, feat, w, b, labels, out, c, hw, classes, n_live);
     HIP_TRY(ctx, hipGetLastError());
     return VIDO_OK;
 }
@@ -870,8 +884,8 @@
     const size_t lds = (size_t)64 * ((pooled_h * pooled_w) | 1) * sizeof(float);
     if (lds > 150 * 1024) return vido_set_error(ctx, VIDO_E_CAPACITY, "roi_align: pooled size %d x %d too large", pooled_h, pooled_w);
     { int rc = roi_lds_limit(ctx, lds); if (rc) return rc; }
-    if (sampling_ratio == 2) hipLaunchKernelGGL(k_roi_align_nhwc<2>, dim3(n_rois, (C + 63) / 64), dim3(256), lds, st, L, C, dr, 5, (const int*)nullptr, pooled_h, pooled_w, sampling_ratio, dout);
-    else hipLaunchKernelGGL(k_roi_align_nhwc<0>, dim3(n_rois, (C + 63) / 64), dim3(256), lds, st, L, C, dr, 5, (const int*)nullptr, pooled_h, pooled_w, sampling_ratio, dout);
+    if (sampling_ratio == 2) hipLaunchKernelGGL(k_roi_align_nhwc<2>, dim3(n_rois, (C + 63) / 64), dim3(256), lds, st, L, C, dr, 5, (const int*)nullptr, pooled_h, pooled_w, sampling_ratio, dout, (const int*)nullptr);
+    else hipLaunchKernelGGL(k_roi_align_nhwc<0>, dim3(n_rois, (C + 63) / 64), dim3(256), lds, st, L, C, dr, 5, (const int*)nullptr, pooled_h, pooled_w, sampling_ratio, dout, (const int*)nullptr);
     HIP_TRY(ctx, hipGetLastError());
     if (!on_device) {
         HIP_TRY(ctx, hipStreamSynchronize(st));
@@ -976,6 +990,11 @@
 int vido_roi_align_fpn_nhwc(vido_ctx* ctx, const float* const feat[4], const int H[4], const int W[4], const float scale[4], int C, const float* boxes, const int32_t* level,
                             int n, int pooled_h, int pooled_w, int sampling_ratio, float* out)
 {
+    return vido_roi_align_fpn_nhwc_n(ctx, feat, H, W, scale, C, boxes, level, n, pooled_h, pooled_w, sampling_ratio, out, nullptr);
+}
+int vido_roi_align_fpn_nhwc_n(vido_ctx* ctx, const float* const feat[4], const int H[4], const int W[4], const float scale[4], int C, const float* boxes, const int32_t* level,
+                              int n, int pooled_h, int pooled_w, int sampling_ratio, float* out, const int32_t* n_live)
+{
     if (!ctx) return VIDO_E_INVALID;
     if (!feat || !H || !W || !scale || C < 1 || n < 0 || pooled_h < 1 || pooled_w < 1 || (n && (!boxes || !level || !out))) return vido_set_error(ctx, VIDO_E_INVALID, "roi_align_fpn_nhwc: bad arguments");
     if (n == 0) return VIDO_OK;
@@ -986,8 +1005,8 @@
     const size_t lds = (size_t)64 * ((pooled_h * pooled_w) | 1) * sizeof(float);
     if (lds > 150 * 1024) return vido_set_error(ctx, VIDO_E_CAPACITY, "roi_align_fpn: pooled size %d x %d too large", pooled_h, pooled_w);
     { int rc = roi_lds_limit(ctx, lds); if (rc) return rc; }
-    if (sampling_ratio == 2) hipLaunchKernelGGL(k_roi_align_nhwc<2>, dim3(n, (C + 63) / 64), dim3(256), lds, st, L, C, boxes, 4, level, pooled_h, pooled_w, sampling_ratio, out);
-    else hipLaunchKernelGGL(k_roi_align_nhwc<0>, dim3(n, (C + 63) / 64), dim3(256), lds, st, L, C, boxes, 4, level, pooled_h, pooled_w, sampling_ratio, out);
+    if (sampling_ratio == 2) hipLaunchKernelGGL(k_roi_align_nhwc<2>, dim3(n, (C + 63) / 64), dim3(256), lds, st, L, C, boxes, 4, level, pooled_h, pooled_w, sampling_ratio, out, n_live);
+    else hipLaunchKernelGGL(k_roi_align_nhwc<0>, dim3(n, (C + 63) / 64), dim3(256), lds, st, L, C, boxes, 4, level, pooled_h, pooled_w, sampling_ratio, out, n_live);
     HIP_TRY(ctx, hipGetLastError());
     return VIDO_OK;
 }
diff --git a/vido-slam_amd/nets/maskrcnn.py b/vido-slam_amd/nets/maskrcnn.py
--- a/vido-slam_amd/nets/maskrcnn.py
+++ b/vido-slam_amd/nets/maskrcnn.py
@@ -240,15 +240,15 @@
         return [self.cls_logits(x) for x in t], [self.bbox_pred(x) for x in t]
 
 
-def _conv_bias_relu(conv, x, ops):
+def _conv_bias_relu(conv, x, ops, n_live=None):
     if ops is None or not x.is_cuda or conv.bias is None:
         return F.relu(conv(x))
     if isinstance(conv, nn.Conv2d) and hasattr(ops, "wino3x3_conv") and not os.environ.get("VIDO_NO_WINO"):
-        y = ops.wino3x3_conv(conv, x, 0.0)
+        y = ops.wino3x3_conv(conv, x, 0.0, n_live=n_live) if n_live is not None else ops.wino3x3_conv(conv, x, 0.0)
         if y is not None:
             return y
     if isinstance(conv, nn.ConvTranspose2d) and hasattr(ops, "deconv2x2_conv"):
-        y = ops.deconv2x2_conv(conv, x, 0.0)
+        y = ops.deconv2x2_conv(conv, x, 0.0, n_live) if n_live is not None else ops.deconv2x2_conv(conv, x, 0.0)
         if y is not None:
             return y
     if isinstance(conv, nn.ConvTranspose2d):
@@ -364,14 +364,14 @@
         self.res, self.scales, self.sr, self.ops = resolution, scales, sampling_ratio, ops
         self.k_min = -math.log2(scales[0]); self.k_max = -math.log2(scales[-1])
 
-    def forward(self, feats, boxes):
+    def forward(self, feats, boxes, n_live=None):
         if boxes.is_cuda and boxes.dtype == torch.float32 and hasattr(self.ops, "roi_levels") and not os.environ.get("VIDO_NO_ROI_LEVELS"):
             lvl = self.ops.roi_levels(boxes, self.k_min, self.k_max)
         else:
             area = (boxes[:, 2] - boxes[:, 0] + 1) * (boxes[:, 3] - boxes[:, 1] + 1)
             lvl = torch.floor(4 + torch.log2(torch.sqrt(area) / 224 + 1e-6)).clamp(min=self.k_min, max=self.k_max).to(torch.int64) - int(self.k_min)
         if isinstance(feats, FpnMaps):
-            return self.ops.roi_align_fpn_nhwc(feats.nhwc, boxes, lvl, (self.res, self.res), self.scales, self.sr)
+            return self.ops.roi_align_fpn_nhwc(feats.nhwc, boxes, lvl, (self.res, self.res), self.scales, self.sr, n_live)
         if hasattr(self.ops, "roi_align_fpn") and boxes.is_cuda and len(feats) == 4:
             return self.ops.roi_align_fpn(feats, boxes, lvl, (self.res, self.res), self.scales, self.sr)
         rois = torch.cat([boxes.new_zeros((len(boxes), 1)), boxes], 1)
@@ -504,10 +504,10 @@
         for i, ch in enumerate(c.mask_layers, 1):
             setattr(self, "mask_fcn%d" % i, nn.Conv2d(cin, ch, 3, 1, 1)); self.names.append("mask_fcn%d" % i); cin = ch
 
-    def forward(self, feats, boxes):
-        x = self.pooler(feats, boxes)
+    def forward(self, feats, boxes, n_live=None):
+        x = self.pooler(feats, boxes, n_live) if n_live is not None else self.pooler(feats, boxes)
         for n in self.names:
-            x = _conv_bias_relu(getattr(self, n), x, self.pooler.ops if hasattr(self.pooler.ops, "bias_act_") else None)
+            x = _conv_bias_relu(getattr(self, n), x, self.pooler.ops if hasattr(self.pooler.ops, "bias_act_") else None, n_live)
         return x
 
 
@@ -522,10 +522,10 @@
     def forward(self, x):
         return self.mask_fcn_logits(_conv_bias_relu(self.conv5_mask, x, self._ops))
 
-    def selected(self, x, labels):
-        y = _conv_bias_relu(self.conv5_mask, x, self._ops)
+    def selected(self, x, labels, n_live=None):
+        y = _conv_bias_relu(self.conv5_mask, x, self._ops, n_live)
         if self._ops is not None and y.is_cuda and hasattr(self._ops, "mask_logit_select") and not os.environ.get("VIDO_NO_MASK_SELECT") and labels.dtype == torch.int64:
-            return self._ops.mask_logit_select(y.contiguous(), self.mask_fcn_logits, labels.contiguous())
+            return self._ops.mask_logit_select(y.contiguous(), self.mask_fcn_logits, labels.contiguous(), n_live)
         return self.mask_fcn_logits(y).sigmoid()[torch.arange(x.shape[0], device=labels.device), labels][:, None]
 
 
@@ -636,7 +636,7 @@
 
 
 @torch.no_grad()
-def _heads_static(self, feats, logits, deltas, image_hw, cap=None):
+def _heads_static(self, feats, logits, deltas, image_hw, cap=None, confidence=None):
     H, W = image_hw; c = self.config; cap = cap or c.detections_per_img
     fused = self.fused_post and hasattr(self.rpn.ops, "det_select") and c.pre_nms_top_n <= 1024 and c.rpn_min_size <= 0
     proposals, objectness = (self.rpn.proposals_fused if fused else self.rpn.proposals_device)(feats, logits, deltas, (W, H))
@@ -645,8 +645,14 @@
     lg, dl = bh.predictor(bh.feature_extractor(maps, proposals))
     boxes, scores, labels, n_det = (bh.postprocess_fused if fused else bh.postprocess_static)(lg, dl, proposals, (W, H), objectness, cap)
     mh = self.roi_heads.mask
-    masks = mh.predictor.selected(mh.feature_extractor(maps, boxes), labels)
-    return dict(boxes=boxes, scores=scores, labels=labels, masks=masks, n_det=n_det, proposals=proposals, objectness=objectness, n_proposals=(objectness >= 0).sum())
+    out = dict(boxes=boxes, scores=scores, labels=labels, n_det=n_det, proposals=proposals, objectness=objectness, n_proposals=(objectness >= 0).sum())
+    if confidence is not None:
+        order, lab, n_live, n32 = self.rpn.ops.det_order(scores.contiguous(), labels.contiguous(), n_det.reshape(1), confidence, count32=True)
+        out.update(order=order, labels_ordered=lab, n_live=n_live,
+                   masks=mh.predictor.selected(mh.feature_extractor(maps, boxes[order], n32), lab, n32))
+        return out
+    out["masks"] = mh.predictor.selected(mh.feature_extractor(maps, boxes), labels)
+    return out
 
 
 MaskRCNN.fused_post = True
@@ -687,7 +693,11 @@
 def analyse_image_static(net, feats, logits, deltas, out_hw, feed=(1088, 800), confidence=0.8, cap=None, label_mode="class", id_base=None):
     _check_label_mode(label_mode)
     H, W = out_hw
-    out = net.heads_static(feats, logits, deltas, feed, cap)
+    ops = net.rpn.ops
+    c = net.config; ncap = cap or c.detections_per_img
+    fused = net.fused_post and hasattr(ops, "det_select") and c.pre_nms_top_n <= 1024 and c.rpn_min_size <= 0
+    live_first = (hasattr(ops, "det_order") and fused and ncap <= 1024 and feats[0].is_cuda and not os.environ.get("VIDO_NO_DET_ORDER") and not os.environ.get("VIDO_MASK_HEAD_ALL"))
+    out = net.heads_static(feats, logits, deltas, feed, cap, confidence) if live_first else net.heads_static(feats, logits, deltas, feed, cap)
     cap = out["boxes"].shape[0]
     rw, rh = float(W) / feed[1], float(H) / feed[0]
     cache = net.__dict__.setdefault("_const_cache", {})
@@ -695,21 +705,25 @@
     if key not in cache:
         cache[key] = out["boxes"].new_tensor([rw, rh, rw, rh])
     boxes = out["boxes"] * cache[key]
-    ops = net.rpn.ops
     nd = out["n_det"]
-    if hasattr(ops, "det_order") and cap <= 1024 and nd.dtype == torch.int32 and out["labels"].dtype == torch.int64 and not os.environ.get("VIDO_NO_DET_ORDER"):
+    if "order" in out:
+        order, labels, n_live = out["order"], out["labels_ordered"], out["n_live"]
+        masks = out["masks"]
+    elif hasattr(ops, "det_order") and cap <= 1024 and nd.dtype == torch.int32 and out["labels"].dtype == torch.int64 and not os.environ.get("VIDO_NO_DET_ORDER"):
         order, labels, n_live = ops.det_order(out["scores"].contiguous(), out["labels"].contiguous(), nd.reshape(1), confidence)
     else:
         live = (out["scores"] > confidence) & (torch.arange(cap, device=boxes.device) < nd)
         order = torch.sort(torch.where(live, out["scores"], out["scores"].new_full((), -1.0)), descending=True, stable=True)[1]
         labels = torch.where(live, out["labels"], torch.zeros_like(out["labels"]))[order]
         n_live = live.sum()
+    if "order" not in out:
+        masks = out["masks"][order]
     if label_mode == "instance":
         if cap > 255:
             raise ValueError("label_mode='instance': %d slots, ids are u8" % cap)
-        img = ops.mask_instance_image(out["masks"][order], boxes[order], labels, H, W, id_base=id_base)
+        img = ops.mask_instance_image(masks, boxes[order], labels, H, W, id_base=id_base)
     else:
-        img = ops.mask_label_image(out["masks"][order], boxes[order], labels, H, W)
+        img = ops.mask_label_image(masks, boxes[order], labels, H, W)
     return img, labels, n_live, out["n_det"]
 
 
diff --git a/vido-slam_amd/nets/ops.py b/vido-slam_amd/nets/ops.py
--- a/vido-slam_amd/nets/ops.py
+++ b/vido-slam_amd/nets/ops.py
@@ -25,6 +25,13 @@
     @property
     def range_safe_active(self):
         return self._range_safe > 0
+
+    @staticmethod
+    def _live_ptr(n_live):
+        if n_live is None:
+            return None
+        assert n_live.is_cuda and n_live.dtype == torch.int32 and n_live.numel() == 1, "n_live: a one-element int32 device tensor"
+        return C.c_void_p(n_live.data_ptr())
 
     def _adopt_stream(self):
         st = torch.cuda.current_stream().cuda_stream
@@ -48,7 +55,7 @@
         self.ctx._check(self.ctx.lib.vido_bias_act(self.ctx.h, C.c_void_p(x.data_ptr()), C.c_void_p(bias.data_ptr()), N, Cc, H, W, C.c_float(slope)))
         return x
 
-    def deconv2x2_conv(self, conv, x, slope):
+    def deconv2x2_conv(self, conv, x, slope, n_live=None):
         w = conv.weight
         if (tuple(w.shape[2:]) != (2, 2) or tuple(conv.stride) != (2, 2) or tuple(conv.padding) != (0, 0) or tuple(conv.output_padding) != (0, 0) or tuple(conv.dilation) != (1, 1)
                 or conv.groups != 1 or not x.is_cuda or x.dtype != torch.float32 or os.environ.get("VIDO_NO_DECONV_H") or self._range_safe):
@@ -63,18 +70,19 @@
         self.gconv_flops = getattr(self, "gconv_flops", 0.0) + 2.0 * n * cin * cout * 4 * H * W
         self._adopt_stream()
         b = conv.bias
-        self.ctx._check(self.ctx.lib.vido_deconv2x2_bias_act(self.ctx.h, C.c_void_p(x.contiguous().data_ptr()), C.c_void_p(conv._dc_w.data_ptr()), C.c_void_p(b.data_ptr()) if b is not None else None,
-                                                             C.c_void_p(out.data_ptr()), n, cin, cout, H, W, C.c_float(slope)))
-        return out
-
-    def det_order(self, scores, labels, n_det, confidence):
+        self.ctx._check(self.ctx.lib.vido_deconv2x2_bias_act_n(self.ctx.h, C.c_void_p(x.contiguous().data_ptr()), C.c_void_p(conv._dc_w.data_ptr()), C.c_void_p(b.data_ptr()) if b is not None else None,
+                                                               C.c_void_p(out.data_ptr()), n, cin, cout, H, W, C.c_float(slope), self._live_ptr(n_live)))
+        return out
+
+    def det_order(self, scores, labels, n_det, confidence, count32=False):
         assert scores.is_cuda and scores.dtype == torch.float32 and labels.dtype == torch.int64 and n_det.dtype == torch.int32 and scores.is_contiguous() and labels.is_contiguous()
         cap = int(scores.shape[0]); dev = scores.device
         order = torch.empty((cap,), device=dev, dtype=torch.int64); lab = torch.empty((cap,), device=dev, dtype=torch.int64); n_live = torch.empty((), device=dev, dtype=torch.int64)
-        self._adopt_stream()
-        self.ctx._check(self.ctx.lib.vido_det_order(self.ctx.h, C.c_void_p(scores.data_ptr()), C.c_void_p(labels.data_ptr()), C.c_void_p(n_det.data_ptr()), C.c_float(confidence), cap,
-                                                    C.c_void_p(order.data_ptr()), C.c_void_p(lab.data_ptr()), C.c_void_p(n_live.data_ptr())))
-        return order, lab, n_live
+        n32 = torch.empty((1,), device=dev, dtype=torch.int32) if count32 else None
+        self._adopt_stream()
+        self.ctx._check(self.ctx.lib.vido_det_order_n(self.ctx.h, C.c_void_p(scores.data_ptr()), C.c_void_p(labels.data_ptr()), C.c_void_p(n_det.data_ptr()), C.c_float(confidence), cap,
+                                                      C.c_void_p(order.data_ptr()), C.c_void_p(lab.data_ptr()), C.c_void_p(n_live.data_ptr()), C.c_void_p(n32.data_ptr()) if count32 else None))
+        return (order, lab, n_live, n32) if count32 else (order, lab, n_live)
 
     def roi_levels(self, boxes, k_min, k_max):
         assert boxes.is_cuda and boxes.dtype == torch.float32
@@ -84,7 +92,7 @@
         self.ctx._check(self.ctx.lib.vido_roi_levels(self.ctx.h, C.c_void_p(boxes.data_ptr()), n, C.c_float(k_min), C.c_float(k_max), C.c_void_p(out.data_ptr())))
         return out
 
-    def mask_logit_select(self, feat, conv, labels):
+    def mask_logit_select(self, feat, conv, labels, n_live=None):
         assert feat.is_cuda and feat.is_contiguous() and feat.dtype == torch.float32 and labels.dtype == torch.int64 and labels.is_contiguous()
         n, c, H, W = feat.shape; classes = int(conv.weight.shape[0])
         w = conv.weight.reshape(classes, c)
@@ -92,8 +100,8 @@
             w = w.contiguous()
         out = torch.empty((n, 1, H, W), device=feat.device, dtype=torch.float32)
         self._adopt_stream()
-        self.ctx._check(self.ctx.lib.vido_mask_logit_select(self.ctx.h, C.c_void_p(feat.data_ptr()), C.c_void_p(w.data_ptr()), C.c_void_p(conv.bias.data_ptr()) if conv.bias is not None else None,
-                                                            C.c_void_p(labels.data_ptr()), C.c_void_p(out.data_ptr()), int(n), int(c), int(H * W), classes))
+        self.ctx._check(self.ctx.lib.vido_mask_logit_select_n(self.ctx.h, C.c_void_p(feat.data_ptr()), C.c_void_p(w.data_ptr()), C.c_void_p(conv.bias.data_ptr()) if conv.bias is not None else None,
+                                                            C.c_void_p(labels.data_ptr()), C.c_void_p(out.data_ptr()), int(n), int(c), int(H * W), classes, self._live_ptr(n_live)))
         return out
 
     def bias_res_act_(self, x, bias, res, slope):
@@ -298,7 +306,7 @@
                                                                 C.c_void_p(out.data_ptr()), int(N), int(cin), int(cout), int(H), int(W), C.c_float(slope), int(form)))
         return out
 
-    def wino3x3_conv(self, conv, x, slope, weight=None, bias=None):
+    def wino3x3_conv(self, conv, x, slope, weight=None, bias=None, n_live=None):
         w = conv.weight if weight is None else weight
         b = conv.bias if bias is None and weight is None else bias
         if (tuple(w.shape[2:]) != (3, 3) or tuple(conv.stride) != (1, 1) or tuple(conv.padding) != (1, 1) or tuple(conv.dilation) != (1, 1) or conv.groups != 1
@@ -312,7 +320,7 @@
             key = (w.data_ptr(), w._version, str(x.device))
             if getattr(conv, "_c3h_key", None) != key:
                 conv._c3h_w = pack_conv3x3_h(w).to(x.device); conv._c3h_key = key
-            return self.conv3x3_h_bias_act(x.contiguous(), conv._c3h_w, b, int(w.shape[0]), slope)
+            return self.conv3x3_h_bias_act(x.contiguous(), conv._c3h_w, b, int(w.shape[0]), slope, n_live)
         form = self.wino3x3_form(x.shape[0], w.shape[1], w.shape[0], x.shape[2], x.shape[3])
         key = (w.data_ptr(), w._version, str(x.device))
         if getattr(conv, "_wino_key", None) != key:
@@ -321,15 +329,15 @@
             conv._wino_u[form] = pack_wino3x3(w, form).to(x.device)
         return self.wino3x3_bias_act(x.contiguous(), conv._wino_u[form], b, int(w.shape[0]), slope, form)
 
-    def conv3x3_h_bias_act(self, x, w_packed, bias, cout, slope):
+    def conv3x3_h_bias_act(self, x, w_packed, bias, cout, slope, n_live=None):
         assert x.is_cuda and x.is_contiguous() and x.dtype == torch.float32
         N, cin, H, W = x.shape
         assert w_packed.dtype == torch.int16 and w_packed.numel() == 2 * cout * ((cin + 15) // 16 * 16 * 9 + 1), "conv3x3_h: weight not packed by pack_conv3x3_h for this layer"
         out = torch.empty((N, cout, H, W), device=x.device, dtype=torch.float32)
         self.gconv_flops = getattr(self, "gconv_flops", 0.0) + 2.0 * N * cout * cin * 9 * H * W
         self._adopt_stream()
-        self.ctx._check(self.ctx.lib.vido_conv3x3_h_bias_act(self.ctx.h, C.c_void_p(x.data_ptr()), C.c_void_p(w_packed.data_ptr()), C.c_void_p(bias.data_ptr()) if bias is not None else None,
-                                                             C.c_void_p(out.data_ptr()), int(N), int(cin), int(cout), int(H), int(W), C.c_float(slope)))
+        self.ctx._check(self.ctx.lib.vido_conv3x3_h_bias_act_n(self.ctx.h, C.c_void_p(x.data_ptr()), C.c_void_p(w_packed.data_ptr()), C.c_void_p(bias.data_ptr()) if bias is not None else None,
+                                                               C.c_void_p(out.data_ptr()), int(N), int(cin), int(cout), int(H), int(W), C.c_float(slope), self._live_ptr(n_live)))
         return out
 
     def fc_h(self, x, w_packed, bias, outs, slope=1.0):
@@ -531,7 +539,7 @@
         self.ctx._check(self.ctx.lib.vido_nchw_to_nhwc(self.ctx.h, C.c_void_p(x.data_ptr()), B, Cc, H, W, C.c_void_p(out.data_ptr())))
         return out
 
-    def roi_align_fpn_nhwc(self, feats_nhwc, boxes, level, output_size, scales, sampling_ratio):
+    def roi_align_fpn_nhwc(self, feats_nhwc, boxes, level, output_size, scales, sampling_ratio, n_live=None):
         n = boxes.shape[0]; ph, pw = output_size; Cc = feats_nhwc[0].shape[3]
         out = torch.empty((n, Cc, ph, pw), device=boxes.device, dtype=torch.float32)
         if n == 0:
@@ -540,8 +548,8 @@
         fp = (C.c_void_p * 4)(*[f.data_ptr() for f in feats_nhwc]); Hs = (C.c_int * 4)(*[f.shape[1] for f in feats_nhwc]); Ws = (C.c_int * 4)(*[f.shape[2] for f in feats_nhwc])
         sc = (C.c_float * 4)(*[float(x) for x in scales])
         self._adopt_stream()
-        self.ctx._check(self.ctx.lib.vido_roi_align_fpn_nhwc(self.ctx.h, fp, Hs, Ws, sc, Cc, C.c_void_p(boxes.data_ptr()), C.c_void_p(level.data_ptr()), n, ph, pw, sampling_ratio,
-                                                             C.c_void_p(out.data_ptr())))
+        self.ctx._check(self.ctx.lib.vido_roi_align_fpn_nhwc_n(self.ctx.h, fp, Hs, Ws, sc, Cc, C.c_void_p(boxes.data_ptr()), C.c_void_p(level.data_ptr()), n, ph, pw, sampling_ratio,
+                                                               C.c_void_p(out.data_ptr()), self._live_ptr(n_live)))
         return out
 
     def mask_label_image(self, masks, boxes, labels, H, W, thresh=0.5, padding=1):
```

Result: faster. 128.4 (median of 6 runs) (+2.1%).
